# usnistgov/alignn

Hardware: AMD Instinct MI355X
Metric: graphs/sec (train fwd+bwd), batch=64 JARVIS-DFT crystals, 4+4 ALIGNN layers (higher is better)
Workload: dtype f32 (projections: split-product MFMA - 3 fp16-slice or 6 bf16-slice products, fp32 accumulate, fp32-grade error)

## Files before the change

### alignn_amd/_abi.py

```python

from __future__ import annotations

import ctypes as C
import keyword
import os
import re
from functools import lru_cache
from typing import NamedTuple

HEADER = os.path.join(os.path.dirname(os.path.dirname(os.path.abspath(__file__))), "include", "alignn_hip.h")

WORKFLOW_HEADERS = ("alignn_thermo.h", "alignn_neb.h", "alignn_traj.h", "alignn_sym.h", "alignn_order.h", "alignn_phsym.h")
LATER_HEADERS = ("alignn_idpp.h", "alignn_cells.h", "alignn_local.h")
ANALYSIS_HEADERS = ("alignn_vanhove.h",)
STRUCTURE_HEADERS = ("alignn_voronoi.h",)

_BASE = {"void": None, "char": C.c_char, "uint8_t": C.c_uint8, "uint64_t": C.c_uint64, "int": C.c_int, "int32_t": C.c_int32,
         "int64_t": C.c_int64, "size_t": C.c_size_t, "float": C.c_float, "double": C.c_double}

_ITEM = re.compile(r"typedef\s+struct\s+(\w+)\s*\{([^{}]*)\}\s*(\w+)\s*;"
                   r"|typedef\s+([^;{}()]+);"
                   r"|([^;{}()]+?\b\w+)\s*\(([^;{}()]*)\)\s*;")
_GAP = re.compile(r'\s*(extern\s*"C"\s*\{)?\s*\}?\s*')
_DECLARATION = re.compile(r"\s*(?:const\s+)?(\w+)\b(.*)", re.S)
_DECLARATOR = re.compile(r"\s*(\**)\s*(\w+)\s*")
_DIRECTIVE = re.compile(r"^[ \t]*#[ \t]*define\b(.*)$", re.M)
_MACRO = re.compile(r"[ \t]+(\w+)(?![\w(])[ \t]*(.*?)[ \t]*")
_INT = re.compile(r"[+-]?(?:0[xX][0-9a-fA-F]+|[1-9][0-9]*|0)")
_FLOAT = re.compile(r"[+-]?(?:[0-9]+\.[0-9]*|\.[0-9]+|[0-9]+(?=[eE]))(?:[eE][+-]?[0-9]+)?")


def _uncomment(text: str) -> str:
    return re.sub(r"/\*.*?\*/", lambda m: " " + "\n" * m.group().count("\n"), text, flags=re.S)


def parse(text: str):
    text = re.sub(r"^[ \t]*#.*$", "", _uncomment(text), flags=re.M)
    types, structs, sigs = dict(_BASE), {}, {}

    def fail(what, at):
        raise ValueError(f"line {text.count(chr(10), 0, at) + 1}: {what}")

    def gap(a, b):
        if not _GAP.fullmatch(text, a, b):
            junk = text[a:b]
            fail(f"cannot read {junk.strip()!r}", a + len(junk) - len(junk.lstrip()))

    def decl(s, at):
        at += len(s) - len(s.lstrip())
        m = _DECLARATION.fullmatch(s)
        if not m or m.group(1) not in types:
            fail(f"unknown type in {s.strip()!r}", at)
        out = []
        for d in m.group(2).split(","):
            dm = _DECLARATOR.fullmatch(d)
            ctype = (C.c_void_p if dm.group(1) else types[m.group(1)]) if dm else None
            if ctype is None:
                fail(f"cannot read the declarator {d.strip()!r} of {s.strip()!r}", at)
            name = dm.group(2)
            out.append((name + "_" if keyword.iskeyword(name) else name, ctype))
        return out

    pos = 0
    for m in _ITEM.finditer(text):
        gap(pos, m.start())
        pos = m.end()
        tag, body, name, alias, head, params = m.groups()
        if tag is not None:
            if tag != name:
                fail(f"struct {tag} is named {name}", m.start())
            fields = [f for s in body.split(";") if s.strip() for f in decl(s, m.start(2) + body.find(s))]
            types[name] = structs[name] = type(name, (C.Structure,), {"_fields_": fields})
        elif alias is not None:
            (name, ctype), = decl(alias, m.start())
            types[name] = ctype
        else:
            (name, res), = decl(head, m.start(5))
            if re.match(r"\s*const\s+char\s*\*", head):
                res = C.c_char_p
            args = [] if params.strip() == "void" else [decl(p, m.start(6))[0][1] for p in params.split(",")]
            sigs[name] = (res, args)
    gap(pos, len(text))
    return structs, sigs


def defines(text: str) -> dict:
    text, out = _uncomment(text), {}
    for m in _DIRECTIVE.finditer(text):
        macro = _MACRO.fullmatch(m.group(1))
        name, value = macro.groups() if macro else (None, None)
        if value and _INT.fullmatch(value):
            out[name] = int(value, 0)
        elif value and _FLOAT.fullmatch(value):
            out[name] = float(value)
        elif value != "":
            raise ValueError(f"line {text.count(chr(10), 0, m.start()) + 1}: cannot read the macro {m.group().strip()!r}")
    return out


class Header(NamedTuple):
    path: str
    structs: dict
    signatures: dict
    defines: dict


@lru_cache(maxsize=None)
def header(name: str) -> Header:
    path = os.path.join(os.path.dirname(HEADER), name)
    with open(path) as f:
        text = f.read()
    structs, sigs = parse(text)
    for block in structs:
        if sigs.get(block + "_size") != (C.c_size_t, []):
            raise ValueError(f"{name}: the argument block {block} has no size query size_t {block}_size(void)")
    return Header(path, structs, sigs, defines(text))


with open(HEADER) as _f:
    STRUCTS, SIGNATURES = parse(_f.read())
```

### alignn_amd/_lib.py

```python

from __future__ import annotations

import ctypes as C
import os

import torch

from ._abi import SIGNATURES, STRUCTS

HERE = os.path.dirname(os.path.abspath(__file__))
LIB_PATH = os.path.join(HERE, "libalignn_hip.so")
LIB_PATH = os.environ.get("ALIGNN_AMD_LIB_PATH", LIB_PATH)

EgcFwdArgs, EgcBwdArgs, EgcWgradArgs = (STRUCTS[f"alignn_egc_{k}_args"] for k in ("fwd", "bwd", "wgrad"))
FireArgs, MdArgs = STRUCTS["alignn_fire_args"], STRUCTS["alignn_md_args"]


_lib = None
_bound = {}


def _type(lib, signatures):
    for name, (res, args) in signatures.items():
        fn = getattr(lib, name)
        fn.restype = res
        fn.argtypes = args


def _check_size(name, size, block):
    if size != C.sizeof(block):
        raise RuntimeError(f"argument block {name}: library says {size} bytes, the header gives {C.sizeof(block)}")


def load() -> C.CDLL:
    global _lib
    if _lib is None:
        if not os.path.exists(LIB_PATH):
            raise RuntimeError(
                f"{LIB_PATH} not found: build it with `python -m alignn_amd.build` "
                "(hipcc --offload-arch=gfx950); alignn_amd has no CPU/eager fallback."
            )
        lib = C.CDLL(LIB_PATH)
        _type(lib, SIGNATURES)
        sizes = [lib.alignn_egc_args_sizeof(k) for k in range(3)] + [lib.alignn_fire_args_sizeof(), lib.alignn_md_args_sizeof()]
        for size, block in zip(sizes, (EgcFwdArgs, EgcBwdArgs, EgcWgradArgs, FireArgs, MdArgs)):
            _check_size(block.__name__, size, block)
        _lib = lib
    return _lib


def bind(header, lib=None):
    lib = load() if lib is None else lib
    if _bound.get(header.path) is not lib:
        _type(lib, header.signatures)
        for name, block in header.structs.items():
            _check_size(name, getattr(lib, name + "_size")(), block)
        _bound[header.path] = lib
    return lib


def ptr(t):
    return None if t is None else t.data_ptr()


_raw_stream = getattr(torch._C, "_cuda_getCurrentRawStream", None)


def stream():
    if _raw_stream is not None:
        return _raw_stream(torch.cuda.current_device())
    return torch.cuda.current_stream().cuda_stream


class _NoGuard:
    def __enter__(self):
        return None

    def __exit__(self, *exc):
        return False


_NO_GUARD = _NoGuard()


def device_guard(t):
    if t.is_cuda and t.device.index != torch.cuda.current_device():
        return torch.cuda.device(t.device)
    return _NO_GUARD


def check(rc: int, what: str):
    if rc != 0:
        raise RuntimeError(f"libalignn_hip: {what} failed with hipError {rc}")


def require_f32(*tensors):
    for t in tensors:
        if t is None:
            continue
        if t.dtype != torch.float32 or not t.is_cuda:
            raise TypeError(
                f"alignn_amd kernels take float32 CUDA(HIP) tensors, got {t.dtype} on {t.device}; "
                "there is no CPU fallback"
            )
```

### alignn_amd/build.py

```python

from __future__ import annotations

import os
import re
import shutil
import subprocess
import sys
import tempfile
from concurrent.futures import ThreadPoolExecutor

from ._abi import ANALYSIS_HEADERS, LATER_HEADERS, STRUCTURE_HEADERS, WORKFLOW_HEADERS

HERE = os.path.dirname(os.path.abspath(__file__))
CSRC = os.path.join(HERE, "csrc")
OBJ = os.path.join(HERE, "build")
LIB = os.path.join(HERE, "libalignn_hip.so")
SOURCES = ["norm.hip", "conv.hip", "gemm_f32.hip", "gemm_x6.hip", "embed.hip", "dual.hip", "knn.hip", "composite.hip", "model.hip", "stage.hip", "radius.hip", "angle.hip", "ff.hip", "convln.hip", "gemm_dw.hip", "relax.hip", "dynamics.hip", "phonon.hip", "defects.hip", "eos.hip", "elastic.hip", "interface.hip", "thermo.hip", "neb.hip", "trajectory.hip", "symmetry.hip", "order.hip", "phonon_sym.hip", "idpp.hip", "cells.hip", "local_order.hip", "vanhove.hip", "voronoi.hip"]
FLAGS = ["--offload-arch=gfx950", "-O3", "-std=c++17", "-fPIC"]
DEVICE_FLAGS: list = []
_NO_SLP = ["-fno-slp-vectorize"]
EXTRA_FLAGS = {"norm.hip": _NO_SLP, "dual.hip": _NO_SLP, "convln.hip": _NO_SLP, "radius.hip": _NO_SLP, "ff.hip": _NO_SLP}

_OBJDUMP = "/opt/rocm/lib/llvm/bin/llvm-objdump"
_PK = re.compile(r"\b(v_pk_(?:fma|mul|add)_f32)\b(.*)$")
_OPSEL = re.compile(r"op_sel:\[([01]),([01])")
_SYM = re.compile(r"^[0-9a-f]+ <([^>]+)>:$")


def faulting_packed_forms(lib: str = None) -> list:
    lib = lib or LIB
    found = []
    with tempfile.TemporaryDirectory() as tmp:
        copy = os.path.join(tmp, "lib.so")
        shutil.copy(lib, copy)
        subprocess.run([_OBJDUMP, "--offloading", copy], check=True, capture_output=True)
        bundles = sorted(f for f in os.listdir(tmp) if "gfx950" in f)
        if not bundles:
            raise RuntimeError(f"{lib}: no gfx950 code object found")
        for b in bundles:
            dis = subprocess.run([_OBJDUMP, "-d", "--no-show-raw-insn", os.path.join(tmp, b)], check=True, capture_output=True, text=True).stdout
            cur = "?"
            for line in dis.splitlines():
                m = _SYM.match(line)
                if m:
                    cur = m.group(1)
                    continue
                m = _PK.search(line)
                if m:
                    o = _OPSEL.search(m.group(2))
                    if o and o.group(2) == "1":
                        found.append((cur, (m.group(1) + m.group(2)).split("//")[0].strip()))
    return found


def _headers():
    include = os.path.join(os.path.dirname(HERE), "include")
    return [os.path.join(CSRC, f) for f in os.listdir(CSRC) if f.endswith(".h")] + [
        os.path.join(include, f) for f in ("alignn_hip.h",) + WORKFLOW_HEADERS + LATER_HEADERS + ANALYSIS_HEADERS + STRUCTURE_HEADERS]


def _stale(target, deps) -> bool:
    if not os.path.exists(target):
        return True
    t = os.path.getmtime(target)
    return any(os.path.getmtime(d) > t for d in deps)


def build(force: bool = False, verbose: bool = False) -> str:
    hipcc = os.environ.get("HIPCC", "/opt/rocm/bin/hipcc")
    hdrs = _headers()
    srcs = [s for s in SOURCES if os.path.exists(os.path.join(CSRC, s))]
    if not force and not _stale(LIB, [os.path.join(CSRC, s) for s in srcs] + hdrs + [os.path.abspath(__file__)]):
        return LIB
    os.makedirs(OBJ, exist_ok=True)
    objs = [os.path.join(OBJ, s.replace(".hip", ".o")) for s in srcs]

    def compile_one(pair):
        src, obj = pair
        if force or _stale(obj, [os.path.join(CSRC, src), os.path.abspath(__file__)] + hdrs):
            cmd = [hipcc] + FLAGS + DEVICE_FLAGS + EXTRA_FLAGS.get(src, []) + ["-c", os.path.join(CSRC, src), "-o", obj]
            if verbose:
                print(" ".join(cmd), flush=True)
            subprocess.run(cmd, check=True)
            return True
        return False

    with ThreadPoolExecutor(max_workers=min(8, len(srcs))) as pool:
        rebuilt = list(pool.map(compile_one, zip(srcs, objs)))
    if force or any(rebuilt) or _stale(LIB, objs):
        cmd = [hipcc, "--offload-arch=gfx950", "-shared", "-fPIC", "-o", LIB] + objs
        if verbose:
            print(" ".join(cmd), flush=True)
        subprocess.run(cmd, check=True)
        bad = faulting_packed_forms(LIB)
        if bad:
            os.replace(LIB, LIB + ".rejected")
            raise RuntimeError("libalignn_hip.so contains the packed-fp32 form that MI355X gets wrong beside MFMA waves "
                               "(see EXTRA_FLAGS in alignn_amd/build.py): " + "; ".join(f"{k}: {i}" for k, i in bad[:8]))
    return LIB


if __name__ == "__main__":
    print(build(force="--force" in sys.argv, verbose=True))
```

### alignn_amd/csrc/composite.hip

```cpp
#include "common.h"
#include "../../include/alignn_hip.h"

namespace {

inline size_t al(size_t floats) { return (floats + 63) / 64 * 64; }

#define ALIGNN_TRY(call)            \
    do {                            \
        int rc__ = (call);          \
        if (rc__ != 0) return rc__; \
    } while (0)

struct FwdScratch {
    size_t e_part, e_fold, n_part, bd2, total;
    int e_slabs, n_slabs;
};
FwdScratch fwd_scratch(int64_t n, int64_t m, int H, int Kin, int edge_kind) {
    FwdScratch s{};
    s.n_slabs = alignn_egc_slabs(n);
    s.e_slabs = edge_kind >= 1 ? alignn_gemm_nt_x6_row_tiles(m, H, Kin) : s.n_slabs;
    size_t off = 0;
    s.e_part = off, off += al(edge_kind >= 1 ? (size_t)(s.e_slabs + 1) * 2 * H : (size_t)s.e_slabs * (3 * H + 1));
    s.e_fold = off, off += al((size_t)alignn_slab_fold_slabs() * 2 * H);
    s.n_part = off, off += al((size_t)s.n_slabs * (3 * H + 1));
    s.bd2 = off, off += edge_kind == 2 ? al((size_t)n * H) : 0;
    s.total = off;
    return s;
}

struct BwdScratch {
    size_t n_red_part, e_red_part, dx_ws, dy_part, dy_fold, total;
    int n_slabs, e_slabs, dy_tiles;
    size_t dx_bytes;
};
BwdScratch bwd_scratch(int64_t n, int64_t m, int H, int Kin, int dx_kind, int dy_kind) {
    BwdScratch s{};
    s.n_slabs = alignn_col_stats_slabs(n);
    s.e_slabs = alignn_col_stats_slabs(m);
    size_t off = 0;
    s.n_red_part = off, off += al((size_t)s.n_slabs * 2 * H);
    s.e_red_part = off, off += al((size_t)s.e_slabs * 2 * H);
    s.dx_bytes = dx_kind == 2 ? alignn_gemm_nn_split_workspace(n, 4 * H, Kin) : 0;
    s.dx_ws = off, off += al(s.dx_bytes / 4);
    s.dy_tiles = dy_kind == 1 ? alignn_gemm_nt_x6_row_tiles(m, Kin, H) : 0;
    s.dy_part = off, off += al((size_t)(s.dy_tiles + 1) * 2 * Kin);
    s.dy_fold = off, off += al((size_t)alignn_slab_fold_slabs() * 2 * Kin);
    s.total = off;
    return s;
}

int bn_finalize_folded(const float* partial, int slabs, float* fold, int64_t rows, int F, const float* gamma,
                       const float* beta, float eps, float momentum, float* rm, float* rv, float* stat,
                       alignn_stream_t st) {
    if (slabs > kFoldAbove) {
        ALIGNN_TRY(alignn_slab_fold(partial, slabs, 2 * F, fold, st));
        partial = fold;
        slabs = alignn_slab_fold_slabs();
    }
    return alignn_bn_finalize(partial, slabs, rows, F, gamma, beta, eps, momentum, rm, rv, stat, st);
}

hipEvent_t g_fork_ev[kMaxDevices][2];
bool g_fork_ok[kMaxDevices];

inline bool fork_events(hipEvent_t* fork, hipEvent_t* join) {
    int dev = -1;
    if (hipGetDevice(&dev) != hipSuccess || dev < 0 || dev >= kMaxDevices || !g_fork_ok[dev]) return false;
    *fork = g_fork_ev[dev][0];
    *join = g_fork_ev[dev][1];
    return true;
}

}

extern "C" {

int alignn_fork_events_init(void) {
    int dev = -1;
    hipError_t e = hipGetDevice(&dev);
    if (e != hipSuccess) return (int)e;
    if (dev < 0 || dev >= kMaxDevices) return (int)hipErrorInvalidDevice;
    if (g_fork_ok[dev]) return 0;
    for (int i = 0; i < 2; ++i) {
        e = hipEventCreateWithFlags(&g_fork_ev[dev][i], hipEventDisableTiming);
        if (e != hipSuccess) return (int)e;
    }
    g_fork_ok[dev] = true;
    return 0;
}

size_t alignn_egc_args_sizeof(int which) {
    switch (which) {
        case 0: return sizeof(alignn_egc_fwd_args);
        case 1: return sizeof(alignn_egc_bwd_args);
        case 2: return sizeof(alignn_egc_wgrad_args);
        default: return 0;
    }
}

size_t alignn_egc_conv_fwd_scratch(int64_t n, int64_t m, int H, int Kin, int edge_kind) {
    return fwd_scratch(n, m, H, Kin, edge_kind).total * sizeof(float);
}

int alignn_egc_conv_fwd(const alignn_egc_fwd_args* a, alignn_stream_t st) {
    if (a == nullptr || a->scratch == nullptr || a->H <= 0 || (a->H & 3)) return (int)hipErrorInvalidValue;
    const int H = a->H, Kin = a->Kin;
    const int64_t n = a->n, m = a->m;
    const FwdScratch s = fwd_scratch(n, m, H, Kin, a->edge_kind);
    if (a->scratch_bytes < s.total * sizeof(float)) return (int)hipErrorInvalidValue;
    float* e_part = a->scratch + s.e_part;
    float* e_fold = a->scratch + s.e_fold;
    float* n_part = a->scratch + s.n_part;
    if (a->node_kind == 1)
        ALIGNN_TRY(alignn_gemm_nt_f16x3(a->x, Kin, a->x_amax, a->wcat_img, a->wcat_amax, a->bcat, nullptr, 0, a->P, 4 * H, n,
                                        4 * H, Kin, st));
    else
        ALIGNN_TRY(alignn_gemm_nt(a->x, Kin, a->wcat, Kin, a->bcat, nullptr, 0, a->P, 4 * H, n, 4 * H, Kin, st));
    if (a->edge_kind >= 1) {
        if (a->edge_kind == 2) {
            if (a->seg_rank == nullptr || a->seg_node == nullptr) return (int)hipErrorInvalidValue;
            float* bd2 = a->scratch + s.bd2;
            ALIGNN_TRY(alignn_gather_rows_ld(a->P + H, 4 * H, a->seg_node, bd2, H, n, H, st));
            ALIGNN_TRY(alignn_gemm_nt_f16x3_gather2(a->y, Kin, a->y_amax, a->weg_img, a->weg_amax, a->b_eg, a->M, H, m, H, Kin,
                                                    a->P, 4 * H, a->src, bd2, H, a->seg_rank, e_part, st));
        } else
            ALIGNN_TRY(alignn_gemm_nt_f16x3_gather(a->y, Kin, a->y_amax, a->weg_img, a->weg_amax, a->b_eg, a->M, H, m, H, Kin,
                                                   a->P, 4 * H, a->src, a->dst, e_part, st));
        ALIGNN_TRY(bn_finalize_folded(e_part, s.e_slabs, e_fold, m, H, a->e_gamma, a->e_beta, a->eps, a->momentum, a->e_rm,
                                      a->e_rv, a->e_stat, st));
        if (a->y_out != nullptr)
            ALIGNN_TRY(alignn_egc_gate_fwd_pre_norm(a->P, a->M, a->seg_ptr, a->seg_node, a->src, n, m, H, a->xpre, a->s0, a->hh,
                                                    n_part, a->e_stat, a->residual ? a->y : nullptr, a->y_out, a->y_out_amax, st));
        else
            ALIGNN_TRY(alignn_egc_gate_fwd_pre(a->P, a->M, a->seg_ptr, a->seg_node, a->src, n, m, H, a->xpre, a->s0, a->hh,
                                               nullptr, n_part, st));
    } else {
        ALIGNN_TRY(alignn_gemm_nt(a->y, Kin, a->w_eg, Kin, a->b_eg, nullptr, 0, a->M, H, m, H, Kin, st));
        ALIGNN_TRY(alignn_egc_gate_fwd(a->P, a->M, a->seg_ptr, a->seg_node, a->src, n, m, H, a->xpre, a->s0, a->hh, e_part,
                                       n_part, st));
        ALIGNN_TRY(alignn_bn_finalize_welford(e_part, s.e_slabs, m, H, a->e_gamma, a->e_beta, a->eps, a->momentum, a->e_rm,
                                              a->e_rv, a->e_stat, st));
        if (a->y_out != nullptr)
            ALIGNN_TRY(alignn_bn_silu_fwd(a->M, H, a->residual ? a->y : nullptr, a->residual ? Kin : 0, a->e_stat, a->y_out, H,
                                          m, H, a->y_out_amax, st));
    }
    ALIGNN_TRY(alignn_bn_finalize_welford(n_part, s.n_slabs, n, H, a->n_gamma, a->n_beta, a->eps, a->momentum, a->n_rm,
                                          a->n_rv, a->n_stat, st));
    ALIGNN_TRY(alignn_bn_silu_fwd(a->xpre, H, a->residual ? a->x : nullptr, a->residual ? Kin : 0, a->n_stat, a->x_out, H, n, H,
                                  a->x_out_amax, st));
    return 0;
}

size_t alignn_egc_conv_bwd_scratch(int64_t n, int64_t m, int H, int Kin, int dx_kind, int dy_kind) {
    return bwd_scratch(n, m, H, Kin, dx_kind, dy_kind).total * sizeof(float);
}

int alignn_egc_conv_bwd(const alignn_egc_bwd_args* a, alignn_stream_t st) {
    if (a == nullptr || a->scratch == nullptr || a->H <= 0 || (a->H & 3)) return (int)hipErrorInvalidValue;
    const int H = a->H, Kin = a->Kin;
    const int64_t n = a->n, m = a->m;
    const BwdScratch s = bwd_scratch(n, m, H, Kin, a->dx_kind, a->dy_kind);
    if (a->scratch_bytes < s.total * sizeof(float)) return (int)hipErrorInvalidValue;
    float* n_red_part = a->scratch + s.n_red_part;
    float* e_red_part = a->scratch + s.e_red_part;
    float* g_xpre = a->GP + 3 * (size_t)H;
    ALIGNN_TRY(alignn_bn_silu_bwd_reduce(a->gx_out, H, a->xpre, H, a->n_stat, n, H, n_red_part, st));
    ALIGNN_TRY(alignn_bn_bwd_finalize(n_red_part, s.n_slabs, H, a->n_red, st));
    ALIGNN_TRY(alignn_bn_silu_bwd_apply_node(a->gx_out, H, a->xpre, H, a->n_stat, a->n_gamma, a->n_red, 0, g_xpre, 4 * H, n, H,
                                             a->gp_amax, a->s0, a->hh, a->gs1, a->gs0, st));
    const float* e_red = a->e_red_in;
    if (a->gy_out != nullptr && e_red == nullptr) {
        ALIGNN_TRY(alignn_bn_silu_bwd_reduce(a->gy_out, H, a->M, H, a->e_stat, m, H, e_red_part, st));
        ALIGNN_TRY(alignn_bn_bwd_finalize(e_red_part, s.e_slabs, H, a->e_red, st));
        e_red = a->e_red;
    }
    if (a->gate_mode == 2) {
        ALIGNN_TRY(alignn_egc_bwd_lg_dense(a->gy_out, a->M, a->P, a->gs1, a->gs0, a->e_stat, e_red, 0, m, a->grp_seg_ptr,
                                           a->grp_src_ptr, a->n_groups, a->dense_max_src, a->seg_ptr, a->seg_node, H, a->GM,
                                           a->GP, a->gb_part, a->gm_amax, a->gp_amax, st));
    } else if (a->gate_mode == 1) {
        ALIGNN_TRY(alignn_egc_bwd_lg_fused(a->gy_out, a->M, a->P, a->gs1, a->gs0, a->e_stat, e_red, 0, m, a->grp_seg_ptr,
                                           a->grp_src_ptr, a->n_groups, a->seg_ptr, a->seg_node, a->dst, a->out_ptr, a->out_slot,
                                           H, a->GM, a->GP, a->gb_part, a->gm_amax, a->gp_amax, st));
    } else {
        ALIGNN_TRY(alignn_egc_bwd_dst(a->gy_out, a->M, a->P, a->gs1, a->gs0, a->e_stat, a->e_gamma, e_red, 0, m, a->seg_ptr,
                                      a->seg_node, a->src, n, H, a->GM, a->GP, a->gb_part, a->gm_amax, a->gp_amax, st));
        ALIGNN_TRY(alignn_egc_bwd_src(a->GM, a->M, a->gs1, a->out_ptr, a->out_slot, a->dst, n, H, a->GP, a->gp_amax, st));
    }
    hipEvent_t ev_fork, ev_join;
    const bool forked = a->aux_stream != nullptr && fork_events(&ev_fork, &ev_join);
    alignn_stream_t st_main = st;
    if (forked) {
        ALIGNN_TRY((int)hipEventRecord(ev_fork, (hipStream_t)st_main));
        ALIGNN_TRY((int)hipStreamWaitEvent((hipStream_t)a->aux_stream, ev_fork, 0));
        st = a->aux_stream;
    }
    const float* addx = a->residual ? a->gx_out : nullptr;
    switch (a->dx_kind) {
        case 1:
            ALIGNN_TRY(alignn_gemm_nt_f16x3(a->GP, 4 * H, a->gp_amax, a->wcat_t_img, a->wcat_amax, nullptr, addx, addx ? H : 0, a->g_x, Kin, n,
                                            Kin, 4 * H, st));
            break;
        case 2:
            ALIGNN_TRY(alignn_gemm_nn_split(a->GP, 4 * H, a->wcat, Kin, addx, addx ? H : 0, a->g_x, Kin, n, 4 * H, Kin,
                                            a->scratch + s.dx_ws, s.dx_bytes, st));
            break;
        case 4:
            ALIGNN_TRY(alignn_gemm_nt(a->GP, 4 * H, a->wcat_t, 4 * H, nullptr, addx, addx ? H : 0, a->g_x, Kin, n, Kin, 4 * H, st));
            break;
        default:
            ALIGNN_TRY(alignn_gemm_nn(a->GP, 4 * H, a->wcat, Kin, addx, addx ? H : 0, a->g_x, Kin, n, 4 * H, Kin, st));
    }
    if (forked) {
        ALIGNN_TRY((int)hipEventRecord(ev_join, (hipStream_t)a->aux_stream));
        st = st_main;
    }
    const float* addy = (a->residual && a->gy_out != nullptr) ? a->gy_out : nullptr;
    switch (a->dy_kind) {
        case 1: {
            float* part = a->scratch + s.dy_part;
            ALIGNN_TRY(alignn_gemm_nt_f16x3_bnred(a->GM, H, a->gm_amax, a->weg_t_img, a->weg_amax, nullptr, addy, addy ? H : 0,
                                                  a->g_y, Kin, m, Kin, H, a->src_xn, a->src_ldxn, a->src_nstat, part, st));
            int tiles = s.dy_tiles;
            if (tiles > kFoldAbove) {
                ALIGNN_TRY(alignn_slab_fold(part, tiles, 2 * Kin, a->scratch + s.dy_fold, st));
                part = a->scratch + s.dy_fold;
                tiles = alignn_slab_fold_slabs();
            }
            ALIGNN_TRY(alignn_bn_bwd_finalize(part, tiles, Kin, a->src_red, st));
            break;
        }
        case 5:
            ALIGNN_TRY(alignn_gemm_nt_f16x3(a->GM, H, a->gm_amax, a->weg_t_img, a->weg_amax, nullptr, addy, addy ? H : 0, a->g_y,
                                            Kin, m, Kin, H, st));
            break;
        case 2: {
            const size_t bytes = alignn_gemm_nn_split_workspace(m, H, Kin);
            (void)bytes;
            return (int)hipErrorInvalidValue;
        }
        case 4:
            ALIGNN_TRY(alignn_gemm_nt(a->GM, H, a->weg_t, H, nullptr, addy, addy ? H : 0, a->g_y, Kin, m, Kin, H, st));
            break;
        default:
            ALIGNN_TRY(alignn_gemm_nn(a->GM, H, a->w_eg, Kin, addy, addy ? H : 0, a->g_y, Kin, m, H, Kin, st));
    }
    if (forked) ALIGNN_TRY((int)hipStreamWaitEvent((hipStream_t)st_main, ev_join, 0));
    return 0;
}

size_t alignn_egc_conv_wgrad_scratch(int64_t n, int64_t m, int H, int Kin) {
    return (al(alignn_gemm_tn_workspace(m, H, Kin) / 4 + 1) + al(alignn_gemm_tn_workspace(n, 4 * H, Kin) / 4 + 1) +
            al((size_t)alignn_col_stats_slabs(n) * 2 * 4 * H)) * sizeof(float);
}

int alignn_egc_conv_wgrad(const alignn_egc_wgrad_args* a, alignn_stream_t st) {
    if (a == nullptr || a->scratch == nullptr) return (int)hipErrorInvalidValue;
    const int H = a->H, Kin = a->Kin;
    const int64_t n = a->n, m = a->m;
    const size_t b1 = alignn_gemm_tn_workspace(m, H, Kin), b2 = alignn_gemm_tn_workspace(n, 4 * H, Kin);
    float* ws1 = a->scratch;
    float* ws2 = ws1 + al(b1 / 4 + 1);
    float* ws3 = ws2 + al(b2 / 4 + 1);
    if (a->scratch_bytes < alignn_egc_conv_wgrad_scratch(n, m, H, Kin)) return (int)hipErrorInvalidValue;
    ALIGNN_TRY(alignn_slab_sum(a->gb_part, a->gb_slabs, H, a->g_beg, st));
    ALIGNN_TRY(alignn_gemm_tn(a->GM, H, a->gm_amax, a->y, Kin, a->y_amax, a->g_weg, Kin, m, H, Kin, ws1, b1, st));
    ALIGNN_TRY(alignn_gemm_tn(a->GP, 4 * H, a->gp_amax, a->x, Kin, a->x_amax, a->g_wcat, Kin, n, 4 * H, Kin, ws2, b2, st));
    ALIGNN_TRY(alignn_col_sum(a->GP, 4 * H, n, 4 * H, a->g_bcat, ws3, st));
    return 0;
}

}
```

### alignn_amd/csrc/gemm_f32.hip

```cpp
#include "mfma_f16x3.h"
#include "../../include/alignn_hip.h"

namespace {

constexpr int BK = 32;
constexpr int RC_LD = BK + 4;

template <int BMN, bool RC>
struct TileShape {
    static constexpr int kFloats = RC ? BMN * RC_LD : BK * BMN;
};

template <int BMN, bool RC, int NT>
struct Stager {
    static constexpr int NV = (BMN * BK / 4) / NT;
    static_assert((BMN * BK / 4) % NT == 0, "tile must divide over the block");
    float4 v[NV];

    __device__ __forceinline__ void load(const float* __restrict__ S, int64_t ld, int64_t i0, int64_t i_ext,
                                         int64_t r0, int64_t r_ext, int t) {
#pragma unroll
        for (int j = 0; j < NV; ++j) {
            const int id = t + j * NT;
            int64_t gi, gr;
            if (RC) {
                gi = i0 + id / (BK / 4);
                gr = r0 + (id % (BK / 4)) * 4;
            } else {
                gr = r0 + id / (BMN / 4);
                gi = i0 + (id % (BMN / 4)) * 4;
            }
            if (gi < i_ext && gr < r_ext)
                v[j] = RC ? f4_ld(S + gi * ld + gr) : f4_ld(S + gr * ld + gi);
            else
                v[j] = f4_zero();
        }
    }
    __device__ __forceinline__ void store(float* T, int t) const {
#pragma unroll
        for (int j = 0; j < NV; ++j) {
            const int id = t + j * NT;
            if (RC)
                f4_st(T + (id / (BK / 4)) * RC_LD + (id % (BK / 4)) * 4, v[j]);
            else
                f4_st(T + (id / (BMN / 4)) * BMN + (id % (BMN / 4)) * 4, v[j]);
        }
    }
};

template <int BMN, bool RC>
__device__ __forceinline__ void fetch4(const float* T, int irow, int j, int half, float (&out)[4]) {
    if (RC) {
        float4 q = f4_ld(T + irow * RC_LD + 8 * j + 4 * half);
        out[0] = q.x;
        out[1] = q.y;
        out[2] = q.z;
        out[3] = q.w;
    } else {
        const float* p = T + (8 * j + 4 * half) * BMN + irow;
        out[0] = p[0];
        out[1] = p[BMN];
        out[2] = p[2 * BMN];
        out[3] = p[3 * BMN];
    }
}

struct GemmArgs {
    const float* A;
    int64_t lda;
    const float* B;
    int64_t ldb;
    const float* bias;
    const float* addend;
    int64_t ldadd;
    float* C;
    int64_t ldc;
    int64_t Mo;
    int No;
    int64_t R;
    int64_t r_chunk;
    int64_t c_split;
    int xcd_group;
    int tiles_m, tiles_n, splits;
};

template <int BM, int BN, int WM, int WN, bool A_RC, bool B_RC, bool HAS_ADD>
__global__ __launch_bounds__(WM * WN * 64) void gemm_mfma_kernel(GemmArgs g) {
    constexpr int NT = WM * WN * 64;
    constexpr int TM = BM / WM, TN = BN / WN;
    constexpr int RM = TM / 32, RN = TN / 32;
    constexpr int A_FL = TileShape<BM, A_RC>::kFloats, B_FL = TileShape<BN, B_RC>::kFloats;
    extern __shared__ __attribute__((aligned(16))) float smem[];
    constexpr int STAGE = A_FL + B_FL;

    const int t = threadIdx.x;
    const int lane = t & 63, wave = t >> 6;
    const int wm = wave / WN, wn = wave % WN;
    const int il = lane & 31, half = lane >> 5;
    int bx = blockIdx.x, by = blockIdx.y, bz = blockIdx.z;
    if (g.xcd_group) {
        const int tiles = g.tiles_m * g.tiles_n;
        const int L = blockIdx.x;
        const int xcd = L & 7, j = L >> 3;
        bz = xcd + 8 * (j / tiles);
        const int tile = j % tiles;
        bx = tile % g.tiles_m;
        by = tile / g.tiles_m;
        if (bz >= g.splits) return;
    }
    const int64_t m0 = (int64_t)bx * BM;
    const int64_t n0 = (int64_t)by * BN;
    const int64_t rbeg = (int64_t)bz * g.r_chunk;
    int64_t rend = rbeg + g.r_chunk;
    if (rend > g.R) rend = g.R;
    float* C = g.C + (int64_t)bz * g.c_split;

    f32x16 acc[RM][RN];
#pragma unroll
    for (int a = 0; a < RM; ++a)
#pragma unroll
        for (int b = 0; b < RN; ++b)
#pragma unroll
            for (int r = 0; r < 16; ++r) acc[a][b][r] = 0.0f;

    const bool vec = ((g.No & 3) == 0) && ((g.ldc & 3) == 0) && ((reinterpret_cast<uintptr_t>(C) & 15) == 0) &&
                     (g.addend == nullptr || (((g.ldadd & 3) == 0) && ((reinterpret_cast<uintptr_t>(g.addend) & 15) == 0)));
    const int64_t ecol = n0 + wn * TN + (lane & 15) * 4;
    float4 ebias = f4_zero();
    if (vec && g.bias && ecol < g.No) ebias = f4_ld(g.bias + ecol);

    Stager<BM, A_RC, NT> sa;
    Stager<BN, B_RC, NT> sb;
    const int nk = rend > rbeg ? (int)((rend - rbeg + BK - 1) / BK) : 0;
    if (nk > 0) {
        sa.load(g.A, g.lda, m0, g.Mo, rbeg, rend, t);
        sb.load(g.B, g.ldb, n0, g.No, rbeg, rend, t);
        sa.store(smem, t);
        sb.store(smem + A_FL, t);
    }
    __syncthreads();
    for (int kt = 0; kt < nk; ++kt) {
        const int cur = kt & 1;
        if (kt + 1 < nk) {
            sa.load(g.A, g.lda, m0, g.Mo, rbeg + (int64_t)(kt + 1) * BK, rend, t);
            sb.load(g.B, g.ldb, n0, g.No, rbeg + (int64_t)(kt + 1) * BK, rend, t);
        }
        const float* At = smem + cur * STAGE;
        const float* Bt = At + A_FL;
#pragma unroll
        for (int j = 0; j < 4; ++j) {
            float af[RM][4], bf[RN][4];
#pragma unroll
            for (int a = 0; a < RM; ++a) fetch4<BM, A_RC>(At, wm * TM + a * 32 + il, j, half, af[a]);
#pragma unroll
            for (int b = 0; b < RN; ++b) fetch4<BN, B_RC>(Bt, wn * TN + b * 32 + il, j, half, bf[b]);
#pragma unroll
            for (int s = 0; s < 4; ++s)
#pragma unroll
                for (int a = 0; a < RM; ++a)
#pragma unroll
                    for (int b = 0; b < RN; ++b)
                        acc[a][b] = __builtin_amdgcn_mfma_f32_32x32x2f32(af[a][s], bf[b][s], acc[a][b], 0, 0, 0);
        }
        if (kt + 1 < nk) {
            sa.store(smem + (cur ^ 1) * STAGE, t);
            sb.store(smem + (cur ^ 1) * STAGE + A_FL, t);
        }
        __syncthreads();
    }

    if (vec) {
        constexpr int PLD = TN + 4;
        static_assert(WM * WN * 32 * PLD <= 2 * STAGE, "epilogue patch must fit in the staging LDS");
        float* patch = smem + wave * (32 * PLD);
        const int prow = lane >> 4, pc4 = (lane & 15) * 4;
        static_assert(TN == 64, "epilogue assumes 64-column wave tiles");
        const int64_t col = ecol;
        const int64_t colc = col < g.No ? col : 0;
        const float4 bv = ebias;
#pragma unroll
        for (int a = 0; a < RM; ++a) {
            __syncthreads();
#pragma unroll
            for (int b = 0; b < RN; ++b)
#pragma unroll
                for (int r = 0; r < 16; ++r)
                    patch[((r & 3) + 8 * (r >> 2) + 4 * half) * PLD + b * 32 + il] = acc[a][b][r];
            __syncthreads();
            float4 ov[8], av[8];
#pragma unroll
            for (int i = 0; i < 8; ++i) ov[i] = f4_ld(patch + (i * 4 + prow) * PLD + pc4);
            const int64_t row0 = m0 + wm * TM + a * 32 + prow;
            if (HAS_ADD) {
#pragma unroll
                for (int i = 0; i < 8; ++i) {
                    int64_t row = row0 + i * 4;
                    if (row >= g.Mo) row = g.Mo - 1;
                    av[i] = f4_ld(g.addend + row * g.ldadd + colc);
                }
            }
#pragma unroll
            for (int i = 0; i < 8; ++i) {
                const int64_t row = row0 + i * 4;
                float4 v = f4_add(ov[i], bv);
                if (HAS_ADD) v = f4_add(v, av[i]);
                if (row < g.Mo && col < g.No) f4_st(C + row * g.ldc + col, v);
            }
        }
        return;
    }
#pragma unroll
    for (int a = 0; a < RM; ++a) {
#pragma unroll
        for (int b = 0; b < RN; ++b) {
            const int64_t col = n0 + wn * TN + b * 32 + il;
            if (col >= g.No) continue;
            const float bv = g.bias ? g.bias[col] : 0.0f;
#pragma unroll
            for (int r = 0; r < 16; ++r) {
                const int64_t row = m0 + wm * TM + a * 32 + (r & 3) + 8 * (r >> 2) + 4 * half;
                if (row < g.Mo) {
                    float v = acc[a][b][r] + bv;
                    if (HAS_ADD) v += g.addend[row * g.ldadd + col];
                    C[row * g.ldc + col] = v;
                }
            }
        }
    }
}

__global__ void gemm_naive_kernel(const float* __restrict__ A, int64_t sai, int64_t sar, const float* __restrict__ B,
                                  int64_t sbj, int64_t sbr, const float* __restrict__ bias,
                                  const float* __restrict__ addend, int64_t ldadd, float* __restrict__ C, int64_t ldc,
                                  int64_t Mo, int No, int64_t R) {
    int64_t idx = (int64_t)blockIdx.x * blockDim.x + threadIdx.x;
    if (idx >= Mo * No) return;
    int64_t i = idx / No;
    int j = (int)(idx - i * No);
    float acc = 0.0f;
    for (int64_t r = 0; r < R; ++r) acc = fmaf(A[i * sai + r * sar], B[j * sbj + r * sbr], acc);
    if (bias) acc += bias[j];
    if (addend) acc += addend[i * ldadd + j];
    C[i * ldc + j] = acc;
}

__global__ __launch_bounds__(256) void gemm_naive_wave_kernel(const float* __restrict__ A, int64_t sai, const float* __restrict__ B,
                                                              int64_t sbj, const float* __restrict__ bias,
                                                              const float* __restrict__ addend, int64_t ldadd, float* __restrict__ C,
                                                              int64_t ldc, int64_t Mo, int No, int64_t R) {
    const int lane = threadIdx.x & 63;
    const int64_t idx = (int64_t)blockIdx.x * 4 + (threadIdx.x >> 6);
    if (idx >= Mo * No) return;
    const int64_t i = idx / No;
    const int j = (int)(idx - i * No);
    float acc = 0.0f;
    for (int64_t r = lane; r < R; r += 64) acc = fmaf(A[i * sai + r], B[j * sbj + r], acc);
#pragma unroll
    for (int o = 32; o > 0; o >>= 1) acc += __shfl_xor(acc, o, 64);
    if (lane == 0) {
        if (bias) acc += bias[j];
        if (addend) acc += addend[i * ldadd + j];
        C[i * ldc + j] = acc;
    }
}

__global__ __launch_bounds__(1024) void slab_reduce_kernel(const float* __restrict__ ws, int splits, int64_t count,
                                                           int cols, float* __restrict__ out, int64_t ldo) {
    __shared__ double sh[32][32];
    const int64_t idx = (int64_t)blockIdx.x * 32 + threadIdx.x;
    double s = 0.0;
    if (idx < count)
        for (int k = threadIdx.y; k < splits; k += 32) s += (double)ws[(int64_t)k * count + idx];
    sh[threadIdx.y][threadIdx.x] = s;
    __syncthreads();
    if (threadIdx.y == 0 && idx < count) {
        double t = 0.0;
#pragma unroll 8
        for (int k = 0; k < 32; ++k) t += sh[k][threadIdx.x];
        out[(idx / cols) * ldo + (idx % cols)] = (float)t;
    }
}


__global__ __launch_bounds__(1024) void slab_reduce4_kernel(const float* __restrict__ ws, int splits, int64_t count,
                                                            int cols, float* __restrict__ out, int64_t ldo) {
    __shared__ double sh[16][64][4];
    const int64_t idx = ((int64_t)blockIdx.x * 64 + threadIdx.x) * 4;
    double s0 = 0.0, s1 = 0.0, s2 = 0.0, s3 = 0.0;
    if (idx < count) {
        int k = threadIdx.y;
        for (; k + 48 < splits; k += 64) {
            float4 v[4];
#pragma unroll
            for (int u = 0; u < 4; ++u) v[u] = f4_ld(ws + (int64_t)(k + 16 * u) * count + idx);
#pragma unroll
            for (int u = 0; u < 4; ++u) {
                s0 += (double)v[u].x;
                s1 += (double)v[u].y;
                s2 += (double)v[u].z;
                s3 += (double)v[u].w;
            }
        }
        for (; k < splits; k += 16) {
            float4 v = f4_ld(ws + (int64_t)k * count + idx);
            s0 += (double)v.x;
            s1 += (double)v.y;
            s2 += (double)v.z;
            s3 += (double)v.w;
        }
    }
    double* mine = sh[threadIdx.y][threadIdx.x];
    mine[0] = s0, mine[1] = s1, mine[2] = s2, mine[3] = s3;
    __syncthreads();
    if (threadIdx.y == 0 && idx < count) {
        double t0 = 0.0, t1 = 0.0, t2 = 0.0, t3 = 0.0;
#pragma unroll 4
        for (int k = 0; k < 16; ++k) {
            const double* p = sh[k][threadIdx.x];
            t0 += p[0], t1 += p[1], t2 += p[2], t3 += p[3];
        }
        f4_st(out + (idx / cols) * ldo + (idx % cols), make_float4((float)t0, (float)t1, (float)t2, (float)t3));
    }
}

inline void launch_slab_reduce(const float* ws, int splits, int64_t count, int cols, float* out, int64_t ldo,
                               hipStream_t st) {
    if ((count & 3) == 0 && (cols & 3) == 0 && (ldo & 3) == 0 && aligned16(out) && aligned16(ws))
        hipLaunchKernelGGL(slab_reduce4_kernel, dim3(alignn_ceil_div(count, 256)), dim3(64, 16), 0, st, ws, splits, count,
                           cols, out, ldo);
    else
        hipLaunchKernelGGL(slab_reduce_kernel, dim3(alignn_ceil_div(count, 32)), dim3(32, 32), 0, st, ws, splits, count,
                           cols, out, ldo);
}

template <int BM, int BN, int WM, int WN, bool A_RC, bool B_RC, bool HAS_ADD>
int launch_k(const GemmArgs& g, int splits, hipStream_t stream);

template <int BM, int BN, int WM, int WN, bool A_RC, bool B_RC>
int launch(const GemmArgs& g, int splits, hipStream_t stream) {
    return g.addend ? launch_k<BM, BN, WM, WN, A_RC, B_RC, true>(g, splits, stream)
                    : launch_k<BM, BN, WM, WN, A_RC, B_RC, false>(g, splits, stream);
}

template <int BM, int BN, int WM, int WN, bool A_RC, bool B_RC, bool HAS_ADD>
int launch_k(const GemmArgs& g, int splits, hipStream_t stream) {
    constexpr int NT = WM * WN * 64;
    constexpr size_t lds = 2 * (TileShape<BM, A_RC>::kFloats + TileShape<BN, B_RC>::kFloats) * sizeof(float);
    auto kern = gemm_mfma_kernel<BM, BN, WM, WN, A_RC, B_RC, HAS_ADD>;
    static bool attr_set = false;
    if (!attr_set && lds > 64 * 1024) {
        hipError_t e = hipFuncSetAttribute((const void*)kern, hipFuncAttributeMaxDynamicSharedMemorySize, (int)lds);
        if (e != hipSuccess) return (int)e;
        attr_set = true;
    }
    dim3 grid(alignn_ceil_div(g.Mo, BM), alignn_ceil_div(g.No, BN), splits);
    if (g.xcd_group) {
        GemmArgs h = g;
        h.tiles_m = grid.x;
        h.tiles_n = grid.y;
        h.splits = splits;
        const int per_xcd = alignn_ceil_div(splits, 8) * h.tiles_m * h.tiles_n;
        hipLaunchKernelGGL(kern, dim3(per_xcd * 8), dim3(NT), lds, stream, h);
        ALIGNN_CHECK_LAUNCH();
        return 0;
    }
    hipLaunchKernelGGL(kern, grid, dim3(NT), lds, stream, g);
    ALIGNN_CHECK_LAUNCH();
    return 0;
}

int naive(const float* A, int64_t sai, int64_t sar, const float* B, int64_t sbj, int64_t sbr, const float* bias,
          const float* addend, int64_t ldadd, float* C, int64_t ldc, int64_t Mo, int No, int64_t R,
          hipStream_t stream) {
    if (Mo * No == 0) return 0;
    if (sar == 1 && sbr == 1 && R >= 128 && Mo * No <= 4096) {
        hipLaunchKernelGGL(gemm_naive_wave_kernel, dim3(alignn_ceil_div(Mo * No, 4)), dim3(256), 0, stream, A, sai, B, sbj, bias,
                           addend, ldadd, C, ldc, Mo, No, R);
        ALIGNN_CHECK_LAUNCH();
        return 0;
    }
    hipLaunchKernelGGL(gemm_naive_kernel, dim3(alignn_ceil_div(Mo * No, 256)), dim3(256), 0, stream, A, sai, sar, B,
                       sbj, sbr, bias, addend, ldadd, C, ldc, Mo, No, R);
    ALIGNN_CHECK_LAUNCH();
    return 0;
}


inline int64_t tn_chunk(int64_t M, int N, int K) {
    const int bn = K > 64 ? 128 : 64;
    const int bm = (N <= 64 && K <= 64) ? 64 : 128;
    const int64_t tiles = (int64_t)alignn_ceil_div(N, bm) * alignn_ceil_div(K, bn);
    int64_t want = (768 + tiles - 1) / tiles;
    if (want < 1) want = 1;
    int64_t chunk = (M + want - 1) / want;
    chunk = ((chunk + BK - 1) / BK) * BK;
    if (chunk < 4 * BK) chunk = 4 * BK;
    return chunk;
}
inline int tn_splits(int64_t M, int N, int K) {
    const int64_t c = tn_chunk(M, N, K);
    int64_t s = (M + c - 1) / c;
    return (int)(s < 1 ? 1 : s);
}

}

extern "C" {

int alignn_gemm_nt(const float* A, int64_t lda, const float* W, int64_t ldw, const float* bias, const float* addend,
                   int64_t ldadd, float* C, int64_t ldc, int64_t M, int N, int K, alignn_stream_t stream) {
    if (M < 0 || N <= 0 || K <= 0) return (int)hipErrorInvalidValue;
    if (M == 0) return 0;
    hipStream_t st = (hipStream_t)stream;
    const bool vec_ok = (K % 4 == 0) && (lda % 4 == 0) && (ldw % 4 == 0) && aligned16(A) && aligned16(W);
    if (!vec_ok || N < 16 || (bias != nullptr && !aligned16(bias)))
        return naive(A, lda, 1, W, ldw, 1, bias, addend, ldadd, C, ldc, M, N, K, st);
    GemmArgs g{A, lda, W, ldw, bias, addend, ldadd, C, ldc, M, N, K, K, 0, 0, 0, 0, 0};
    const int64_t big_blocks = (int64_t)alignn_ceil_div(M, 128) * alignn_ceil_div(N, 256);
    if (N > 128 && big_blocks >= 1024) return launch<128, 256, 2, 4, true, true>(g, 1, st);
    if (N > 64) return launch<64, 128, 2, 2, true, true>(g, 1, st);
    return launch<128, 64, 4, 1, true, true>(g, 1, st);
}

int alignn_gemm_nn(const float* G, int64_t ldg, const float* W, int64_t ldw, const float* addend, int64_t ldadd,
                   float* C, int64_t ldc, int64_t M, int N, int K, alignn_stream_t stream) {
    if (M < 0 || N <= 0 || K <= 0) return (int)hipErrorInvalidValue;
    if (M == 0) return 0;
    hipStream_t st = (hipStream_t)stream;
    const bool vec_ok = (N % 4 == 0) && (K % 4 == 0) && (ldg % 4 == 0) && (ldw % 4 == 0) && aligned16(G) && aligned16(W);
    if (!vec_ok || K < 16)
        return naive(G, ldg, 1, W, 1, ldw, nullptr, addend, ldadd, C, ldc, M, K, N, st);
    GemmArgs g{G, ldg, W, ldw, nullptr, addend, ldadd, C, ldc, M, K, N, N, 0, 0, 0, 0, 0};
    if (K > 128) return launch<128, 256, 2, 4, true, false>(g, 1, st);
    if (K > 64) return launch<128, 128, 2, 2, true, false>(g, 1, st);
    return launch<128, 64, 4, 1, true, false>(g, 1, st);
}

static int nn_splits(int64_t M, int N, int K) {
    const int64_t tiles = (int64_t)alignn_ceil_div(M, 128) * alignn_ceil_div(K, 256);
    if (K <= 128 || tiles >= 128 || N < 512 || (N % 128) != 0) return 1;
    int s = N / 128;
    while (s > 8) s >>= 1;
    return (N % s == 0 && (N / s) % BK == 0) ? s : 1;
}

namespace {
__global__ __launch_bounds__(256) void splitk_sum_kernel(const float* __restrict__ ws, int splits, int64_t slab, int cols,
                                                         const float* __restrict__ addend, int64_t ldadd,
                                                         float* __restrict__ out, int64_t ldo, int64_t rows) {
    const int Q = cols >> 2;
    const RowQuad rq(Q);
    const int64_t total = rows * Q;
    for (int64_t i = (int64_t)blockIdx.x * 256 + threadIdx.x; i < total; i += (int64_t)gridDim.x * 256) {
        int64_t r;
        int q;
        rq.split(i, total, r, q);
        float4 s = addend ? f4_ld(addend + r * ldadd + q * 4) : f4_zero();
        for (int z = 0; z < splits; ++z) s = f4_add(s, f4_ld(ws + (int64_t)z * slab + r * cols + q * 4));
        f4_st(out + r * ldo + q * 4, s);
    }
}
}

size_t alignn_gemm_nn_split_workspace(int64_t M, int N, int K) {
    const int s = nn_splits(M, N, K);
    return s > 1 ? (size_t)s * (size_t)M * (size_t)K * sizeof(float) : 0;
}

int alignn_gemm_nn_split(const float* G, int64_t ldg, const float* W, int64_t ldw, const float* addend, int64_t ldadd,
                         float* C, int64_t ldc, int64_t M, int N, int K, void* workspace, size_t workspace_bytes,
                         alignn_stream_t stream) {
    const int splits = nn_splits(M, N, K);
    const bool vec_ok = (N % 4 == 0) && (K % 4 == 0) && (ldg % 4 == 0) && (ldw % 4 == 0) && (ldc % 4 == 0) && aligned16(G) &&
                        aligned16(W) && aligned16(C) && (addend == nullptr || ((ldadd % 4 == 0) && aligned16(addend)));
    if (splits <= 1 || !vec_ok || workspace == nullptr || workspace_bytes < alignn_gemm_nn_split_workspace(M, N, K) ||
        !aligned16(workspace))
        return (int)hipErrorInvalidValue;
    hipStream_t st = (hipStream_t)stream;
    GemmArgs g{G, ldg, W, ldw, nullptr, nullptr, 0, (float*)workspace, K, M, K, N, N / splits, M * (int64_t)K, 0, 0, 0, 0};
    int rc = launch<128, 256, 2, 4, true, false>(g, splits, st);
    if (rc) return rc;
    const int64_t quads = M * (int64_t)(K >> 2);
    int grid = (int)((quads + 255) / 256);
    if (grid > 4096) grid = 4096;
    hipLaunchKernelGGL(splitk_sum_kernel, dim3(grid), dim3(256), 0, st, (const float*)workspace, splits, M * (int64_t)K, K,
                       addend, ldadd, C, ldc, M);
    ALIGNN_CHECK_LAUNCH();
    return 0;
}

int alignn_gemm_tn_x6_supported(int64_t M, int N, int K);
size_t alignn_gemm_tn_x6_workspace(int64_t M, int N, int K);
int alignn_gemm_tn_x6_splits(int64_t M, int N, int K);
static bool tn_use_x6(const float* G, int64_t ldg, const float* A, int64_t lda, int64_t M, int N, int K) {
    return alignn_gemm_tn_x6_supported(M, N, K) && (ldg % 4 == 0) && (lda % 4 == 0) && aligned16(G) && aligned16(A);
}

size_t alignn_gemm_tn_workspace(int64_t M, int N, int K) {
    const size_t f32 = (size_t)tn_splits(M, N, K) * (size_t)N * (size_t)K * sizeof(float);
    if (alignn_gemm_tn_x6_supported(M, N, K)) {
        const size_t x6 = alignn_gemm_tn_x6_workspace(M, N, K);
        return x6 > f32 ? x6 : f32;
    }
    return f32;
}

int alignn_gemm_tn(const float* G, int64_t ldg, const float* g_amax, const float* A, int64_t lda, const float* a_amax,
                   float* dW, int64_t lddw, int64_t M, int N, int K, void* workspace, size_t workspace_bytes,
                   alignn_stream_t stream) {
    if (M < 0 || N <= 0 || K <= 0) return (int)hipErrorInvalidValue;
    hipStream_t st = (hipStream_t)stream;
    const bool vec_ok = (N % 4 == 0) && (K % 4 == 0) && (ldg % 4 == 0) && (lda % 4 == 0) && aligned16(G) && aligned16(A);
    if (!vec_ok || M == 0) return naive(G, 1, ldg, A, 1, lda, nullptr, nullptr, 0, dW, lddw, N, K, M, st);
    if (workspace_bytes < alignn_gemm_tn_workspace(M, N, K) || workspace == nullptr) return (int)hipErrorInvalidValue;
    float* ws = (float*)workspace;
    if (tn_use_x6(G, ldg, A, lda, M, N, K)) {
        const bool f16 = g_amax != nullptr && a_amax != nullptr;
        int rc6 = alignn_gemm_tn_x6_partials(G, ldg, f16 ? g_amax : nullptr, A, lda, f16 ? a_amax : nullptr, M, N, K,
                                             workspace, workspace_bytes, stream);
        if (rc6) return rc6;
        const int64_t count6 = (int64_t)N * K;
        launch_slab_reduce(ws, alignn_gemm_tn_x6_splits(M, N, K), count6, K, dW, lddw, st);
        ALIGNN_CHECK_LAUNCH();
        return 0;
    }
    const int splits = tn_splits(M, N, K);
    GemmArgs g{G, ldg, A, lda, nullptr, nullptr, 0, ws, K, N, K, M, tn_chunk(M, N, K), (int64_t)N * K, 1, 0, 0, 0};
    int rc;
    if (K > 64)
        rc = launch<128, 128, 2, 2, false, false>(g, splits, st);
    else if (N > 64)
        rc = launch<128, 64, 4, 1, false, false>(g, splits, st);
    else
        rc = launch<64, 64, 2, 1, false, false>(g, splits, st);
    if (rc) return rc;
    const int64_t count = (int64_t)N * K;
    launch_slab_reduce(ws, splits, count, K, dW, lddw, st);
    ALIGNN_CHECK_LAUNCH();
    return 0;
}

}
```

### alignn_amd/csrc/gemm_x6.hip

```cpp
#include <cstdlib>

#include "mfma_f16x3.h"
#include "../../include/alignn_hip.h"

namespace {

typedef __bf16 bf16x8 __attribute__((ext_vector_type(8)));
typedef _Float16 f16x2 __attribute__((ext_vector_type(2)));

constexpr int WM = 2, WN = 2, NT = WM * WN * 64;
constexpr int BN = 256, BK = 16;
constexpr int TN = BN / WN, RN = TN / 32;
constexpr int B_PLANE = BN * BK * 2;
template <int RM_>
struct Geo {
    static constexpr int RM = RM_, BM = WM * 32 * RM_, TM = BM / WM;
    static constexpr int A_BYTES = BM * BK * 4;
    static constexpr int A_DMA = A_BYTES / 1024 / (NT / 64);
};
constexpr int EPI_BYTES = (NT / 64) * 32 * (64 + 4) * 4;
constexpr int EPI1_LDS = EPI_BYTES + (NT / 64) * 2 * 2 * 256 * 4;
template <bool F16, int RM_ = 2>
struct Sch {
    static constexpr int NPL = F16 ? 2 : 3;
// ... 492 lines not shown
                bh[b] = __builtin_bit_cast(f16x8, *reinterpret_cast<const uint4*>(q));
                bl[b] = __builtin_bit_cast(f16x8, *reinterpret_cast<const uint4*>(q + B_PLANE));
            }
#define X6_PASS(AA, BB)                                                                              \
    _Pragma("unroll") for (int a = 0; a < RM; ++a) _Pragma("unroll") for (int b = 0; b < RN; ++b)    \
        acc[a][b] = __builtin_amdgcn_mfma_f32_32x32x16_f16(AA[a], BB[b], acc[a][b], 0, 0, 0);
            X6_PASS(ah, bh)
#pragma unroll
            for (int a = 0; a < RM; ++a) slice8_f16_lo(xs[a], ah[a], al[a]);
            X6_PASS(ah, bl)
            X6_PASS(al, bh)
#undef X6_PASS
        }
        wait_vmcnt<0>();
        block_barrier();
        float* patch = reinterpret_cast<float*>(smem + (slot == 0 ? NS - 1 : slot - 1) * STAGE_BYTES + wave * PATCH_BYTES);
        const int last_row = (int)(g.M - 1 - m0 < BM - 1 ? g.M - 1 - m0 : BM - 1);
        int prow_e = prow, pc4_e = pc4;
        asm volatile("" : "+v"(prow_e), "+v"(pc4_e));
        float* c_t = g.C + m0 * g.ldc;
        const float* bd_tab = GATHER ? (g.gp2 ? g.gp2 : g.gp + g.N) : nullptr;
        const int64_t bd_ld = GATHER ? (g.gp2 ? g.ldgp2 : g.ldgp) : 0;
        const float* add_t = HAS_ADD ? g.addend + m0 * g.ldadd : nullptr;
        const float* xn_t = BNRED ? g.xn + m0 * g.ldxn : nullptr;
        const int col0 = n0 + wn * TN + pc4_e;
        constexpr int D = (BNRED && HAS_ADD) ? 1 : 2, NH = 2 * RN * RM;
        float4 av[(HAS_ADD || GATHER) ? D : 1][2], xv[BNRED ? D : 1][2], nst[BNRED ? 2 : 1][3], bias_b[2], s0, s1;
        auto row_of = [&](int a, int i) {
            const int rrel = wm * TM + a * 32 + prow_e + i * 8;
            return rrel < last_row ? rrel : last_row;
        };
        auto load_half = [&](int q) {
            const int b = q / (2 * RM), a = (q / 2) % RM, h = q & 1, col = col0 + b * 32, sl = q % D;
            if constexpr (GATHER) {
                int ui[2], vi[2];
#pragma unroll
                for (int i = 0; i < 2; ++i) {
                    const int holder = a * 32 + (2 * h + i) * 8 + prow_e;
                    ui[i] = __shfl(src_l, holder);
                    vi[i] = __shfl(dst_l, holder);
                }
#pragma unroll
                for (int i = 0; i < 2; ++i)
                    av[sl][i] = f4_add(f4_ld(g.gp + (int64_t)ui[i] * g.ldgp + col), f4_ld(bd_tab + (int64_t)vi[i] * bd_ld + col));
            }
            if constexpr (HAS_ADD) {
#pragma unroll
                for (int i = 0; i < 2; ++i) av[sl][i] = f4_ld(add_t + (row_of(a, 2 * h + i) * (int)g.ldadd + col));
            }
            if constexpr (BNRED) {
#pragma unroll
                for (int i = 0; i < 2; ++i) xv[sl][i] = f4_lds<true>(xn_t + (row_of(a, 2 * h + i) * (int)g.ldxn + col));
            }
            if (a == 0 && h == 0) {
                bias_b[b & 1] = g.bias ? f4_ld(g.bias + col) : f4_zero();
                if constexpr (BNRED)
                    nst[b & 1][0] = f4_ld(g.nstat + col), nst[b & 1][1] = f4_ld(g.nstat + 2 * g.N + col),
                              nst[b & 1][2] = f4_ld(g.nstat + 3 * g.N + col);
            }
        };
#pragma unroll
        for (int q = 0; q < D; ++q) load_half(q);
#pragma unroll
        for (int rd = 0; rd < RN * RM; ++rd) {
            const int b = rd / RM, a = rd % RM;
            const int col = col0 + b * 32;
            if (a == 0 && (BNRED || STATS)) s0 = s1 = f4_zero();
#pragma unroll
            for (int r = 0; r < 16; ++r) patch[((r & 3) + 8 * (r >> 2) + 4 * half) * PLD + il] = acc[a][b][r];
#pragma unroll
            for (int h = 0; h < 2; ++h) {
                const int q = 2 * rd + h, sl = q % D;
                float4 v[2];
#pragma unroll
                for (int i = 0; i < 2; ++i) {
                    v[i] = f4_ld(patch + ((2 * h + i) * 8 + prow) * PLD + pc4);
                    v[i] = f4_scale(f4_scale(v[i], inv_sa), inv_sw);
                    v[i] = f4_add(v[i], bias_b[b & 1]);
                    if constexpr (HAS_ADD || GATHER) v[i] = f4_add(v[i], av[sl][i]);
                    const bool valid = wm * TM + a * 32 + prow_e + (2 * h + i) * 8 <= last_row;
                    if constexpr (STATS) {
                        const float4 u = valid ? v[i] : f4_zero();
                        s0 = f4_add(s0, u);
                        s1 = f4_fma(u, u, s1);
                    }
                    if constexpr (BNRED) {
                        const float4 xc = f4_sub(xv[sl][i], nst[b & 1][0]);
                        const float4 z = f4_fma(xc, nst[b & 1][1], nst[b & 1][2]);
                        float4 gz = make_float4(v[i].x * dsilu_f(z.x), v[i].y * dsilu_f(z.y), v[i].z * dsilu_f(z.z), v[i].w * dsilu_f(z.w));
                        gz = valid ? gz : f4_zero();
                        s0 = f4_add(s0, gz);
                        s1 = f4_fma(gz, xc, s1);
                    }
                }
                __builtin_amdgcn_sched_barrier(0);
                if (q + D < NH) load_half(q + D);
                __builtin_amdgcn_sched_barrier(0);
#pragma unroll
                for (int i = 0; i < 2; ++i) f4_sts<true>(c_t + (row_of(a, 2 * h + i) * (int)g.ldc + col), v[i]);
                if (a == RM - 1 && h == 1 && (BNRED || STATS)) {
#pragma unroll
                    for (int d = 8; d < 64; d <<= 1) {
                        s0 = f4_add(s0, make_float4(__shfl_xor(s0.x, d), __shfl_xor(s0.y, d), __shfl_xor(s0.z, d), __shfl_xor(s0.w, d)));
                        s1 = f4_add(s1, make_float4(__shfl_xor(s1.x, d), __shfl_xor(s1.y, d), __shfl_xor(s1.z, d), __shfl_xor(s1.w, d)));
                    }
                    if constexpr (BNRED) s1 = f4_mul(s1, f4_ld(g.nstat + g.N + col));
                    const int64_t n_strips = (g.M + TM - 1) / TM;
                    int64_t strip = m0 / TM + wm;
                    strip = strip < n_strips ? strip : n_strips;
                    f4_st(g.red_partial + (strip * 2 + 0) * g.N + col, s0);
                    f4_st(g.red_partial + (strip * 2 + 1) * g.N + col, s1);
                }
            }
        }
    }
}

template <bool HAS_ADD>
__global__ __launch_bounds__(NT) void gemm_nt_f16p_kernel(X6Args g) {
    gemm_nt_f16p_body<HAS_ADD, 0>(g);
}
template <bool HAS_ADD>
__global__ __launch_bounds__(NT) __attribute__((amdgpu_waves_per_eu(2))) void gemm_nt_f16p_bnred_kernel(X6Args g) {
    gemm_nt_f16p_body<HAS_ADD, 1>(g);
}
template <bool STATS>
__global__ __launch_bounds__(NT) __attribute__((amdgpu_waves_per_eu(2))) void gemm_nt_f16p_gather_kernel(X6Args g) {
    gemm_nt_f16p_body<false, 2 | (STATS ? 4 : 0)>(g);
}
__global__ __launch_bounds__(NT) __attribute__((amdgpu_waves_per_eu(2))) void gemm_nt_f16p_stats_kernel(X6Args g) {
    gemm_nt_f16p_body<false, 4>(g);
}


namespace tn {
constexpr int TBN = 256, TBK = 256, TSTEP = 16;
constexpr int TWM = 4, TWN = 2, TNT = TWM * TWN * 64;
constexpr int TRM = 2, TRN = 4;
constexpr int TPLANE = TBN * TSTEP * 2;
constexpr int TEPI = (TNT / 64) * 32 * (64 + 4) * 4;
template <bool F16>
struct TSch {
    static constexpr int NPL = F16 ? 2 : 3;
    static constexpr int BUF = 2 * NPL * TPLANE;
    static constexpr int LDS = 2 * BUF > TEPI ? 2 * BUF : TEPI;
};

struct TnArgs {
    const float* G;
    int64_t ldg;
    const float* X;
    int64_t ldx;
    float* ws;
    int64_t M;
    int N, K;
    int64_t chunk;
    int tiles_n, tiles_k, splits;
    const float* g_amax;
    const float* x_amax;
};

template <bool F16>
__global__ __launch_bounds__(TNT) void gemm_tn_x6_kernel(TnArgs g) {
    extern __shared__ __attribute__((aligned(16))) unsigned char smem[];
    constexpr int NPL = TSch<F16>::NPL, BUF = TSch<F16>::BUF;
    const int t = threadIdx.x;
    const int lane = t & 63;
    const int wave = __builtin_amdgcn_readfirstlane(t >> 6);
    const int wm = wave / TWN, wn = wave % TWN;
    const int il = lane & 31, half = lane >> 5;
    const int tiles = g.tiles_n * g.tiles_k;
    const int L = blockIdx.x;
    const int z = (L & 7) + 8 * ((L >> 3) / tiles);
    if (z >= g.splits) return;
    const int tile = (L >> 3) % tiles;
    const int n0 = (tile % g.tiles_n) * TBN, k0 = (tile / g.tiles_n) * TBK;
    const int64_t rbeg = (int64_t)z * g.chunk;
    int64_t rend = rbeg + g.chunk;
    if (rend > g.M) rend = g.M;
    const int nst = rend > rbeg ? (int)((rend - rbeg + TSTEP - 1) / TSTEP) : 0;

    f32x16 acc[TRM][TRN];
#pragma unroll
    for (int a = 0; a < TRM; ++a)
#pragma unroll
        for (int b = 0; b < TRN; ++b)
#pragma unroll
            for (int r = 0; r < 16; ++r) acc[a][b][r] = 0.0f;

    const bool is_x = wave >= 4;
    const int col = t & 255;
    const float* src = is_x ? g.X + k0 + col : g.G + n0 + col;
    const int64_t ld = is_x ? g.ldx : g.ldg;
    float scale = 1.0f, inv_s0 = 1.0f, inv_s1 = 1.0f;
    if constexpr (F16) {
        const float sg = f16_scale(*g.g_amax), sx = f16_scale(*g.x_amax);
        scale = is_x ? sx : sg;
        const float inv_sg = 1.0f / sg, inv_sx = 1.0f / sx, inv_gx = inv_sg * inv_sx;
        inv_s0 = inv_gx != 0.0f ? inv_gx : inv_sg;
        inv_s1 = inv_gx != 0.0f ? 1.0f : inv_sx;
    }
    const int w_off = (is_x ? NPL * TPLANE : 0) + col * (TSTEP * 2);
    const int w_swz = (col >> 3) & 1;
    int a_off[TRM], b_off[TRN];
#pragma unroll
    for (int a = 0; a < TRM; ++a) {
        const int n = wm * 64 + a * 32 + il;
        a_off[a] = n * (TSTEP * 2) + ((half ^ ((n >> 3) & 1)) << 4);
    }
#pragma unroll
    for (int b = 0; b < TRN; ++b) {
        const int k = wn * 128 + b * 32 + il;
        b_off[b] = NPL * TPLANE + k * (TSTEP * 2) + ((half ^ ((k >> 3) & 1)) << 4);
    }

    const unsigned col_bytes = (unsigned)col * 4u;
    const char* sbase = reinterpret_cast<const char*>(is_x ? g.X + k0 : g.G + n0);
    const int64_t ld_bytes = ld * 4;
#define TN_LOAD(R, ST)                                                                                 \
    if ((ST) < nst) {                                                                                  \
        const int64_t r0_ = rbeg + (int64_t)(ST) * TSTEP;                                              \
        if (r0_ + TSTEP <= g.M) {                                                                      \
            const char* p_ = sbase + r0_ * ld_bytes;                                                   \
            _Pragma("unroll") for (int m = 0; m < TSTEP; ++m) {                                        \
                R[m] = __builtin_nontemporal_load(reinterpret_cast<const float*>(p_ + col_bytes));     \
                p_ += ld_bytes;                                                                        \
            }                                                                                          \
        } else {                                                                                       \
            _Pragma("unroll") for (int m = 0; m < TSTEP; ++m) {                                        \
                int64_t row = r0_ + m;                                                                 \
                row = row < g.M ? row : g.M - 1;                      \
                R[m] = __builtin_nontemporal_load(src + row * ld);                                     \
            }                                                                                          \
        }                                                                                              \
    }
#define TN_SLICE(R, ST, buf)                                                                                    \
    {                                                                                                           \
        const int valid = (int)((rend - (rbeg + (int64_t)(ST) * TSTEP)) < TSTEP ? (rend - (rbeg + (int64_t)(ST) * TSTEP)) : TSTEP); \
        if (valid < TSTEP) {       \
            _Pragma("unroll") for (int m = 0; m < TSTEP; ++m) R[m] = m < valid ? R[m] : 0.0f;                   \
        }                                                                                                       \
        _Pragma("unroll") for (int c = 0; c < 2; ++c) {                                                         \
            float x[8];                                                                                         \
            _Pragma("unroll") for (int j = 0; j < 8; ++j) x[j] = R[8 * c + j];                                  \
            unsigned char* dst = (buf) + w_off + ((c ^ w_swz) << 4);                                            \
            if constexpr (F16) {                                                                                \
                f16x8 h, l;                                                                                     \
                slice8_f16(make_float4(x[0], x[1], x[2], x[3]), make_float4(x[4], x[5], x[6], x[7]), scale, h, l); \
                *reinterpret_cast<f16x8*>(dst) = h;                                                             \
                *reinterpret_cast<f16x8*>(dst + TPLANE) = l;                                                    \
            } else {                                                                                            \
                bf16x8 h, mm, l;                                                                                \
                slice8(make_float4(x[0], x[1], x[2], x[3]), make_float4(x[4], x[5], x[6], x[7]), h, mm, l);     \
                *reinterpret_cast<bf16x8*>(dst) = h;                                                            \
                *reinterpret_cast<bf16x8*>(dst + TPLANE) = mm;                                                  \
                *reinterpret_cast<bf16x8*>(dst + 2 * TPLANE) = l;                                               \
            }                                                                                                   \
        }                                                                                                       \
    }
#define TN_PASS(TY, AA, BB)                                                                            \
    _Pragma("unroll") for (int a = 0; a < TRM; ++a) _Pragma("unroll") for (int b = 0; b < TRN; ++b)    \
        acc[a][b] = __builtin_amdgcn_mfma_f32_32x32x16_##TY(AA[a], BB[b], acc[a][b], 0, 0, 0);
#define TN_READ_F16(buf)                                                                                        \
    f16x8 ah[TRM], al[TRM], bh[TRN], bl[TRN];                                                                   \
    _Pragma("unroll") for (int a = 0; a < TRM; ++a) {                                                           \
        ah[a] = *reinterpret_cast<const f16x8*>((buf) + a_off[a]);                                              \
        al[a] = *reinterpret_cast<const f16x8*>((buf) + a_off[a] + TPLANE);                                     \
    }                                                                                                           \
    _Pragma("unroll") for (int b = 0; b < TRN; ++b) {                                                           \
        bh[b] = *reinterpret_cast<const f16x8*>((buf) + b_off[b]);                                              \
        bl[b] = *reinterpret_cast<const f16x8*>((buf) + b_off[b] + TPLANE);                                     \
    }
#define TN_MMA_F16 TN_PASS(f16, al, bh) TN_PASS(f16, ah, bl) TN_PASS(f16, ah, bh)
#define TN_MMA_BF16(buf)                                                                                        \
    {                                                                                                           \
        bf16x8 ah[TRM], am[TRM], al[TRM], bh[TRN], bm[TRN], bl[TRN];                                            \
        _Pragma("unroll") for (int a = 0; a < TRM; ++a) {                                                       \
            ah[a] = *reinterpret_cast<const bf16x8*>((buf) + a_off[a]);                                         \
            am[a] = *reinterpret_cast<const bf16x8*>((buf) + a_off[a] + TPLANE);                                \
            al[a] = *reinterpret_cast<const bf16x8*>((buf) + a_off[a] + 2 * TPLANE);                            \
        }                                                                                                       \
        _Pragma("unroll") for (int b = 0; b < TRN; ++b) {                                                       \
            bh[b] = *reinterpret_cast<const bf16x8*>((buf) + b_off[b]);                                         \
            bm[b] = *reinterpret_cast<const bf16x8*>((buf) + b_off[b] + TPLANE);                                \
            bl[b] = *reinterpret_cast<const bf16x8*>((buf) + b_off[b] + 2 * TPLANE);                            \
        }                                                                                                       \
        TN_PASS(bf16, al, bh) TN_PASS(bf16, ah, bl) TN_PASS(bf16, am, bm)                                       \
        TN_PASS(bf16, am, bh) TN_PASS(bf16, ah, bm) TN_PASS(bf16, ah, bh)                                       \
    }

    float ra[TSTEP], rb[TSTEP];
#define TN_STEP(R, ST, BUFI)                                                                                    \
    if ((ST) < nst) {                                                                                           \
        if ((ST) + 1 < nst)                                                                                     \
            wait_vmcnt<TSTEP>();                                                                                \
        else                                                                                                    \
            wait_vmcnt<0>();                                                                                    \
        unsigned char* buf = smem + (BUFI) * BUF;                                                               \
        TN_SLICE(R, ST, buf)                                                                                    \
        TN_LOAD(R, (ST) + 2)                                                                                    \
        block_barrier();     \
        if constexpr (F16) {                                                                                    \
            TN_READ_F16(buf)                                                                                    \
            TN_MMA_F16                                                                                          \
        } else {                                                                                                \
            TN_MMA_BF16(buf)                                                                                    \
        }                                                                                                       \
    }
    TN_LOAD(ra, 0)
    TN_LOAD(rb, 1)
    for (int st = 0; st < nst; st += 2) {
        TN_STEP(ra, st, 0)
        TN_STEP(rb, st + 1, 1)
    }
#undef TN_STEP
#undef TN_MMA_BF16
#undef TN_MMA_F16
#undef TN_READ_F16
#undef TN_PASS
#undef TN_SLICE
#undef TN_LOAD

    constexpr int PLD = 64 + 4;
    float* patch = reinterpret_cast<float*>(smem) + wave * (32 * PLD);
    const int prow = lane >> 4, pc4 = (lane & 15) * 4;
    float* out = g.ws + (int64_t)z * g.N * g.K;
#pragma unroll
    for (int ahb = 0; ahb < TRM * (TRN / 2); ++ahb) {
        const int a = ahb / (TRN / 2), hb = ahb % (TRN / 2);
        __syncthreads();
#pragma unroll
        for (int b = 0; b < 2; ++b)
#pragma unroll
            for (int r = 0; r < 16; ++r)
                patch[((r & 3) + 8 * (r >> 2) + 4 * half) * PLD + b * 32 + il] = acc[a][2 * hb + b][r];
        __syncthreads();
        float4 ov[8];
#pragma unroll
        for (int i = 0; i < 8; ++i) ov[i] = f4_ld(patch + (i * 4 + prow) * PLD + pc4);
        const int ocol = k0 + wn * 128 + hb * 64 + pc4;
        const int row0 = n0 + wm * 64 + a * 32 + prow;
#pragma unroll
        for (int i = 0; i < 8; ++i) {
            float4 v = ov[i];
            if constexpr (F16) v = f4_scale(f4_scale(v, inv_s0), inv_s1);
            f4_st(out + (int64_t)(row0 + i * 4) * g.K + ocol, v);
        }
    }
}

inline int64_t tn_chunk(int64_t M, int N, int K) {
    const int64_t tiles = (int64_t)(N / TBN) * (K / TBK);
    int64_t want = (256 + tiles - 1) / tiles;
    if (want < 1) want = 1;
    int64_t chunk = (M + want - 1) / want;
    chunk = ((chunk + TSTEP - 1) / TSTEP) * TSTEP;
    if (chunk < 8 * TSTEP) chunk = 8 * TSTEP;
    return chunk;
}
inline int tn_splits(int64_t M, int N, int K) {
    const int64_t c = tn_chunk(M, N, K);
    return (int)((M + c - 1) / c);
}
}

__global__ void split_bf16x3_kernel(const float* __restrict__ W, int64_t ldw, int N, int Npad, int K, int transpose,
                                    unsigned short* __restrict__ out) {
    const int64_t total = (int64_t)Npad * K;
    const int ntiles = Npad / BN;
    for (int64_t i = (int64_t)blockIdx.x * blockDim.x + threadIdx.x; i < total; i += (int64_t)gridDim.x * blockDim.x) {
        const int n = (int)(i / K), k = (int)(i % K);
        float x = 0.0f;
        if (n < N) x = transpose ? W[(int64_t)k * ldw + n] : W[(int64_t)n * ldw + k];
        const float r1 = x - trunc16(x);
        const float r2 = r1 - trunc16(r1);
        const int kb = k / BK, c = (k % BK) >> 3, e = k & 7;
        const int nt = n / BN, nin = n % BN;
        constexpr int plane = BN * BK;
        const int64_t o = ((int64_t)kb * ntiles + nt) * (3 * plane) + nin * BK + ((c ^ ((n >> 3) & 1)) << 3) + e;
        out[o] = (unsigned short)(__float_as_uint(x) >> 16);
        out[o + plane] = (unsigned short)(__float_as_uint(r1) >> 16);
        out[o + 2 * plane] = (unsigned short)(__float_as_uint(r2) >> 16);
    }
}

__global__ void split_f16x2_kernel(const float* __restrict__ W, int64_t ldw, int N, int Npad, int K, int transpose,
                                   const float* __restrict__ w_amax, _Float16* __restrict__ out) {
    const int64_t total = (int64_t)Npad * K;
    const int ntiles = Npad / BN;
    const float sw = f16_scale(*w_amax);
    for (int64_t i = (int64_t)blockIdx.x * blockDim.x + threadIdx.x; i < total; i += (int64_t)gridDim.x * blockDim.x) {
        const int n = (int)(i / K), k = (int)(i % K);
        float x = 0.0f;
        if (n < N) x = transpose ? W[(int64_t)k * ldw + n] : W[(int64_t)n * ldw + k];
        x *= sw;
        const _Float16 h = (_Float16)x;
        const _Float16 l = (_Float16)(x - (float)h);
        const int kb = k / BK, c = (k % BK) >> 3, e = k & 7;
        const int nt = n / BN, nin = n % BN;
        constexpr int plane = BN * BK;
        const int64_t o = ((int64_t)kb * ntiles + nt) * (2 * plane) + nin * BK + ((c ^ ((n >> 3) & 1)) << 3) + e;
        out[o] = h;
        out[o + plane] = l;
    }
}

__global__ void split_f16x2_both_kernel(const float* __restrict__ W, int64_t ldw, int N, int K, const float* __restrict__ w_amax,
                                        _Float16* __restrict__ out, _Float16* __restrict__ outT) {
    const float sw = f16_scale(*w_amax);
    constexpr int plane = BN * BK;
#pragma unroll
    for (int tr = 0; tr < 2; ++tr) {
        _Float16* o = tr ? outT : out;
        const int n_ = tr ? K : N, k_ = tr ? N : K, np = ((n_ + BN - 1) / BN) * BN, ntiles = np / BN;
        const int total = np * k_;
        for (int i = blockIdx.x * blockDim.x + threadIdx.x; i < total; i += gridDim.x * blockDim.x) {
            const int n = i / k_, k = i % k_;
            float x = 0.0f;
            if (n < n_) x = tr ? W[(int64_t)k * ldw + n] : W[(int64_t)n * ldw + k];
            x *= sw;
            const _Float16 h = (_Float16)x;
            const _Float16 l = (_Float16)(x - (float)h);
            const int kb = k / BK, c = (k % BK) >> 3, e = k & 7;
            const int nt = n / BN, nin = n % BN;
            const int64_t q = ((int64_t)kb * ntiles + nt) * (2 * plane) + nin * BK + ((c ^ ((n >> 3) & 1)) << 3) + e;
            o[q] = h;
            o[q + plane] = l;
        }
    }
}

__global__ __launch_bounds__(256) void absmax_kernel(const float* __restrict__ X, int64_t ldx, int64_t rows, int F,
                                                      float* __restrict__ amax) {
    const int Q = F >> 2;
    const RowQuad rq(Q);
    const int64_t total = rows * Q;
    float m = 0.0f;
    for (int64_t i = (int64_t)blockIdx.x * 256 + threadIdx.x; i < total; i += (int64_t)gridDim.x * 256) {
        int64_t r;
        int q;
        rq.split(i, total, r, q);
        const float4 v = f4_ld(X + r * ldx + q * 4);
        m = fmaxf(m, fmaxf(fmaxf(fabsf(v.x), fabsf(v.y)), fmaxf(fabsf(v.z), fabsf(v.w))));
    }
    block_amax_commit(m, amax);
}

struct WeightDesc {
    const float* W;
    int64_t ldw;
    int32_t N, K;
    float* amax;
    _Float16* out;
    _Float16* outT;
};
static_assert(sizeof(WeightDesc) == 48, "descriptor layout is part of the C ABI (alignn_prepare_weights)");

__global__ void zero_floats_kernel(float* __restrict__ p, int n) {
    const int i = blockIdx.x * blockDim.x + threadIdx.x;
    if (i < n) p[i] = 0.0f;
}

__global__ __launch_bounds__(256) void absmax_batched_kernel(const WeightDesc* __restrict__ descs) {
    const WeightDesc d = descs[blockIdx.y];
    const int Q = d.K >> 2;
    const int64_t total = (int64_t)d.N * Q;
    float m = 0.0f;
    for (int64_t i = (int64_t)blockIdx.x * 256 + threadIdx.x; i < total; i += (int64_t)gridDim.x * 256) {
        const int64_t r = i / Q;
        const int q = (int)(i - r * Q);
        const float4 v = f4_ld(d.W + r * d.ldw + q * 4);
        m = fmaxf(m, fmaxf(fmaxf(fabsf(v.x), fabsf(v.y)), fmaxf(fabsf(v.z), fabsf(v.w))));
    }
    block_amax_commit(m, d.amax);
}

__global__ __launch_bounds__(256) void split_f16x2_both_batched_kernel(const WeightDesc* __restrict__ descs) {
    const WeightDesc d = descs[blockIdx.y];
    const float sw = f16_scale(*d.amax);
// ... 109 lines not shown
    static bool attr_set = false;
    if (!attr_set) {
        const void* fns[] = {(const void*)gemm_nt_f16p_kernel<false>,        (const void*)gemm_nt_f16p_kernel<true>,
                             (const void*)gemm_nt_f16p_bnred_kernel<false>,  (const void*)gemm_nt_f16p_bnred_kernel<true>,
                             (const void*)gemm_nt_f16p_gather_kernel<false>, (const void*)gemm_nt_f16p_gather_kernel<true>,
                             (const void*)gemm_nt_f16p_stats_kernel};
        for (const void* fn : fns) {
            hipError_t e = hipFuncSetAttribute(fn, hipFuncAttributeMaxDynamicSharedMemorySize, lds);
            if (e != hipSuccess) return (int)e;
        }
        attr_set = true;
    }
    if (g_in.ldc >= (1 << 20) || g_in.ldadd >= (1 << 20) || g_in.ldxn >= (1 << 20)) return (int)hipErrorInvalidValue;
    X6Args g = g_in;
    g.xcd_map = 1;
    const int64_t tiles = alignn_ceil_div(g.M, 128) * (int64_t)(g.Npad / BN);
    constexpr int resident = kResidentP;
    const dim3 grid((unsigned)(tiles < resident ? tiles : resident)), block(NT);
    if (g.gp != nullptr) {
        if (g.red_partial)
            hipLaunchKernelGGL(gemm_nt_f16p_gather_kernel<true>, grid, block, lds, st, g);
        else
            hipLaunchKernelGGL(gemm_nt_f16p_gather_kernel<false>, grid, block, lds, st, g);
    } else if (g.red_partial != nullptr && g.xn == nullptr) {
        if (g.addend) return (int)hipErrorInvalidValue;
        hipLaunchKernelGGL(gemm_nt_f16p_stats_kernel, grid, block, lds, st, g);
    } else if (g.red_partial != nullptr) {
        if (g.addend)
            hipLaunchKernelGGL(gemm_nt_f16p_bnred_kernel<true>, grid, block, lds, st, g);
        else
            hipLaunchKernelGGL(gemm_nt_f16p_bnred_kernel<false>, grid, block, lds, st, g);
    } else if (g.addend) {
        hipLaunchKernelGGL(gemm_nt_f16p_kernel<true>, grid, block, lds, st, g);
    } else {
        hipLaunchKernelGGL(gemm_nt_f16p_kernel<false>, grid, block, lds, st, g);
    }
    ALIGNN_CHECK_LAUNCH();
    return 0;
}
inline int64_t rm1_below() { return 256; }
inline int nt_block_rows(int64_t M, int N, int K) {
    if (nt_persistent(M, N, K)) return 64;
    const int64_t tiles128 = alignn_ceil_div(M, 128) * (int64_t)(npad(N) / BN);
    return (K <= 64 || tiles128 < rm1_below()) ? 64 : 128;
}
template <bool F16>
int launch_nt(const X6Args& g, hipStream_t st) {
    const int64_t tiles128 = alignn_ceil_div(g.M, 128) * (int64_t)(g.Npad / BN);
    if constexpr (F16)
        if (nt_persistent(g.M, g.N, g.K)) {
            if (g.addend == nullptr) return launch_nt_p(g, st);
            X6Args gs = g;
            gs.strip_slabs = 1;
            return launch_nt_rm<F16, 2>(gs, st);
        }
    if (g.K <= 64 || tiles128 < rm1_below()) return launch_nt_rm<F16, 1>(g, st);
    return launch_nt_rm<F16, 2>(g, st);
}
inline bool nt_args_ok(const float* A, int64_t lda, const void* Wsplit, const float* bias, const float* addend,
                       int64_t ldadd, float* C, int64_t ldc) {
    return !((lda & 3) || (ldc & 3) || !aligned16(A) || !aligned16(C) || !aligned16(Wsplit) || (bias && !aligned16(bias)) ||
             (addend && ((ldadd & 3) || !aligned16(addend))));
}
}

extern "C" {

size_t alignn_split_bf16x3_bytes(int N, int K) { return (size_t)3 * npad(N) * (size_t)K * 2; }

int alignn_split_bf16x3(const float* W, int64_t ldw, int N, int K, int transpose, void* out, alignn_stream_t stream) {
    if (N <= 0 || K <= 0 || (K % BK) != 0 || out == nullptr) return (int)hipErrorInvalidValue;
    const int64_t total = (int64_t)npad(N) * K;
    int grid = (int)((total + 255) / 256);
    if (grid > 2048) grid = 2048;
    hipLaunchKernelGGL(split_bf16x3_kernel, dim3(grid), dim3(256), 0, (hipStream_t)stream, W, ldw, N, npad(N), K,
                       transpose, (unsigned short*)out);
    ALIGNN_CHECK_LAUNCH();
    return 0;
}

size_t alignn_split_f16x2_bytes(int N, int K) { return (size_t)2 * npad(N) * (size_t)K * 2; }

int alignn_split_f16x2(const float* W, int64_t ldw, int N, int K, int transpose, const float* w_amax, void* out,
                       alignn_stream_t stream) {
    if (N <= 0 || K <= 0 || (K % BK) != 0 || out == nullptr || w_amax == nullptr) return (int)hipErrorInvalidValue;
    const int64_t total = (int64_t)npad(N) * K;
    int grid = (int)((total + 255) / 256);
    if (grid > 2048) grid = 2048;
    hipLaunchKernelGGL(split_f16x2_kernel, dim3(grid), dim3(256), 0, (hipStream_t)stream, W, ldw, N, npad(N), K,
                       transpose, w_amax, (_Float16*)out);
    ALIGNN_CHECK_LAUNCH();
    return 0;
}

int alignn_split_f16x2_both(const float* W, int64_t ldw, int N, int K, const float* w_amax, void* out, void* out_t,
                            alignn_stream_t stream) {
    if (N <= 0 || K <= 0 || (K % BK) != 0 || (N % BK) != 0 || out == nullptr || out_t == nullptr || w_amax == nullptr ||
        (int64_t)npad(N) * K > ((int64_t)1 << 28) || (int64_t)npad(K) * N > ((int64_t)1 << 28))
        return (int)hipErrorInvalidValue;
    const int64_t total = (int64_t)npad(N) * K > (int64_t)npad(K) * N ? (int64_t)npad(N) * K : (int64_t)npad(K) * N;
    int grid = (int)((total + 255) / 256);
    if (grid > 2048) grid = 2048;
    hipLaunchKernelGGL(split_f16x2_both_kernel, dim3(grid), dim3(256), 0, (hipStream_t)stream, W, ldw, N, K, w_amax,
                       (_Float16*)out, (_Float16*)out_t);
    ALIGNN_CHECK_LAUNCH();
    return 0;
}

int alignn_prepare_weights(const void* descs, int n_weights, float* amax_slots, alignn_stream_t stream) {
    if (n_weights == 0) return 0;
    if (descs == nullptr || n_weights < 0 || amax_slots == nullptr) return (int)hipErrorInvalidValue;
    hipLaunchKernelGGL(zero_floats_kernel, dim3(alignn_ceil_div(n_weights, 256)), dim3(256), 0, (hipStream_t)stream, amax_slots,
                       n_weights);
    hipLaunchKernelGGL(absmax_batched_kernel, dim3(32, n_weights), dim3(256), 0, (hipStream_t)stream, (const WeightDesc*)descs);
    hipLaunchKernelGGL(split_f16x2_both_batched_kernel, dim3(256, n_weights), dim3(256), 0, (hipStream_t)stream,
                       (const WeightDesc*)descs);
    ALIGNN_CHECK_LAUNCH();
    return 0;
}

int alignn_absmax_raise(const float* X, int64_t ldx, int64_t rows, int F, float* amax, alignn_stream_t stream) {
    if (F <= 0 || (F & 3) || (ldx & 3) || rows < 0 || amax == nullptr || !aligned16(X)) return (int)hipErrorInvalidValue;
    if (rows == 0) return 0;
    int64_t blocks = (rows * (F >> 2) + 256 * 8 - 1) / (256 * 8);
    if (blocks > 4096) blocks = 4096;
    if (blocks < 1) blocks = 1;
    hipLaunchKernelGGL(absmax_kernel, dim3((int)blocks), dim3(256), 0, (hipStream_t)stream, X, ldx, rows, F, amax);
    ALIGNN_CHECK_LAUNCH();
    return 0;
}

int alignn_absmax(const float* X, int64_t ldx, int64_t rows, int F, float* amax, alignn_stream_t stream) {
    if (F <= 0 || (F & 3) || (ldx & 3) || rows < 0 || amax == nullptr || !aligned16(X)) return (int)hipErrorInvalidValue;
    hipLaunchKernelGGL(zero_floats_kernel, dim3(1), dim3(64), 0, (hipStream_t)stream, amax, 1);
    if (rows == 0) return 0;
    int64_t blocks = (rows * (F >> 2) + 256 * 8 - 1) / (256 * 8);
    if (blocks > 4096) blocks = 4096;
    if (blocks < 1) blocks = 1;
    hipLaunchKernelGGL(absmax_kernel, dim3((int)blocks), dim3(256), 0, (hipStream_t)stream, X, ldx, rows, F, amax);
    ALIGNN_CHECK_LAUNCH();
    return 0;
}

int alignn_gemm_tn_x6_supported(int64_t M, int N, int K) {
    return (M >= 4096 && N % tn::TBN == 0 && K % tn::TBK == 0) ? 1 : 0;
}

size_t alignn_gemm_tn_x6_workspace(int64_t M, int N, int K) {
    return (size_t)tn::tn_splits(M, N, K) * (size_t)N * (size_t)K * sizeof(float);
}

int alignn_gemm_tn_x6_splits(int64_t M, int N, int K) { return tn::tn_splits(M, N, K); }

int alignn_gemm_tn_x6_partials(const float* G, int64_t ldg, const float* g_amax, const float* X, int64_t ldx,
                               const float* x_amax, int64_t M, int N, int K, void* workspace, size_t workspace_bytes,
                               alignn_stream_t stream) {
    if (!alignn_gemm_tn_x6_supported(M, N, K)) return (int)hipErrorInvalidValue;
    if ((ldg & 3) || (ldx & 3) || !aligned16(G) || !aligned16(X) || !aligned16(workspace) ||
        workspace_bytes < alignn_gemm_tn_x6_workspace(M, N, K))
        return (int)hipErrorInvalidValue;
    if ((g_amax == nullptr) != (x_amax == nullptr)) return (int)hipErrorInvalidValue;
    tn::TnArgs g{G, ldg, X, ldx, (float*)workspace, M, N, K, tn::tn_chunk(M, N, K), N / tn::TBN, K / tn::TBK,
                 tn::tn_splits(M, N, K), g_amax, x_amax};
    static bool tn_attr = false;
    if (!tn_attr) {
        hipError_t e = hipFuncSetAttribute((const void*)tn::gemm_tn_x6_kernel<false>,
                                           hipFuncAttributeMaxDynamicSharedMemorySize, tn::TSch<false>::LDS);
        if (e == hipSuccess)
            e = hipFuncSetAttribute((const void*)tn::gemm_tn_x6_kernel<true>, hipFuncAttributeMaxDynamicSharedMemorySize,
                                    tn::TSch<true>::LDS);
        if (e != hipSuccess) return (int)e;
        tn_attr = true;
    }
    const int tiles = g.tiles_n * g.tiles_k;
    const int per_xcd = alignn_ceil_div(g.splits, 8) * tiles;
    if (g_amax)
        hipLaunchKernelGGL(tn::gemm_tn_x6_kernel<true>, dim3(per_xcd * 8), dim3(tn::TNT), tn::TSch<true>::LDS, (hipStream_t)stream, g);
    else
        hipLaunchKernelGGL(tn::gemm_tn_x6_kernel<false>, dim3(per_xcd * 8), dim3(tn::TNT), tn::TSch<false>::LDS, (hipStream_t)stream, g);
    ALIGNN_CHECK_LAUNCH();
    return 0;
}

int alignn_gemm_nt_x6_supported(int64_t M, int N, int K) { return (M > 0 && N >= 128 && N % 4 == 0 && K > 0 && K % BK == 0) ? 1 : 0; }

int alignn_gemm_nt_x6(const float* A, int64_t lda, const void* Wsplit, const float* bias, const float* addend,
                      int64_t ldadd, float* C, int64_t ldc, int64_t M, int N, int K, alignn_stream_t stream) {
    if (!alignn_gemm_nt_x6_supported(M, N, K)) return (int)hipErrorInvalidValue;
    if (!nt_args_ok(A, lda, Wsplit, bias, addend, ldadd, C, ldc)) return (int)hipErrorInvalidValue;
    X6Args g{A, lda, (const unsigned char*)Wsplit, nullptr, nullptr, bias, addend, ldadd, C, ldc, M, N, npad(N), K,
             exceeds_llc(M, N), nullptr, 0, nullptr, nullptr, nullptr, 0, nullptr, nullptr};
    return launch_nt<false>(g, (hipStream_t)stream);
}

int alignn_gemm_nt_f16x3(const float* A, int64_t lda, const float* a_amax, const void* Wsplit, const float* w_amax,
                         const float* bias, const float* addend, int64_t ldadd, float* C, int64_t ldc, int64_t M, int N,
                         int K, alignn_stream_t stream) {
    if (!alignn_gemm_nt_x6_supported(M, N, K) || a_amax == nullptr || w_amax == nullptr) return (int)hipErrorInvalidValue;
    if (!nt_args_ok(A, lda, Wsplit, bias, addend, ldadd, C, ldc)) return (int)hipErrorInvalidValue;
    X6Args g{A, lda, (const unsigned char*)Wsplit, a_amax, w_amax, bias, addend, ldadd, C, ldc, M, N, npad(N), K,
             exceeds_llc(M, N), nullptr, 0, nullptr, nullptr, nullptr, 0, nullptr, nullptr};
    return launch_nt<true>(g, (hipStream_t)stream);
}

int alignn_gemm_nt_f16x3_gather(const float* A, int64_t lda, const float* a_amax, const void* Wsplit, const float* w_amax,
                                const float* bias, float* C, int64_t ldc, int64_t M, int N, int K, const float* P, int64_t ldp,
                                const int32_t* src, const int32_t* dst, float* stats_partial, alignn_stream_t stream) {
    if (!alignn_gemm_nt_x6_supported(M, N, K) || a_amax == nullptr || w_amax == nullptr) return (int)hipErrorInvalidValue;
    if (!nt_args_ok(A, lda, Wsplit, bias, nullptr, 0, C, ldc)) return (int)hipErrorInvalidValue;
    if (P == nullptr || src == nullptr || dst == nullptr || (ldp & 3) || !aligned16(P) || (N & 3) || ldp < 2 * (int64_t)N ||
        (stats_partial && !aligned16(stats_partial)))
        return (int)hipErrorInvalidValue;
    X6Args g{A, lda, (const unsigned char*)Wsplit, a_amax, w_amax, bias, nullptr, 0, C, ldc, M, N, npad(N), K,
             exceeds_llc(M, N), nullptr, 0, nullptr, stats_partial, P, ldp, src, dst};
    return launch_nt<true>(g, (hipStream_t)stream);
}

int alignn_gemm_nt_f16x3_gather2(const float* A, int64_t lda, const float* a_amax, const void* Wsplit, const float* w_amax,
                                 const float* bias, float* C, int64_t ldc, int64_t M, int N, int K, const float* P, int64_t ldp,
                                 const int32_t* src, const float* Bd2, int64_t ldbd2, const int32_t* rank,
                                 float* stats_partial, alignn_stream_t stream) {
    if (!alignn_gemm_nt_x6_supported(M, N, K) || a_amax == nullptr || w_amax == nullptr) return (int)hipErrorInvalidValue;
    if (!nt_args_ok(A, lda, Wsplit, bias, nullptr, 0, C, ldc)) return (int)hipErrorInvalidValue;
    if (P == nullptr || src == nullptr || Bd2 == nullptr || rank == nullptr || (ldp & 3) || (ldbd2 & 3) || !aligned16(P) || !aligned16(Bd2) ||
        (N & 3) || ldp < (int64_t)N || ldbd2 < (int64_t)N || (stats_partial && !aligned16(stats_partial)))
        return (int)hipErrorInvalidValue;
    X6Args g{A, lda, (const unsigned char*)Wsplit, a_amax, w_amax, bias, nullptr, 0, C, ldc, M, N, npad(N), K,
             exceeds_llc(M, N), nullptr, 0, nullptr, stats_partial, P, ldp, src, rank};
    g.gp2 = Bd2;
    g.ldgp2 = ldbd2;
    return launch_nt<true>(g, (hipStream_t)stream);
}

int alignn_gemm_nt_f16x3_stats(const float* A, int64_t lda, const float* a_amax, const void* Wsplit, const float* w_amax,
                               const float* bias, float* C, int64_t ldc, int64_t M, int N, int K, float* stats_partial,
                               alignn_stream_t stream) {
    if (!alignn_gemm_nt_x6_supported(M, N, K) || a_amax == nullptr || w_amax == nullptr) return (int)hipErrorInvalidValue;
    if (!nt_args_ok(A, lda, Wsplit, bias, nullptr, 0, C, ldc)) return (int)hipErrorInvalidValue;
    if (stats_partial == nullptr || !aligned16(stats_partial) || (N & 3)) return (int)hipErrorInvalidValue;
    X6Args g{A, lda, (const unsigned char*)Wsplit, a_amax, w_amax, bias, nullptr, 0, C, ldc, M, N, npad(N), K,
             exceeds_llc(M, N), nullptr, 0, nullptr, stats_partial, nullptr, 0, nullptr, nullptr};
    return launch_nt<true>(g, (hipStream_t)stream);
}

int alignn_gemm_nt_x6_row_tiles(int64_t M, int N, int K) { return alignn_ceil_div(M, nt_block_rows(M, N, K)); }

int alignn_gemm_nt_f16x3_bnred(const float* A, int64_t lda, const float* a_amax, const void* Wsplit, const float* w_amax,
                               const float* bias, const float* addend, int64_t ldadd, float* C, int64_t ldc, int64_t M,
                               int N, int K, const float* Xn, int64_t ldxn, const float* nstat, float* red_partial,
                               alignn_stream_t stream) {
    if (!alignn_gemm_nt_x6_supported(M, N, K) || a_amax == nullptr || w_amax == nullptr) return (int)hipErrorInvalidValue;
    if (!nt_args_ok(A, lda, Wsplit, bias, addend, ldadd, C, ldc)) return (int)hipErrorInvalidValue;
    if (Xn == nullptr || nstat == nullptr || red_partial == nullptr || (ldxn & 3) || !aligned16(Xn) || !aligned16(nstat) ||
        !aligned16(red_partial))
        return (int)hipErrorInvalidValue;
    X6Args g{A, lda, (const unsigned char*)Wsplit, a_amax, w_amax, bias, addend, ldadd, C, ldc, M, N, npad(N), K,
             exceeds_llc(M, N), Xn, ldxn, nstat, red_partial, nullptr, 0, nullptr, nullptr};
    return launch_nt<true>(g, (hipStream_t)stream);
}

}
```

### alignn_amd/csrc/model.hip

```cpp
#include <atomic>
#include <chrono>
#include <cstdio>
#include <cstdlib>
#include <vector>

#include "../../include/alignn_hip.h"
#include "common.h"

namespace {

constexpr int kEvents = 512;
constexpr int kAmaxSlots = 1024;

struct EventPool {
    hipEvent_t ev[kEvents];
    int next = 0;
    bool ok = false;
};
EventPool g_pool[kMaxDevices];

__global__ void fill_kernel(float* __restrict__ p, int64_t n, float v) {
    const int64_t i = (int64_t)blockIdx.x * blockDim.x + threadIdx.x;
    if (i < n) p[i] = v;
}
__global__ void bump_kernel(int64_t* const* __restrict__ ptrs, int n) {
    const int i = blockIdx.x * blockDim.x + threadIdx.x;
    if (i < n) ptrs[i][0] += 1;
}
__global__ __launch_bounds__(256) void transpose_kernel(const float* __restrict__ in, int64_t ld, int rows, int cols,
                                                        float* __restrict__ out) {
    __shared__ float tile[32][33];
    const int tx = threadIdx.x & 31, ty = threadIdx.x >> 5;
    const int r0 = blockIdx.y * 32, c0 = blockIdx.x * 32;
    for (int j = ty; j < 32; j += 8)
        if (r0 + j < rows && c0 + tx < cols) tile[j][tx] = in[(int64_t)(r0 + j) * ld + c0 + tx];
    __syncthreads();
    for (int j = ty; j < 32; j += 8)
        if (c0 + j < cols && r0 + tx < rows) out[(int64_t)(c0 + j) * rows + r0 + tx] = tile[tx][j];
}

struct Ready {
    hipStream_t st = nullptr;
    hipEvent_t ev = nullptr;
    int at = 0;
};
struct Act {
    float* p = nullptr;
    float* amax = nullptr;
    float* xn = nullptr;
    float* stat = nullptr;
    float* red = nullptr;
    Ready rdy;
};
struct Grad {
    float* p = nullptr;
    Ready rdy;
    bool pre_red = false;
};

struct MlpTape {
    const alignn_mlp_params* p = nullptr;
    Act x, y;
    float *pre = nullptr, *stat = nullptr;
    int64_t rows = 0;
    bool lane = false;
};
struct ConvTape {
    const alignn_conv_params* p = nullptr;
    const alignn_graph_csr* g = nullptr;
    Act x, y, x_out, y_out;
    float *P = nullptr, *M = nullptr, *xpre = nullptr, *s0 = nullptr, *hh = nullptr, *n_stat = nullptr, *e_stat = nullptr;
    bool lane = false, need_y = true;
};
struct Tape {
    float *bl = nullptr, *rbf_e = nullptr, *rbf_a = nullptr, *pool = nullptr;
    float *hcos_buf = nullptr, *pred = nullptr, *seed = nullptr, *g_r = nullptr;
    const float* hcos = nullptr;
    bool angle_fused = false, angle_lane = false;
    float *a_stat1 = nullptr, *a_stat2 = nullptr, *a_scal = nullptr;
    MlpTape atom, e1, e2, a1, a2;
    std::vector<ConvTape> convs;
};

std::atomic<int64_t> g_dbg_aux_marks{0}, g_dbg_late_waits{0}, g_dbg_max_dist{0};
std::vector<std::pair<size_t, size_t>> g_dbg_allocs;
bool dbg_allocs_on() {
    static int on = -1;
    if (on < 0) on = getenv("ALIGNN_AMD_DEBUG_ALLOCS") ? 1 : 0;
    return on == 1;
}

struct Ctx {
    const alignn_model_desc* d;
    const alignn_model_batch* b;
    char* base;
    size_t off = 0, cap = 0;
    bool launch = false;
    bool unsupported = false;
    int unsupported_line = 0;
    int rc = 0;
    hipStream_t main = nullptr, T = nullptr, side = nullptr, aux = nullptr;
    float* amax_arena = nullptr;
    int amax_next = 0;
    EventPool* pool = nullptr;

    float* alloc(size_t floats) {
        const size_t bytes = al256(floats * sizeof(float));
        float* p = reinterpret_cast<float*>(base + off);
        if (launch && dbg_allocs_on()) g_dbg_allocs.emplace_back(off, bytes);
        off += bytes;
        if (launch && off > cap && rc == 0) rc = (int)hipErrorInvalidValue;
        return p;
    }
    size_t sbase[4] = {0, 0, 0, 0}, scur[4] = {0, 0, 0, 0}, speak[4] = {0, 0, 0, 0};
    int which(hipStream_t st) const { return st == main ? 0 : st == T ? 1 : st == side ? 2 : 3; }
    void tmp_reset(hipStream_t st) { scur[which(st)] = 0; }
    float* tmp(hipStream_t st, size_t floats) {
        const int i = which(st);
        const size_t bytes = al256(floats * sizeof(float));
        float* p = reinterpret_cast<float*>(base + sbase[i] + scur[i]);
        scur[i] += bytes;
        if (scur[i] > speak[i]) speak[i] = scur[i];
        if (launch && sbase[i] + scur[i] > cap && rc == 0) rc = (int)hipErrorInvalidValue;
        return p;
    }
    float* new_amax() {
        if (amax_next >= kAmaxSlots) {
            if (rc == 0) rc = (int)hipErrorInvalidValue;
            return amax_arena;
        }
        return amax_arena + amax_next++;
    }
    float* new_amax2() {
        if (amax_next + 2 > kAmaxSlots) {
            if (rc == 0) rc = (int)hipErrorInvalidValue;
            return amax_arena;
        }
        amax_next += 2;
        return amax_arena + amax_next - 2;
    }
    bool track(int64_t rows) const { return rows >= d->amax_min_rows; }
    const alignn_ff_desc* ff = nullptr;
    bool param_grads = true;
    bool geom = false;
    float *g_rbf_e = nullptr, *g_rbf_a = nullptr;
    bool g_rbf_a_on_T = false;
    ptrdiff_t toff = 0;
    float* sink = nullptr;
    int64_t sink_floats = 0;
    ptrdiff_t sink_toff = 0;
    float* twin(float* dW) const { return dW + ((sink != nullptr && dW >= sink && dW < sink + sink_floats) ? sink_toff : toff); }
    int n_sync = 0, n_launch = 0;
    double t_sync = 0.0;
    bool timing = false;
    void sync(hipStream_t waiter, hipStream_t src) {
        if (!launch || rc != 0 || waiter == src) return;
        const auto t0 = timing ? std::chrono::steady_clock::now() : std::chrono::steady_clock::time_point();
        wait(waiter, mark(src));
        ++n_sync;
// ... 285 lines not shown

void run_forward(Ctx& c, Tape& tp, float* out) {
    const alignn_model_desc& d = *c.d;
    const alignn_model_batch& b = *c.b;
    const int64_t N = b.g.n, E = b.g.m, Tn = b.lg.m;
    const int H = d.H;
    c.amax_arena = c.alloc(kAmaxSlots);
    c.amax_next = 0;
    fill(c, c.amax_arena, kAmaxSlots, 0.0f, c.main);
    const bool angle_first = c.ff == nullptr && d.norm == 0 && d.angle_fused != 0 && Tn > 0 && c.T != c.main && Tn >= d.lane_min_rows &&
                             alignn_angle_embed_supported(d.angle_bins, d.angle1.out, d.angle2.out) != 0;
    if (angle_first) c.sync(c.T, c.main);
    const bool prep_aside = angle_first && c.aux != c.main && d.n_weights > 0 && c.ff == nullptr &&
                            !x6_shape_ok(c, N, d.atom.in, d.atom.out, d.atom.in) &&
                            !x6_shape_ok(c, E, d.edge1.in, d.edge1.out, d.edge1.in);
    hipStream_t prep_st = prep_aside ? c.aux : c.main;
    if (prep_aside) c.sync(c.aux, c.main);
    if (d.n_weights > 0) L(alignn_prepare_weights(d.weight_descs, d.n_weights, d.weight_amax, prep_st));
    if (d.n_bump > 0 && c.launch && c.rc == 0) {
        hipLaunchKernelGGL(bump_kernel, dim3((d.n_bump + 63) / 64), dim3(64), 0, c.main, (int64_t* const*)d.bump_ptrs, d.n_bump);
        c.rc = (int)hipGetLastError();
    }
    tp.hcos = b.h;
    if (c.ff != nullptr && c.ff->lg_on_fly) {
        tp.hcos_buf = c.alloc((size_t)Tn);
        L(alignn_bond_cosine_fwd(b.r, b.lg.src, b.lg.dst, tp.hcos_buf, Tn, c.main));
        tp.hcos = tp.hcos_buf;
    }
    if (!angle_first) c.sync(c.T, c.main);
    Act z;
    tp.angle_fused = d.norm == 0 && d.angle_fused != 0 && Tn > 0 &&
                     alignn_angle_embed_supported(d.angle_bins, d.angle1.out, d.angle2.out) != 0;
    if (tp.angle_fused) {
        tp.angle_lane = c.T != c.main && Tn >= d.lane_min_rows;
        hipStream_t st = tp.angle_lane ? c.T : c.main;
        tp.a_stat1 = c.alloc((size_t)4 * d.angle1.out);
        tp.a_stat2 = c.alloc((size_t)4 * d.angle2.out);
        tp.a_scal = c.alloc((size_t)alignn_angle_embed_scal_floats());
        alignn_angle_args a = angle_args(c, tp);
        z.p = c.alloc((size_t)Tn * H);
        z.amax = c.track(Tn) ? c.new_amax() : nullptr;
        z.rdy = c.by(st);
        a.z = z.p;
        a.z_amax = z.amax;
        a.workspace_bytes = alignn_angle_embed_workspace(Tn, d.angle_bins, 0);
        a.workspace = c.alloc(a.workspace_bytes / sizeof(float));
        L(alignn_angle_embed_fwd(&a, st));
    } else {
        tp.rbf_a = c.alloc((size_t)Tn * d.angle_bins);
        L(alignn_rbf_fwd(tp.hcos, d.angle_centers, d.angle_gamma, tp.rbf_a, Tn, d.angle_bins, c.main));
        Act za;
        za.p = tp.rbf_a;
        z = mlp_fwd(c, tp.a2, d.angle2, mlp_fwd(c, tp.a1, d.angle1, za, Tn), Tn);
    }
    Act xa;
    xa.p = const_cast<float*>(b.atom_features);
    Act x = mlp_fwd(c, tp.atom, d.atom, xa, N);
    tp.bl = c.alloc((size_t)E);
    L(alignn_norm3_fwd(b.r, tp.bl, E, c.main));
    tp.rbf_e = c.alloc((size_t)E * d.edge_bins);
    L(alignn_rbf_fwd(tp.bl, d.edge_centers, d.edge_gamma, tp.rbf_e, E, d.edge_bins, c.main));
    Act ye;
    ye.p = tp.rbf_e;
    Act y1 = mlp_fwd(c, tp.e1, d.edge1, ye, E);
    if (prep_aside) c.sync(c.main, c.aux);
    Act y = mlp_fwd(c, tp.e2, d.edge2, y1, E);
    if (c.unsupported) return;
    tp.convs.assign(conv_count(d), ConvTape{});
    int k = 0;
    for (int i = 0; i < d.alignn_layers; ++i) {
        ConvTape& tg = tp.convs[k];
        conv_fwd(c, tg, d.convs[k], b.g, x, y, true);
        ++k;
        ConvTape& tl = tp.convs[k];
        conv_fwd(c, tl, d.convs[k], b.lg, tg.y_out, z, i + 1 < d.alignn_layers);
        ++k;
        x = tg.x_out;
        y = tl.x_out;
        z = tl.y_out;
        if (c.unsupported) return;
    }
    for (int i = 0; i < d.gcn_layers; ++i) {
        ConvTape& tg = tp.convs[k];
        conv_fwd(c, tg, d.convs[k], b.g, x, y, i + 1 < d.gcn_layers);
        ++k;
        x = tg.x_out;
        y = tg.y_out;
        if (c.unsupported) return;
    }
    c.need(c.main, x.rdy);
    tp.pool = c.alloc((size_t)b.B * H);
    L(alignn_segment_mean_fwd(x.p, b.graph_ptr, tp.pool, b.B, H, c.main));
    L(alignn_gemm_nt(tp.pool, H, d.fc_W, H, d.fc_b, nullptr, 0, out, d.out_features, b.B, d.out_features, H, c.main));
    c.sync(c.main, c.T);
}


void transpose(Ctx& c, const float* w, int64_t ld, int rows, int cols, float* out, hipStream_t st) {
    if (!c.launch || c.rc != 0) return;
    hipLaunchKernelGGL(transpose_kernel, dim3((cols + 31) / 32, (rows + 31) / 32), dim3(256), 0, st, w, ld, rows, cols, out);
    c.rc = (int)hipGetLastError();
}

void dgrad(Ctx& c, const float* g, int64_t ldg, const float* g_amax, const float* w, int Nred, int Kout, const void* img_t,
           const float* w_amax, const float* addend, int64_t ldadd, float* out, int64_t M, hipStream_t st, const Act* src,
           bool* pre_red) {
    if (pre_red) *pre_red = false;
    const bool x6 = x6_shape_ok(c, M, ldg, Kout, Nred);
    if (x6) {
        if (g_amax == nullptr || img_t == nullptr) {
            UNSUP();
            return;
        }
        if (src != nullptr && src->xn != nullptr) {
            const int tiles = alignn_gemm_nt_x6_row_tiles(M, Kout, Nred);
            float* part = c.alloc((size_t)(tiles + 1) * 2 * Kout);
            L(alignn_gemm_nt_f16x3_bnred(g, ldg, g_amax, img_t, w_amax, nullptr, addend, ldadd, out, Kout, M, Kout, Nred, src->xn,
                                         Kout, src->stat, part, st));
            bn_bwd_finalize_folded(c, part, tiles, Kout, src->red, st);
            if (pre_red) *pre_red = true;
            return;
        }
        L(alignn_gemm_nt_f16x3(g, ldg, g_amax, img_t, w_amax, nullptr, addend, ldadd, out, Kout, M, Kout, Nred, st));
        return;
    }
    const size_t sb = alignn_gemm_nn_split_workspace(M, Nred, Kout);
    if (sb) {
        if ((ldg % 4) == 0 && (Kout % 4) == 0 && (addend == nullptr || (ldadd % 4) == 0)) {
            c.tmp_reset(st);
            float* ws = c.tmp(st, sb / 4);
            L(alignn_gemm_nn_split(g, ldg, w, Kout, addend, ldadd, out, Kout, M, Nred, Kout, ws, sb, st));
        } else
            L(alignn_gemm_nn(g, ldg, w, Kout, addend, ldadd, out, Kout, M, Nred, Kout, st));
        return;
    }
    if ((Nred % 4) == 0 && Kout >= 16) {
        c.tmp_reset(st);
        float* wt = c.tmp(st, (size_t)Kout * Nred);
        transpose(c, w, Kout, Nred, Kout, wt, st);
        L(alignn_gemm_nt(g, ldg, wt, Nred, nullptr, addend, ldadd, out, Kout, M, Kout, Nred, st));
        return;
    }
    L(alignn_gemm_nn(g, ldg, w, Kout, addend, ldadd, out, Kout, M, Nred, Kout, st));
}

void gemm_tn(Ctx& c, const float* g, int64_t ldg, const float* g_amax, const float* a, int64_t lda, const float* a_amax,
             float* dW, int64_t M, int N, int K, hipStream_t st) {
    if (g_amax == nullptr || a_amax == nullptr) g_amax = a_amax = nullptr;
    const size_t nb = alignn_gemm_tn_workspace(M, N, K);
    float* ws = c.tmp(st, nb / 4 + 1);
    L(alignn_gemm_tn(g, ldg, g_amax, a, lda, a_amax, dW, K, M, N, K, ws, nb, st));
}

void col_sum(Ctx& c, const float* x, int64_t ldx, int64_t rows, int F, float* out, hipStream_t st) {
    float* ws = c.tmp(st, (size_t)alignn_col_stats_slabs(rows) * 2 * F);
    L(alignn_col_sum(x, ldx, rows, F, out, ws, st));
}

hipStream_t side_for(Ctx& c, int64_t rows) { return (c.side != c.main && rows >= c.d->side_min_rows) ? c.side : c.main; }

float* edge_grad_buffer(Ctx& c, const ConvTape& t, int64_t m, int Kin) {
    if (c.d->reuse_tape && c.ff == nullptr && t.M != nullptr && Kin == c.d->H) return t.M;
    return c.alloc((size_t)m * Kin);
}

bool dgrad_wgrad(Ctx& c, const ConvTape& t, const float* GM, const float* gm_amax, const float* gy, float* g_y, int64_t m, int H,
                 int Kin, hipStream_t st, const Act* src, bool* pre_red) {
    const alignn_conv_params& p = *t.p;
    if (c.d->dw_fused <= 0 || m < c.d->dw_fused || !c.param_grads || gm_amax == nullptr || t.y.amax == nullptr || p.weg_img_t == nullptr || Kin != H ||
        !alignn_gemm_dgrad_wgrad_supported(m, H, Kin) || !x6_shape_ok(c, m, H, Kin, H))
        return false;
    const size_t nb = alignn_gemm_dgrad_wgrad_workspace(m);
    c.tmp_reset(st);
    float* ws = c.tmp(st, nb / 4);
    const int slabs = 2 * alignn_gemm_dgrad_wgrad_slabs(m);
    float* part = src != nullptr ? c.alloc((size_t)slabs * 2 * Kin) : nullptr;
    L(alignn_gemm_dgrad_wgrad_f16x3(GM, H, gm_amax, t.y.p, Kin, t.y.amax, p.weg_img_t, p.weg_amax, gy, H, g_y, Kin,
                                    src != nullptr ? src->xn : nullptr, Kin, src != nullptr ? src->stat : nullptr, part, p.g_weg, Kin, m,
                                    ws, nb, st));
    if (src != nullptr) bn_bwd_finalize_folded(c, part, slabs, Kin, src->red, st);
    if (pre_red) *pre_red = src != nullptr;
    return true;
}

Grad mlp_bwd(Ctx& c, const MlpTape& t, const Grad& gy, bool need_gx) {
    const bool ln = c.d->norm == 1;
    const alignn_mlp_params& p = *t.p;
    const int F = p.out, K = p.in;
    const int64_t rows = t.rows;
    hipStream_t st = t.lane ? c.T : c.main;
    c.need(st, gy.rdy);
    float* gpre = c.alloc((size_t)rows * F);
    float* g_amax = c.track(rows) ? c.new_amax() : nullptr;
    const int slabs = ln ? alignn_ln_slabs(rows) : alignn_col_stats_slabs(rows);
    float* gb_part = nullptr;
    if (ln) {
        float* part = c.alloc((size_t)slabs * 2 * F);
        L(alignn_ln_silu_bwd(gy.p, F, t.pre, F, p.gamma, p.beta, t.stat, gpre, F, part, rows, F, g_amax, st));
        if (c.param_grads) L(alignn_bn_bwd_finalize(part, slabs, F, p.red, st));
    } else {
        if (!gy.pre_red) {
            float* part = c.alloc((size_t)slabs * 2 * F);
            L(alignn_bn_silu_bwd_reduce(gy.p, F, t.pre, F, t.stat, rows, F, part, st));
            L(alignn_bn_bwd_finalize(part, slabs, F, p.red, st));
        }
        if (F <= 1024) {
            gb_part = c.alloc((size_t)slabs * F);
            L(alignn_bn_silu_bwd_apply_sum(gy.p, F, t.pre, F, t.stat, p.red, 0, gpre, F, rows, F, g_amax, gb_part, st));
        } else
            L(alignn_bn_silu_bwd_apply(gy.p, F, t.pre, F, t.stat, p.gamma, p.red, 0, gpre, F, rows, F, g_amax, st));
    }
    Grad gx;
    if (need_gx) {
        gx.p = c.alloc((size_t)rows * K);
        gx.rdy = c.by(st);
        const Act* src = (t.x.xn != nullptr && g_amax != nullptr) ? &t.x : nullptr;
        dgrad(c, gpre, F, g_amax, p.W, F, K, p.img_t, p.w_amax, nullptr, 0, gx.p, rows, st, src, &gx.pre_red);
    }
    if (!c.param_grads) return gx;
    hipStream_t sd = side_for(c, rows);
    if (sd != st) {
        c.sync(sd, c.main);
        if (t.lane) c.sync(sd, c.T);
    }
    c.tmp_reset(sd);
    gemm_tn(c, gpre, F, g_amax, t.x.p, K, t.x.amax, p.gW, rows, F, K, sd);
    if (gb_part != nullptr)
        L(alignn_slab_sum(gb_part, slabs, F, p.gb, sd));
    else
        col_sum(c, gpre, F, rows, F, p.gb, sd);
    return gx;
}

struct NodeBranch {
    float *GP = nullptr, *gp_amax = nullptr, *gm_amax = nullptr, *gs1 = nullptr, *gs0 = nullptr;
    Ready rdy;
};
NodeBranch conv_bwd_node(Ctx& c, const ConvTape& t, const Grad& gx_out) {
    const bool ln = c.d->norm == 1;
    const alignn_conv_params& p = *t.p;
    const int H = c.d->H;
    const int64_t n = t.g->n, m = t.g->m;
    hipStream_t st = (!t.lane && c.aux != c.main && c.where(gx_out.rdy) == c.aux) ? c.aux : c.main;
    c.need(st, gx_out.rdy);
    NodeBranch nb;
    nb.GP = c.alloc((size_t)n * 4 * H);
    nb.gp_amax = c.track(n) ? c.new_amax() : nullptr;
    nb.gm_amax = c.track(m) ? c.new_amax() : nullptr;
    float* g_xpre = nb.GP + 3 * (size_t)H;
    const int n_slabs = ln ? alignn_ln_slabs(n) : alignn_col_stats_slabs(n);
    float* n_part = c.alloc((size_t)n_slabs * 2 * H);
    nb.gs1 = c.alloc((size_t)n * H);
    nb.gs0 = c.alloc((size_t)n * H);
    if (ln) {
        L(alignn_ln_silu_bwd_node(gx_out.p, H, t.xpre, H, p.n_gamma, p.n_beta, t.n_stat, g_xpre, 4 * H, n_part, n, H, nb.gp_amax, t.s0,
                                  t.hh, nb.gs1, nb.gs0, st));
        if (c.param_grads) L(alignn_bn_bwd_finalize(n_part, n_slabs, H, p.n_red, st));
    } else {
        L(alignn_bn_silu_bwd_reduce(gx_out.p, H, t.xpre, H, t.n_stat, n, H, n_part, st));
        L(alignn_bn_bwd_finalize(n_part, n_slabs, H, p.n_red, st));
        L(alignn_bn_silu_bwd_apply_node(gx_out.p, H, t.xpre, H, t.n_stat, p.n_gamma, p.n_red, 0, g_xpre, 4 * H, n, H, nb.gp_amax, t.s0,
                                        t.hh, nb.gs1, nb.gs0, st));
    }
    nb.rdy = c.marked(st);
    return nb;
}

void conv_bwd(Ctx& c, const ConvTape& t, const NodeBranch& nb, const Grad& gx_out, const Grad* gy_out, Grad& g_x, Grad& g_y,
              bool need_gx = true) {
    const bool ln = c.d->norm == 1;
    const alignn_conv_params& p = *t.p;
    const alignn_graph_csr& g = *t.g;
    const int H = c.d->H, Kin = H;
    const int64_t n = g.n, m = g.m;
    hipStream_t main = c.main, T = t.lane ? c.T : c.main;
    float *GP = nb.GP, *gp_amax = nb.gp_amax, *gm_amax = nb.gm_amax, *gs1 = nb.gs1, *gs0 = nb.gs0;
    if (!t.lane && gy_out != nullptr) c.need(main, gy_out->rdy);
    const float* gy = gy_out != nullptr ? gy_out->p : nullptr;
    if (t.lane && gy_out != nullptr) c.need(T, gy_out->rdy);
    const bool lg_blocks = g.grp_seg_ptr != nullptr;
    const bool dense = lg_blocks && g.dense_max_src > 0 && alignn_egc_bwd_lg_dense_supported(g.dense_max_src);
    const bool ln_inside = ln && gy != nullptr && dense && alignn_egc_ln_fused_supported(H, m);
    const bool ln_dst = ln && gy != nullptr && !lg_blocks && alignn_egc_ln_dst_supported(H);
    const float *ge = gy, *e_stat = t.e_stat, *e_red = nullptr;
    if (ln) {
        ge = e_stat = nullptr;
        if (gy != nullptr && !ln_inside && !ln_dst) {
            float* g_branch = c.alloc((size_t)m * H);
            const int e_slabs = alignn_ln_slabs(m);
            float* e_part = c.alloc((size_t)e_slabs * 2 * H);
            L(alignn_ln_silu_bwd(gy, H, t.M, H, p.e_gamma, p.e_beta, t.e_stat, g_branch, H, e_part, m, H, nullptr, T));
            if (c.param_grads) L(alignn_bn_bwd_finalize(e_part, e_slabs, H, p.e_red, T));
            ge = g_branch;
        }
    } else if (gy != nullptr) {
        if (!gy_out->pre_red) {
            const int e_slabs = alignn_col_stats_slabs(m);
            float* e_part = c.alloc((size_t)e_slabs * 2 * H);
            L(alignn_bn_silu_bwd_reduce(gy, H, t.M, H, t.e_stat, m, H, e_part, T));
            L(alignn_bn_bwd_finalize(e_part, e_slabs, H, p.e_red, T));
        }
        e_red = p.e_red;
    }
    c.need(main, nb.rdy);
    if (t.lane) c.sync(T, main);
    float* GM = c.alloc((size_t)m * H);
    const int gslabs = lg_blocks ? (int)g.n_groups : (ln_dst ? alignn_egc_ln_dst_slabs(n) : alignn_egc_slabs(n));
    float* gb_part = c.alloc((size_t)gslabs * H);
    float* e_part = (ln_inside || ln_dst) ? c.alloc((size_t)gslabs * 2 * H) : nullptr;
    if (ln_inside)
        L(alignn_egc_bwd_lg_dense_ln(gy, t.M, t.P, gs1, gs0, p.e_gamma, p.e_beta, t.e_stat, m, g.grp_seg_ptr, g.grp_src_ptr, g.n_groups,
                                     g.dense_max_src, g.seg_ptr, g.seg_node, H, GM, GP, gb_part, e_part, gm_amax, gp_amax, T));
    else if (dense)
        L(alignn_egc_bwd_lg_dense(ge, t.M, t.P, gs1, gs0, e_stat, e_red, 0, m, g.grp_seg_ptr, g.grp_src_ptr, g.n_groups,
                                  g.dense_max_src, g.seg_ptr, g.seg_node, H, GM, GP, gb_part, gm_amax, gp_amax, T));
    else if (lg_blocks)
        L(alignn_egc_bwd_lg_fused(ge, t.M, t.P, gs1, gs0, e_stat, e_red, 0, m, g.grp_seg_ptr, g.grp_src_ptr, g.n_groups,
                                  g.seg_ptr, g.seg_node, g.dst, g.out_ptr, g.out_slot, H, GM, GP, gb_part, gm_amax, gp_amax, T));
    else if (ln_dst)
        L(alignn_egc_bwd_dst_ln(gy, t.M, t.P, gs1, gs0, p.e_gamma, p.e_beta, t.e_stat, g.seg_ptr, g.seg_node, g.src, n, H, GM, GP, gb_part,
                                e_part, gm_amax, gp_amax, T));
    else
        L(alignn_egc_bwd_dst(ge, t.M, t.P, gs1, gs0, e_stat, p.e_gamma, e_red, 0, m, g.seg_ptr, g.seg_node, g.src, n, H, GM, GP,
                             gb_part, gm_amax, gp_amax, T));
    if (e_part != nullptr && c.param_grads) L(alignn_bn_bwd_finalize(e_part, gslabs, H, p.e_red, T));
    if (!lg_blocks) L(alignn_egc_bwd_src(GM, t.M, gs1, g.out_ptr, g.out_slot, g.dst, n, H, GP, gp_amax, T));
    if (t.lane) c.sync(main, T);
    g_y.p = edge_grad_buffer(c, t, m, Kin);
    hipStream_t sx = main;
    if (need_gx) {
        g_x.p = c.alloc((size_t)n * Kin);
        if (!t.lane && c.aux != main) {
            c.sync(c.aux, main);
            sx = c.aux;
        }
        c.need(sx, gx_out.rdy);
        dgrad(c, GP, 4 * H, gp_amax, p.wcat, 4 * H, Kin, p.wcat_img_t, p.wcat_amax, gx_out.p, H, g_x.p, n, sx, nullptr, nullptr);
    }
    const Act* src = (t.y.xn != nullptr && gm_amax != nullptr) ? &t.y : nullptr;
    const bool dw = dgrad_wgrad(c, t, GM, gm_amax, gy, g_y.p, m, H, Kin, T, src, &g_y.pre_red);
    if (!dw) dgrad(c, GM, H, gm_amax, p.w_eg, H, Kin, p.weg_img_t, p.weg_amax, gy, H, g_y.p, m, T, src, &g_y.pre_red);
    g_y.rdy = c.by(T);
    if (need_gx) g_x.rdy = c.marked(sx);
    if (!c.param_grads) return;
    hipStream_t sd = side_for(c, m);
    if (sd != main) {
        c.sync(sd, main);
        if (t.lane) c.sync(sd, c.T);
    } else if (t.lane)
        c.sync(main, c.T);
    c.tmp_reset(sd);
    L(alignn_slab_sum(gb_part, gslabs, H, p.g_beg, sd));
    if (!dw) gemm_tn(c, GM, H, gm_amax, t.y.p, Kin, t.y.amax, p.g_weg, m, H, Kin, sd);
    gemm_tn(c, GP, 4 * H, gp_amax, t.x.p, Kin, t.x.amax, p.g_wcat, n, 4 * H, Kin, sd);
    col_sum(c, GP, 4 * H, n, 4 * H, p.g_bcat, sd);
}

void run_backward(Ctx& c, const Tape& tp, const float* g_out) {
    const alignn_model_desc& d = *c.d;
    const alignn_model_batch& b = *c.b;
    const int64_t N = b.g.n;
    const int H = d.H, OF = d.out_features, B = b.B;
    c.amax_arena = c.alloc(kAmaxSlots);
    c.amax_next = 0;
    fill(c, c.amax_arena, kAmaxSlots, 0.0f, c.main);
    c.sync(c.T, c.main);
    c.sync(c.side, c.main);
    float* g_pool = c.alloc((size_t)B * H);
    dgrad(c, g_out, OF, nullptr, d.fc_W, OF, H, nullptr, nullptr, nullptr, 0, g_pool, B, c.main, nullptr, nullptr);
    if (c.param_grads) {
        c.tmp_reset(c.main);
        gemm_tn(c, g_out, OF, nullptr, tp.pool, H, nullptr, d.g_fc_W, B, OF, H, c.main);
        if ((OF % 4) == 0)
            col_sum(c, g_out, OF, B, OF, d.g_fc_b, c.main);
        else {
            float* ones = c.alloc((size_t)B);
            fill(c, ones, B, 1.0f, c.main);
            gemm_tn(c, g_out, OF, nullptr, ones, 1, nullptr, d.g_fc_b, B, OF, 1, c.main);
        }
    }
    Grad gx;
    gx.p = c.alloc((size_t)N * H);
    L(alignn_segment_mean_bwd(g_pool, b.graph_ptr, gx.p, B, H, c.main));
    int k = conv_count(d) - 1;
    Grad gy, gz;
    bool have_gy = false, have_gz = false;
    for (int i = d.gcn_layers - 1; i >= 0; --i, --k) {
        Grad nx, ny;
        const NodeBranch nb = conv_bwd_node(c, tp.convs[k], gx);
        conv_bwd(c, tp.convs[k], nb, gx, have_gy ? &gy : nullptr, nx, ny);
        gx = nx;
        gy = ny;
        have_gy = true;
        if (c.unsupported) return;
    }
    const bool angle_geom = c.geom && c.ff != nullptr && c.ff->lg_on_fly;
    for (int i = d.alignn_layers - 1; i >= 0; --i) {
        const NodeBranch nb_g = conv_bwd_node(c, tp.convs[k - 1], gx);
        Grad gm, nz;
        const NodeBranch nb_lg = conv_bwd_node(c, tp.convs[k], gy);
        conv_bwd(c, tp.convs[k], nb_lg, gy, have_gz ? &gz : nullptr, gm, nz);
        --k;
        gz = nz;
        have_gz = true;
        if (i == 0) {
            if (tp.angle_fused) {
                hipStream_t st = tp.angle_lane ? c.T : c.main;
                c.need(st, gz.rdy);
                alignn_angle_args a = angle_args(c, tp);
                a.gz = gz.p;
                a.workspace_bytes = alignn_angle_embed_workspace(a.rows, d.angle_bins, 1);
                a.workspace = c.alloc(a.workspace_bytes / sizeof(float));
                L(alignn_angle_embed_bwd(&a, st));
            } else if (c.param_grads || angle_geom) {
                Grad ga = mlp_bwd(c, tp.a2, gz, true);
                Grad gr = mlp_bwd(c, tp.a1, ga, angle_geom);
                c.g_rbf_a = gr.p;
                c.g_rbf_a_on_T = c.where(gr.rdy) != c.main;
            }
        }
        Grad nx, ny;
        conv_bwd(c, tp.convs[k], nb_g, gx, &gm, nx, ny, i > 0 || c.param_grads);
        --k;
        gx = nx;
        gy = ny;
        if (c.unsupported) return;
    }
    if (c.param_grads) mlp_bwd(c, tp.atom, gx, false);
    Grad ge = mlp_bwd(c, tp.e2, gy, true);
    Grad gre = mlp_bwd(c, tp.e1, ge, c.geom);
    c.g_rbf_e = gre.p;
    c.join_aux();
    c.sync(c.main, c.T);
    c.sync(c.main, c.side);
}

Act mlp_infer(Ctx& c, const alignn_mlp_params& p, const Act& x, int64_t rows) {
    const int F = p.out, K = p.in;
    const bool lane = c.T != c.main && rows >= c.d->lane_min_rows;
    hipStream_t st = lane ? c.T : c.main;
    c.need(st, x.rdy);
    float* pre = c.alloc((size_t)rows * F);
    float* stat = c.alloc((size_t)4 * F);
    project(c, x.p, K, x.amax, p.W, K, p.img, p.w_amax, p.b, pre, F, rows, F, K, st);
    L(alignn_bn_finalize(nullptr, 0, rows, F, p.gamma, p.beta, c.d->eps, c.d->momentum, p.rm, p.rv, stat, st));
    Act y;
    y.p = c.alloc((size_t)rows * F);
    y.amax = c.track(rows) ? c.new_amax() : nullptr;
    L(alignn_bn_silu_fwd(pre, F, nullptr, 0, stat, y.p, F, rows, F, y.amax, st));
    y.rdy = c.by(st);
    return y;
}

void conv_infer(Ctx& c, const alignn_conv_params& p, const alignn_graph_csr& g, const Act& x, const Act& y, bool need_y,
                Act& x_out, Act& y_out) {
    const int H = c.d->H, Kin = H;
    const int64_t n = g.n, m = g.m;
    const bool lane = c.T != c.main && m >= c.d->lane_min_rows;
    hipStream_t main = c.main, T = lane ? c.T : c.main;
    c.need(main, x.rdy);
    if (!lane) c.need(main, y.rdy);
    float* P = c.alloc((size_t)n * 4 * H);
    project(c, x.p, Kin, x.amax, p.wcat, Kin, p.wcat_img, p.wcat_amax, p.bcat, P, 4 * H, n, 4 * H, Kin, main);
    float* stats = c.alloc((size_t)8 * H);
    L(alignn_bn_finalize(nullptr, 0, n, H, p.n_gamma, p.n_beta, c.d->eps, c.d->momentum, p.n_rm, p.n_rv, stats, main));
    L(alignn_bn_finalize(nullptr, 0, m, H, p.e_gamma, p.e_beta, c.d->eps, c.d->momentum, p.e_rm, p.e_rv, stats + 4 * H, main));
    if (lane) c.sync(T, main);
    float* Cm = c.alloc((size_t)m * H);
    project(c, y.p, Kin, y.amax, p.w_eg, Kin, p.weg_img, p.weg_amax, p.b_eg, Cm, H, m, H, Kin, T);
    float* xpre = c.alloc((size_t)n * H);
    Act yo;
    if (need_y) {
        yo.p = c.alloc((size_t)m * H);
        yo.amax = c.track(m) ? c.new_amax() : nullptr;
        yo.rdy = c.by(T);
    }
    L(alignn_egc_gate_infer(P, Cm, g.seg_ptr, g.seg_node, g.src, n, m, H, xpre, stats + 4 * H, y.p, yo.p, yo.amax, T));
    if (lane) c.sync(main, T);
    x_out = Act{};
    x_out.p = c.alloc((size_t)n * H);
    x_out.amax = c.track(n) ? c.new_amax() : nullptr;
    L(alignn_bn_silu_fwd(xpre, H, x.p, Kin, stats, x_out.p, H, n, H, x_out.amax, main));
    y_out = yo;
}

void run_infer(Ctx& c, float* out) {
    const alignn_model_desc& d = *c.d;
    const alignn_model_batch& b = *c.b;
    const int64_t N = b.g.n, E = b.g.m, Tn = b.lg.m;
    c.amax_arena = c.alloc(kAmaxSlots);
    c.amax_next = 0;
    fill(c, c.amax_arena, kAmaxSlots, 0.0f, c.main);
    if (d.n_weights > 0) L(alignn_prepare_weights(d.weight_descs, d.n_weights, d.weight_amax, c.main));
    c.sync(c.T, c.main);
    Act z;
    if (d.angle_fused != 0 && Tn > 0 && alignn_angle_embed_supported(d.angle_bins, d.angle1.out, d.angle2.out) != 0) {
        const bool lane = c.T != c.main && Tn >= d.lane_min_rows;
        Tape tp;
        tp.hcos = b.h;
        tp.a_stat1 = c.alloc((size_t)4 * d.angle1.out);
        tp.a_stat2 = c.alloc((size_t)4 * d.angle2.out);
        tp.a_scal = c.alloc((size_t)alignn_angle_embed_scal_floats());
        alignn_angle_args a = angle_args(c, tp);
        z.p = c.alloc((size_t)Tn * d.H);
        z.amax = c.track(Tn) ? c.new_amax() : nullptr;
        z.rdy = c.by(lane ? c.T : c.main);
        a.z = z.p;
        a.z_amax = z.amax;
// ... 711 lines not shown
```

### alignn_amd/ops.py

```python

from __future__ import annotations

import ctypes
import weakref

import torch

from . import _lib
from ._lib import check, ptr, require_f32, stream
from .graph import CSRGraph

BN_EPS = 1e-5
BN_MOMENTUM = 0.1
FUSED_LG_BACKWARD = True
INFER_FUSED = True
DENSE_LG_BACKWARD = True


_PARAM_GRADS = {"on": True}


class no_param_grad:
    def __enter__(self):
        self.prev = _PARAM_GRADS["on"]
# ... 634 lines not shown
    N = ws.n
    if K != ws.k:
        raise ValueError(f"reduction length mismatch: {K} vs {ws.k}")
    if out is None:
        out = _empty(M, N, like=a)
    check(
        lib.alignn_gemm_nt_x6(ptr(a), a.stride(0), ptr(ws.buf), ptr(bias), ptr(addend),
                              addend.stride(0) if addend is not None else 0, ptr(out), out.stride(0), M, N, K, stream()),
        "gemm_nt_x6",
    )
    return out


NN_SPLIT = True


def project(a, w, bias=None, addend=None, transpose_w=False, a_amax=None):
    lib = _lib.load()
    M = a.shape[0]
    N, K = (w.shape[1], w.shape[0]) if transpose_w else (w.shape[0], w.shape[1])
    x6_tiles = ((M + 63) // 64) * ((N + 255) // 256)
    if x6_tiles >= X6_MIN_TILES and a.stride(0) % 4 == 0 and lib.alignn_gemm_nt_x6_supported(M, N, K):
        if a_amax is None:
            a_amax = get_amax(a)
        if F16X3 and a_amax is not None:
            return gemm_nt_f16x3(a, a_amax, split_f16x2(w, transpose_w), bias, addend)
        if F16X3:
            REGISTRY_STATS["bf16x6_fallback"] += 1
            _warn_once("bf16x6", f"alignn_amd: a [{M},{K}] x [{K},{N}] projection runs the six-product bf16 scheme because max|a| "
                                 "of its input is unknown (the tensor did not come from a kernel that tracks it, or was cloned / "
                                 "edited in between): correct, but ~1.6x slower than the three-product fp16 scheme")
        return gemm_nt_x6(a, split_bf16x3(w, transpose_w), bias, addend)
    if transpose_w:
        if NN_SPLIT and bias is None and lib.alignn_gemm_nn_split_workspace(M, w.shape[0], w.shape[1]):
            return gemm_nn(a, w, addend)
        if w.shape[0] % 4 == 0 and w.shape[1] >= 16:
            return gemm_nt(a, w.t().contiguous(), bias, addend)
        return gemm_nn(a, w, addend)
    return gemm_nt(a, w, bias, addend)


def gemm_nn(g, w, addend=None, out=None):
    lib = _lib.load()
    require_f32(g, w, addend)
    M, N = g.shape
    K = w.shape[1]
    if out is None:
        out = _empty(M, K, like=g)
    nbytes = lib.alignn_gemm_nn_split_workspace(M, N, K) if NN_SPLIT else 0
    if nbytes and g.stride(0) % 4 == 0 and w.stride(0) % 4 == 0 and (addend is None or addend.stride(0) % 4 == 0):
        ws = torch.empty(nbytes // 4, dtype=torch.float32, device=g.device)
        check(lib.alignn_gemm_nn_split(ptr(g), g.stride(0), ptr(w), w.stride(0), ptr(addend),
                                       addend.stride(0) if addend is not None else 0, ptr(out), out.stride(0), M, N, K,
                                       ptr(ws), nbytes, stream()), "gemm_nn_split")
        return out
    check(
        lib.alignn_gemm_nn(ptr(g), g.stride(0), ptr(w), w.stride(0), ptr(addend),
                           addend.stride(0) if addend is not None else 0, ptr(out), out.stride(0), M, N, K, stream()),
        "gemm_nn",
    )
    return out


def _dgrad(g, w, addend=None, g_amax=None):
    return project(g, w, None, addend, transpose_w=True, a_amax=g_amax)


BNRED_FUSED = True
BNRED_STATS = {"fused": 0, "used": 0}
_NORM_SRC = {}
_PRE_RED = {}


def _register_norm_src(y, xn, stat):
    if y is not None and BNRED_FUSED:
        k = id(y)
        _NORM_SRC[k] = (weakref.ref(y, lambda _r, k=k: _NORM_SRC.pop(k, None)), xn, stat)


def _norm_src_of(y):
    e = _NORM_SRC.get(id(y))
    hit = e is not None and e[0]() is y
    if BNRED_FUSED:
        REGISTRY_STATS["norm_src_hit" if hit else "norm_src_miss"] += 1
    return (e[1], e[2]) if hit else None


def _take_pre_red(gy, xn):
    if gy is None:
        return None
    e = _PRE_RED.pop(id(gy), None)
    if e is not None and e[0]() is gy and e[1] is xn:
        BNRED_STATS["used"] += 1
        REGISTRY_STATS["pre_red_hit"] += 1
        return e[2]
    REGISTRY_STATS["pre_red_miss"] += 1
    lost = _PRE_RED_ORPHANS.pop(id(xn), None) is not None
    for k, rec in list(_PRE_RED.items()):
        if rec[1] is xn:
            _PRE_RED.pop(k, None)
            lost = True
    if lost:
        REGISTRY_STATS["separate_bn_reduce"] += 1
        _warn_once("pre_red", "alignn_amd: BatchNorm-backward sums taken in a projection's epilogue were not picked up by the "
                              "layer they belong to (its incoming gradient is a different tensor object than the one the "
                              "projection wrote: hook / clone / checkpoint in between?) - reducing again in a separate pass")
    return None


_PRE_RED_ORPHANS = {}


def _orphan_pre_red(k):
    rec = _PRE_RED.pop(k, None)
    if rec is not None:
        xn = rec[1]
        kx = id(xn)
        _PRE_RED_ORPHANS[kx] = weakref.ref(xn, lambda _r, kx=kx: _PRE_RED_ORPHANS.pop(kx, None))


def _dgrad_bnred(g, w, addend, g_amax, src):
    lib = _lib.load()
    M, N, K = g.shape[0], w.shape[1], w.shape[0]
    ok = (src is not None and BNRED_FUSED and F16X3 and g_amax is not None and g.stride(0) % 4 == 0
          and ((M + 63) // 64) * ((N + 255) // 256) >= X6_MIN_TILES and lib.alignn_gemm_nt_x6_supported(M, N, K)
          and tuple(src[0].shape) == (M, N) and src[0].stride(0) % 4 == 0)
    if not ok:
        return _dgrad(g, w, addend, g_amax)
    out, red = gemm_nt_f16x3_bnred(g, g_amax, split_f16x2(w, True), src[0], src[1], None, addend)
    BNRED_STATS["fused"] += 1
    k = id(out)
    _PRE_RED[k] = (weakref.ref(out, lambda _r, k=k: _orphan_pre_red(k)), src[0], red)
    return out


def gemm_tn(g, a, g_amax=None, a_amax=None):
    if not F16X3 or g_amax is None or a_amax is None:
        g_amax = a_amax = None
    lib = _lib.load()
    require_f32(g, a)
    M, N = g.shape
    K = a.shape[1]
    out = _empty(N, K, like=g)
    nbytes = lib.alignn_gemm_tn_workspace(M, N, K)
    ws = torch.empty(max(nbytes // 4, 1), dtype=torch.float32, device=g.device)
    check(
        lib.alignn_gemm_tn(ptr(g), g.stride(0), ptr(g_amax), ptr(a), a.stride(0), ptr(a_amax), ptr(out), out.stride(0),
                           M, N, K, ptr(ws), nbytes, stream()),
        "gemm_tn",
    )
    return out


def col_sum(x):
    lib = _lib.load()
    rows, F = x.shape
    out = _empty(F, like=x)
    ws = _empty(lib.alignn_col_stats_slabs(rows) * 2 * F, like=x)
    check(lib.alignn_col_sum(ptr(x), x.stride(0), rows, F, ptr(out), ptr(ws), stream()), "col_sum")
    return out


FOLD_ABOVE = 1024


def _fold(partial, slabs, width):
    if slabs <= FOLD_ABOVE:
        return partial, slabs
    lib = _lib.load()
    g = lib.alignn_slab_fold_slabs()
    out = _empty(g, width, like=partial)
    check(lib.alignn_slab_fold(ptr(partial), slabs, width, ptr(out), stream()), "slab_fold")
    return out, g


def _welford_slabs(slabs, F, like):
    return _empty(slabs * (3 * F + 1), like=like)


def _bn_finalize(partial, slabs, rows, gamma, beta, running_mean, running_var, update_running, welford=False):
    lib = _lib.load()
    F = gamma.numel()
    stat = _empty(4, F, like=gamma)
    rm = running_mean if (update_running or slabs == 0) else None
    rv = running_var if (update_running or slabs == 0) else None
    if welford and slabs:
        check(lib.alignn_bn_finalize_welford(ptr(partial), slabs, rows, F, ptr(gamma), ptr(beta), BN_EPS, BN_MOMENTUM, ptr(rm),
                                             ptr(rv), ptr(stat), stream()), "bn_finalize_welford")
        return stat
    if slabs:
        partial, slabs = _fold(partial, slabs, 2 * F)
    check(
        lib.alignn_bn_finalize(ptr(partial), slabs, rows, F, ptr(gamma), ptr(beta), BN_EPS, BN_MOMENTUM, ptr(rm),
                               ptr(rv), ptr(stat), stream()),
        "bn_finalize",
    )
    return stat


def _bn_silu_fwd(x, res, stat):
    lib = _lib.load()
    rows, F = x.shape
    y = _empty(rows, F, like=x)
    amax = new_amax(x) if _track(rows) else None
    check(
        lib.alignn_bn_silu_fwd(ptr(x), x.stride(0), ptr(res), res.stride(0) if res is not None else 0, ptr(stat),
                               ptr(y), y.stride(0), rows, F, ptr(amax), stream()),
        "bn_silu_fwd",
    )
    return set_amax(y, amax) if amax is not None else y


def _bn_silu_bwd_reduce(gy, x, stat):
    lib = _lib.load()
    rows, F = x.shape
    slabs = lib.alignn_col_stats_slabs(rows)
    partial = _empty(slabs, 2, F, like=x)
    check(
        lib.alignn_bn_silu_bwd_reduce(ptr(gy), gy.stride(0), ptr(x), x.stride(0), ptr(stat), rows, F, ptr(partial),
                                      stream()),
        "bn_silu_bwd_reduce",
    )
    red = _empty(2, F, like=x)
    check(lib.alignn_bn_bwd_finalize(ptr(partial), slabs, F, ptr(red), stream()), "bn_bwd_finalize")
    return red


def _bn_silu_bwd_apply(gy, x, stat, gamma, red, eval_mode, out, amax=None):
    lib = _lib.load()
    rows, F = x.shape
    check(
        lib.alignn_bn_silu_bwd_apply(ptr(gy), gy.stride(0), ptr(x), x.stride(0), ptr(stat), ptr(gamma), ptr(red),
                                     int(eval_mode), ptr(out), out.stride(0), rows, F, ptr(amax), stream()),
        "bn_silu_bwd_apply",
    )
    return out


LN_EPS = 1e-5


def _ln_silu_fwd(x, res, gamma, beta, want_stats=True):
    lib = _lib.load()
    rows, F = x.shape
    y = _empty(rows, F, like=x)
    stats = _empty(rows, 2, like=x) if want_stats else None
    amax = new_amax(x) if _track(rows) else None
    check(
        lib.alignn_ln_silu_fwd(ptr(x), x.stride(0), ptr(res), res.stride(0) if res is not None else 0, ptr(gamma),
                               ptr(beta), LN_EPS, ptr(y), y.stride(0), ptr(stats), rows, F, ptr(amax), stream()),
        "ln_silu_fwd",
    )
    if amax is not None:
        set_amax(y, amax)
    return y, stats


def _ln_silu_bwd(gy, x, gamma, beta, stats, out, amax=None, node=None):
    lib = _lib.load()
    rows, F = x.shape
    slabs = lib.alignn_ln_slabs(rows)
    partial = _empty(slabs, 2, F, like=x)
    if node is not None:
        s0, hh, gs1, gs0 = node
        check(
            lib.alignn_ln_silu_bwd_node(ptr(gy), gy.stride(0), ptr(x), x.stride(0), ptr(gamma), ptr(beta), ptr(stats), ptr(out),
                                        out.stride(0), ptr(partial), rows, F, ptr(amax), ptr(s0), ptr(hh), ptr(gs1), ptr(gs0),
                                        stream()),
            "ln_silu_bwd_node",
        )
    else:
        check(
            lib.alignn_ln_silu_bwd(ptr(gy), gy.stride(0), ptr(x), x.stride(0), ptr(gamma), ptr(beta), ptr(stats), ptr(out),
                                   out.stride(0), ptr(partial), rows, F, ptr(amax), stream()),
            "ln_silu_bwd",
        )
    red = _empty(2, F, like=x)
    check(lib.alignn_bn_bwd_finalize(ptr(partial), slabs, F, ptr(red), stream()), "ln_bwd_finalize")
    return red


def _bond_cosines_raw(r, e1, e2):
    lib = _lib.load()
    require_f32(r)
    h = _empty(e1.numel(), like=r)
    check(lib.alignn_bond_cosine_fwd(ptr(r), ptr(e1), ptr(e2), ptr(h), e1.numel(), stream()), "bond_cosine_fwd")
    return h


def _segment_sum_raw(vals, seg_ptr, slot, node, n_out):
    lib = _lib.load()
    vals = vals.contiguous()
    out = _empty(n_out, vals.shape[1], like=vals)
    check(lib.alignn_segment_sum(ptr(vals), vals.stride(0), ptr(seg_ptr), ptr(slot), ptr(node), ptr(out), out.stride(0),
                                 seg_ptr.numel() - 1, vals.shape[1], stream()), "segment_sum")
    return out


class BondCosFn(torch.autograd.Function):

    @staticmethod
    def forward(ctx, r, lg):
        r = r.contiguous()
        ctx.save_for_backward(r)
        ctx.lg = lg
        return _bond_cosines_raw(r, lg.src, lg.dst)
# ... 16 lines not shown
    if isinstance(e1, CSRGraph):
        if r.requires_grad:
            return BondCosFn.apply(r, e1)
        return _bond_cosines_raw(r.contiguous(), e1.src, e1.dst)
    if r.requires_grad:
        raise NotImplementedError("pass the line graph itself (bond_cosines(r, lg)) to differentiate w.r.t. r")
    return _bond_cosines_raw(r.contiguous(), e1, e2)


class LinearFn(torch.autograd.Function):

    @staticmethod
    def forward(ctx, x, w, b):
        x = x.contiguous()
        w = w.contiguous()
        ctx.save_for_backward(x, w)
        ctx.has_bias = b is not None
        ctx.param_grads = _PARAM_GRADS["on"]
        return project(x, w, b)

    @staticmethod
    def backward(ctx, gy):
        x, w = ctx.saved_tensors
        gy = gy.contiguous()
        gx = _dgrad(gy, w) if ctx.needs_input_grad[0] else None
        gw = gemm_tn(gy, x) if (ctx.needs_input_grad[1] and ctx.param_grads) else None
        gb = None
        if ctx.has_bias and ctx.needs_input_grad[2] and ctx.param_grads:
            if gy.shape[1] % 4 == 0:
                gb = col_sum(gy)
            else:
                ones = torch.ones(gy.shape[0], 1, dtype=torch.float32, device=gy.device)
                gb = gemm_tn(gy, ones).reshape(-1)
        return gx, gw, gb


def linear(x, w, b=None):
    return LinearFn.apply(x, w, b)


APPLY_SUM = True


class MLPLayerFn(torch.autograd.Function):

    @staticmethod
    def _fwd(ctx, x, w, b, gamma, beta, running_mean, running_var, training, norm):
        lib = _lib.load()
        ctx.x_amax = get_amax(x)
        fused_stats = (norm == "batch" and training and STATS_FUSED
                       and _f16x3_applies(x, ctx.x_amax, w.shape[0], w.shape[1]))
        if fused_stats:
            pre, partial, slabs = gemm_nt_f16x3_stats(x, ctx.x_amax, split_f16x2(w), b)
        else:
            pre = project(x, w, b, a_amax=ctx.x_amax)
        rows, F = pre.shape
        if norm == "layer":
            y, stat = _ln_silu_fwd(pre, None, gamma, beta)
        else:
            if training:
                if not fused_stats:
                    slabs = lib.alignn_col_stats_slabs(rows)
                    partial = _welford_slabs(slabs, F, pre)
                    check(lib.alignn_col_stats_welford(ptr(pre), pre.stride(0), rows, F, ptr(partial), stream()), "col_stats")
                stat = _bn_finalize(partial, slabs, rows, gamma, beta, running_mean, running_var, True, welford=not fused_stats)
            else:
                stat = _bn_finalize(None, 0, rows, gamma, beta, running_mean, running_var, False)
            y = _bn_silu_fwd(pre, None, stat)
            _register_norm_src(y, pre, stat)
        return y, pre, stat

    @staticmethod
    def forward(ctx, x, w, b, gamma, beta, running_mean, running_var, training, norm="batch"):
        x = x.contiguous()
        w = w.contiguous()
        lane = _lane_for(x.shape[0])
        ctx.lane = lane is not None
        ctx.x_on_T = _is_on_T(x)
        ctx.x_src = _norm_src_of(x)
        if lane is not None:
            with _on_T(*lane, reads=(x,)):
                y, pre, stat = MLPLayerFn._fwd(ctx, x, w, b, gamma, beta, running_mean, running_var, training, norm)
            _mark_on_T(y)
        else:
            _main_reads(x)
            y, pre, stat = MLPLayerFn._fwd(ctx, x, w, b, gamma, beta, running_mean, running_var, training, norm)
        ctx.save_for_backward(x, w, pre, stat, gamma, beta)
        ctx.training = training
        ctx.norm = norm
        ctx.param_grads = _PARAM_GRADS["on"]
        ctx.wb = (w, b)
        _note_forward(ctx.wb)
        if FORWARD_TAPE is not None and norm == "layer":
            FORWARD_TAPE[w.data_ptr()] = ("mlp", x, pre, y)
        return y

    @staticmethod
    def _bwd(ctx, gy, x, w, pre, stat, gamma, beta):
        gpre = torch.empty_like(pre)
        gb_part = None
        g_amax = new_amax(pre) if _track(pre.shape[0]) else None
        if ctx.norm == "layer":
            red = _ln_silu_bwd(gy, pre, gamma, beta, stat, gpre, g_amax)
        else:
            red = _take_pre_red(gy, pre)
            if red is None:
                red = _bn_silu_bwd_reduce(gy, pre, stat)
            if APPLY_SUM and getattr(ctx, "param_grads", False) and pre.shape[1] <= 1024:
                lib = _lib.load()
                rows, F = pre.shape
                slabs = lib.alignn_col_stats_slabs(rows)
                gb_part = _empty(slabs, F, like=pre)
                check(lib.alignn_bn_silu_bwd_apply_sum(ptr(gy), gy.stride(0), ptr(pre), pre.stride(0), ptr(stat), ptr(red),
                                                       int(not ctx.training), ptr(gpre), gpre.stride(0), rows, F, ptr(g_amax),
                                                       ptr(gb_part), stream()), "bn_silu_bwd_apply_sum")
                gb_part = (gb_part, slabs)
            else:
                _bn_silu_bwd_apply(gy, pre, stat, gamma, red, not ctx.training, gpre, g_amax)
        gx = _dgrad_bnred(gpre, w, None, g_amax, ctx.x_src) if ctx.needs_input_grad[0] else None
        return gpre, g_amax, red, gx, gb_part

    @staticmethod
    def backward(ctx, gy):
        x, w, pre, stat, gamma, beta = ctx.saved_tensors
        gy = gy.contiguous()
        ev = None
        if ctx.lane:
            main, T = _lane_streams(gy.device)
            with _on_T(main, T, reads=(gy,)):
                gpre, g_amax, red, gx, gb_part = MLPLayerFn._bwd(ctx, gy, x, w, pre, stat, gamma, beta)
            ev = _event_after(T)
            if (gx is None or ctx.x_on_T) and (not ctx.param_grads or _deferred_join_is_safe((gamma, beta))):
                _arm_backward_join()
                _mark_on_T(gx)
            else:
                main.wait_event(ev)
                for t in (gx, red):
                    if t is not None:
                        t.record_stream(main)
        else:
            _main_reads(gy)
            gpre, g_amax, red, gx, gb_part = MLPLayerFn._bwd(ctx, gy, x, w, pre, stat, gamma, beta)
        dbeta, dgamma = red[0], red[1]
        if not ctx.param_grads:
            return gx, None, None, None, None, None, None, None, None
        x_amax = ctx.x_amax
        def bias_grad():
            if gb_part is None:
                return col_sum(gpre)
            out = _empty(gpre.shape[1], like=gpre)
            check(_lib.load().alignn_slab_sum(ptr(gb_part[0]), gb_part[1], gpre.shape[1], ptr(out), stream()), "slab_sum")
            return out

        gw, gb = on_side_stream(lambda: (gemm_tn(gpre, x, g_amax, x_amax), bias_grad()),
                                [gpre, x, g_amax, x_amax, gb_part[0] if gb_part is not None else None], ctx.wb, wait=(ev,))
        return gx, gw, gb, dgamma, dbeta, None, None, None, None


ANGLE_FUSED = True


def angle_fused_applies(h, rbf, l1, l2, training) -> bool:
    if not training and (torch.is_grad_enabled() or not INFER_FUSED):
        return False
    if not (ANGLE_FUSED and h.is_cuda and h.dtype == torch.float32 and not h.requires_grad and h.dim() == 1
            and h.numel() > 0):
        return False
    lin1, bn1, lin2, bn2 = l1.layer[0], l1.layer[1], l2.layer[0], l2.layer[1]
    if not (isinstance(bn1, torch.nn.BatchNorm1d) and isinstance(bn2, torch.nn.BatchNorm1d)):
        return False
    for bn in (bn1, bn2):
        if bn.running_mean is None or bn.momentum is None or bn.weight is None or abs(bn.momentum - BN_MOMENTUM) > 0 or bn.eps != BN_EPS:
            return False
    for m in (rbf, l1, l2, lin1, bn1, lin2, bn2, l1.layer, l2.layer):
        if m._forward_hooks or m._forward_pre_hooks or m._backward_hooks:
            return False
    if lin1.weight.dtype != torch.float32 or lin1.bias is None or lin2.bias is None:
        return False
    return bool(_lib.load().alignn_angle_embed_supported(lin1.weight.shape[1], lin1.weight.shape[0], lin2.weight.shape[0])) and (
        lin1.weight.shape[1] == rbf.centers.numel() and lin2.weight.shape[1] == lin1.weight.shape[0])


def _angle_args(h, centers, gamma, p1, p2, bufs, stat1, stat2, scal):
    from .angle import AngleArgs
    from .cmodel import MlpParams

    a = AngleArgs()
    a.h, a.rows = ptr(h), h.numel()
    a.centers, a.gamma, a.bins = ptr(centers), float(gamma), centers.numel()
    for dst, (w, b, g, be), (rm, rv) in ((a.l1, p1, bufs[0]), (a.l2, p2, bufs[1])):
        dst.W, dst.b, dst.gamma, dst.beta, dst.rm, dst.rv = ptr(w), ptr(b), ptr(g), ptr(be), ptr(rm), ptr(rv)
        dst.in_, dst.out = w.shape[1], w.shape[0]
    a.eps, a.momentum = BN_EPS, BN_MOMENTUM
    a.stat1, a.stat2, a.scal = ptr(stat1), ptr(stat2), ptr(scal)
    return a


class AngleEmbedFn(torch.autograd.Function):

    @staticmethod
    def forward(ctx, h, centers, gamma, w1, b1, g1, be1, w2, b2, g2, be2, rm1, rv1, rm2, rv2):
        import ctypes as C

        lib = _lib.load()
        h = h.contiguous()
        T = h.numel()
        lane = _lane_for(T)
        ctx.lane = lane is not None

        def run():
            z = _empty(T, w2.shape[0], like=h)
            amax = new_amax(z) if _track(T) else None
            stat1, stat2, scal = _empty(4 * w1.shape[0], like=h), _empty(4 * w2.shape[0], like=h), _empty(lib.alignn_angle_embed_scal_floats(), like=h)
            a = _angle_args(h, centers, gamma, (w1, b1, g1, be1), (w2, b2, g2, be2), ((rm1, rv1), (rm2, rv2)), stat1, stat2, scal)
            nbytes = lib.alignn_angle_embed_workspace(T, centers.numel(), 0)
            ws = torch.empty(nbytes, dtype=torch.uint8, device=h.device)
            a.z, a.z_amax, a.workspace, a.workspace_bytes = ptr(z), ptr(amax), ptr(ws), nbytes
            check(lib.alignn_angle_embed_fwd(C.byref(a), stream()), "angle_embed_fwd")
            return z, amax, stat1, stat2, scal

        if lane is not None:
            with _on_T(*lane, reads=(h,)):
                z, amax, stat1, stat2, scal = run()
            _mark_on_T(z)
        else:
            z, amax, stat1, stat2, scal = run()
        if amax is not None:
            set_amax(z, amax)
        ctx.save_for_backward(h, centers, w1, b1, g1, be1, w2, b2, g2, be2, rm1, rv1, rm2, rv2, stat1, stat2, scal)
        ctx.gamma = gamma
        ctx.param_grads = _PARAM_GRADS["on"]
        return z

    @staticmethod
    def backward(ctx, gz):
        import ctypes as C

        lib = _lib.load()
        h, centers, w1, b1, g1, be1, w2, b2, g2, be2, rm1, rv1, rm2, rv2, stat1, stat2, scal = ctx.saved_tensors
        none = (None,) * 15
        if not ctx.param_grads:
            return none
        gz = gz.contiguous()
        T = h.numel()

        def run():
            out = [(_empty(*w.shape, like=w), _empty(w.shape[0], like=w), _empty(2, w.shape[0], like=w)) for w in (w1, w2)]
            a = _angle_args(h, centers, ctx.gamma, (w1, b1, g1, be1), (w2, b2, g2, be2), ((rm1, rv1), (rm2, rv2)), stat1, stat2, scal)
            for dst, (gw, gb, red) in ((a.l1, out[0]), (a.l2, out[1])):
                dst.gW, dst.gb, dst.red = ptr(gw), ptr(gb), ptr(red)
            nbytes = lib.alignn_angle_embed_workspace(T, centers.numel(), 1)
            ws = torch.empty(nbytes, dtype=torch.uint8, device=h.device)
            a.gz, a.workspace, a.workspace_bytes = ptr(gz), ptr(ws), nbytes
            check(lib.alignn_angle_embed_bwd(C.byref(a), stream()), "angle_embed_bwd")
            return out

        params = (w1, b1, g1, be1, w2, b2, g2, be2)
        if ctx.lane:
            main, T_ = _lane_streams(gz.device)
            with _on_T(main, T_, reads=(gz,)):
                out = run()
            ev = _event_after(T_)
            if _deferred_join_is_safe(params):
                _arm_backward_join()
            else:
                main.wait_event(ev)
                for grp in out:
                    for t in grp:
                        t.record_stream(main)
        else:
            _main_reads(gz)
            out = run()
        (gw1, gb1, red1), (gw2, gb2, red2) = out
        return (None, None, None, gw1, gb1, red1[1], red1[0], gw2, gb2, red2[1], red2[0], None, None, None, None)


def angle_embed_infer(h, rbf, l1, l2):
    import ctypes as C

    lib = _lib.load()
    lin1, bn1, lin2, bn2 = l1.layer[0], l1.layer[1], l2.layer[0], l2.layer[1]
    h = h.contiguous()
    T = h.numel()
    lane = _lane_for(T)

    def run():
        z = _empty(T, lin2.weight.shape[0], like=h)
        amax = new_amax(z) if _track(T) else None
        stat1, stat2, scal = _empty(4 * lin1.weight.shape[0], like=h), _empty(4 * lin2.weight.shape[0], like=h), _empty(lib.alignn_angle_embed_scal_floats(), like=h)
        a = _angle_args(h, rbf.centers, rbf.gamma, (lin1.weight, lin1.bias, bn1.weight, bn1.bias),
                        (lin2.weight, lin2.bias, bn2.weight, bn2.bias),
                        ((bn1.running_mean, bn1.running_var), (bn2.running_mean, bn2.running_var)), stat1, stat2, scal)
        a.z, a.z_amax = ptr(z), ptr(amax)
        check(lib.alignn_angle_embed_infer(C.byref(a), stream()), "angle_embed_infer")
        return z, amax

    if lane is not None:
        with _on_T(*lane, reads=(h,)):
            z, amax = run()
        _mark_on_T(z)
    else:
        z, amax = run()
    if amax is not None:
        set_amax(z, amax)
    return z


# ... 413 lines not shown
            n_red = _bn_silu_bwd_reduce(gx_out, xpre, n_stat)
        if not layer:
            check(lib.alignn_bn_silu_bwd_apply_node(ptr(gx_out), gx_out.stride(0), ptr(xpre), xpre.stride(0), ptr(n_stat),
                                                    ptr(n_gamma), ptr(n_red), int(ev), ptr(g_xpre), g_xpre.stride(0), n, H,
                                                    ptr(gp_amax), ptr(s0), ptr(hh), ptr(gs1), ptr(gs0), stream()),
                  "bn_silu_bwd_apply_node")
        if gy_out is not None:
            gy_out = gy_out.contiguous()
        lg_blocks = graph.grp_seg_ptr is not None and FUSED_LG_BACKWARD
        dense = lg_blocks and DENSE_LG_BACKWARD and lib.alignn_egc_bwd_lg_dense_supported(graph.dense_max_src)
        ln_inside = bool(layer and dense and gy_out is not None and lib.alignn_egc_ln_fused_supported(H, m))
        ln_dst = bool(layer and not lg_blocks and gy_out is not None and lib.alignn_egc_ln_dst_supported(H))
        fused_red = {}

        def edge_branch():
            e_red = None
            g_branch, e_stat_arg = gy_out, e_stat
            if gy_out is not None:
                if ln_inside or ln_dst:
                    pass
                elif layer:
                    g_branch = _empty(m, H, like=x)
                    e_red = _ln_silu_bwd(gy_out, M, e_gamma, e_beta, e_stat, g_branch)
                    e_stat_arg = None
                else:
                    e_red = _take_pre_red(gy_out, M)
                    if e_red is None:
                        e_red = _bn_silu_bwd_reduce(gy_out, M, e_stat)
            return e_red, g_branch, e_stat_arg

        def gate_backward(e_red, g_branch, e_stat_arg):
            GM = _empty(m, H, like=x)
            if ln_inside:
                gslabs = graph.grp_seg_ptr.numel() - 1
                gb_part = _empty(gslabs, H, like=x)
                ln_part = _empty(gslabs, 2, H, like=x)
                check(
                    lib.alignn_egc_bwd_lg_dense_ln(ptr(gy_out), ptr(M), ptr(P), ptr(gs1), ptr(gs0), ptr(e_gamma), ptr(e_beta),
                                                   ptr(e_stat), m, ptr(graph.grp_seg_ptr), ptr(graph.grp_src_ptr), gslabs,
                                                   graph.dense_max_src, ptr(graph.seg_ptr), ptr(graph.seg_node), H, ptr(GM),
                                                   ptr(GP), ptr(gb_part), ptr(ln_part), ptr(gm_amax), ptr(gp_amax), stream()),
                    "egc_bwd_lg_dense_ln",
                )
                red = _empty(2, H, like=x)
                check(lib.alignn_bn_bwd_finalize(ptr(ln_part), gslabs, H, ptr(red), stream()), "ln_finalize")
                fused_red["e"] = red
            elif dense:
                gslabs = graph.grp_seg_ptr.numel() - 1
                gb_part = _empty(gslabs, H, like=x)
                check(
                    lib.alignn_egc_bwd_lg_dense(ptr(g_branch), ptr(M), ptr(P), ptr(gs1), ptr(gs0), ptr(e_stat_arg),
                                                ptr(e_red), int(ev), m, ptr(graph.grp_seg_ptr), ptr(graph.grp_src_ptr),
                                                gslabs, graph.dense_max_src, ptr(graph.seg_ptr), ptr(graph.seg_node), H,
                                                ptr(GM), ptr(GP), ptr(gb_part), ptr(gm_amax), ptr(gp_amax), stream()),
                    "egc_bwd_lg_dense",
                )
            elif lg_blocks:
                gslabs = graph.grp_seg_ptr.numel() - 1
                gb_part = _empty(gslabs, H, like=x)
                check(
                    lib.alignn_egc_bwd_lg_fused(ptr(g_branch), ptr(M), ptr(P), ptr(gs1), ptr(gs0), ptr(e_stat_arg),
                                                ptr(e_red), int(ev), m, ptr(graph.grp_seg_ptr), ptr(graph.grp_src_ptr),
                                                gslabs, ptr(graph.seg_ptr), ptr(graph.seg_node), ptr(graph.dst),
                                                ptr(graph.out_ptr), ptr(graph.out_slot), H, ptr(GM), ptr(GP), ptr(gb_part),
                                                ptr(gm_amax), ptr(gp_amax), stream()),
                    "egc_bwd_lg_fused",
                )
            elif ln_dst:
                gslabs = lib.alignn_egc_ln_dst_slabs(n)
                gb_part = _empty(gslabs, H, like=x)
                ln_part = _empty(gslabs, 2, H, like=x)
                check(
                    lib.alignn_egc_bwd_dst_ln(ptr(gy_out), ptr(M), ptr(P), ptr(gs1), ptr(gs0), ptr(e_gamma), ptr(e_beta), ptr(e_stat),
                                              ptr(graph.seg_ptr), ptr(graph.seg_node), ptr(graph.src), n, H, ptr(GM), ptr(GP),
                                              ptr(gb_part), ptr(ln_part), ptr(gm_amax), ptr(gp_amax), stream()),
                    "egc_bwd_dst_ln",
                )
                red = _empty(2, H, like=x)
                check(lib.alignn_bn_bwd_finalize(ptr(ln_part), gslabs, H, ptr(red), stream()), "ln_finalize")
                fused_red["e"] = red
                check(
                    lib.alignn_egc_bwd_src(ptr(GM), ptr(M), ptr(gs1), ptr(graph.out_ptr), ptr(graph.out_slot),
                                           ptr(graph.dst), n, H, ptr(GP), ptr(gp_amax), stream()),
                    "egc_bwd_src",
                )
            else:
                gslabs = lib.alignn_egc_slabs(n)
                gb_part = _empty(gslabs, H, like=x)
                check(
                    lib.alignn_egc_bwd_dst(ptr(g_branch), ptr(M), ptr(P), ptr(gs1), ptr(gs0), ptr(e_stat_arg), ptr(e_gamma),
                                           ptr(e_red), int(ev), m, ptr(graph.seg_ptr), ptr(graph.seg_node), ptr(graph.src),
                                           n, H, ptr(GM), ptr(GP), ptr(gb_part), ptr(gm_amax), ptr(gp_amax), stream()),
                    "egc_bwd_dst",
                )
                check(
                    lib.alignn_egc_bwd_src(ptr(GM), ptr(M), ptr(gs1), ptr(graph.out_ptr), ptr(graph.out_slot),
                                           ptr(graph.dst), n, H, ptr(GP), ptr(gp_amax), stream()),
                    "egc_bwd_src",
                )
            return GM, gb_part, gslabs

        fused_dw = {}

        def edge_dgrad(GM):
            addend = gy_out if (ctx.residual and gy_out is not None) else None
            Kin_ = y.shape[1]
            if (ctx.param_grads and Kin_ == H and w_eg.shape == (H, Kin_) and GM.stride(0) % 4 == 0 and y.stride(0) % 4 == 0
                    and dgrad_wgrad_applies(m, H, Kin_, gm_amax, ctx.y_amax) and _x6_shape_ok(_Shape(m, H), Kin_, H)):
                src = ctx.y_src if (ctx.y_src is not None and BNRED_FUSED and not layer and tuple(ctx.y_src[0].shape) == (m, Kin_)
                                    and ctx.y_src[0].stride(0) % 4 == 0) else None
                out, dW, red = gemm_dgrad_wgrad(GM, gm_amax, y, ctx.y_amax, split_f16x2(w_eg, True), addend,
                                                src[0] if src is not None else None, src[1] if src is not None else None)
                fused_dw["g_weg"] = dW
                if src is not None:
                    BNRED_STATS["fused"] += 1
                    k = id(out)
                    _PRE_RED[k] = (weakref.ref(out, lambda _r, k=k: _orphan_pre_red(k)), src[0], red)
                return out
            return _dgrad_bnred(GM, w_eg, addend, gm_amax, ctx.y_src)

        ev_d = ev_w = None
        if ctx.lane:
            main, T = _lane_streams(x.device)
            ev_n = _event_after(main)
            for t in (GP, gs1, gs0, gp_amax, gm_amax, P):
                if t is not None:
                    t.record_stream(T)
            with _on_T(main, T, reads=(gy_out,)):
                e_red, g_branch, e_stat_arg = edge_branch()
                T.wait_event(ev_n)
                GM, gb_part, gslabs = gate_backward(e_red, g_branch, e_stat_arg)
                e_red = fused_red.get("e", e_red)
                ev_d = _event_after(T)
                g_y = edge_dgrad(GM)
                if "g_weg" in fused_dw:
                    ev_w = _event_after(T)
            main.wait_event(ev_d)
            if ctx.y_on_T and (not ctx.param_grads or _deferred_join_is_safe((e_gamma, e_beta))):
                _arm_backward_join()
                _mark_on_T(g_y)
            else:
                main.wait_stream(T)
                for t in (g_y, e_red):
                    if t is not None:
                        t.record_stream(main)
        else:
            e_red, g_branch, e_stat_arg = edge_branch()
            GM, gb_part, gslabs = gate_backward(e_red, g_branch, e_stat_arg)
            e_red = fused_red.get("e", e_red)
        def _wgrads():
            g_beg_ = _empty(H, like=x)
            check(lib.alignn_slab_sum(ptr(gb_part), gslabs, H, ptr(g_beg_), stream()), "slab_sum")
            g_weg_ = fused_dw["g_weg"] if "g_weg" in fused_dw else gemm_tn(GM, y, gm_amax, y_amax)
            return g_weg_, g_beg_, gemm_tn(GP, x, gp_amax, x_amax), col_sum(GP)

        x_amax, y_amax = ctx.x_amax, ctx.y_amax

        g_x = _dgrad(GP, wcat, addend=gx_out if ctx.residual else None, g_amax=gp_amax)
        if not ctx.lane:
            g_y = edge_dgrad(GM)
        if not ctx.param_grads:
            return (None, g_x, g_y) + (None,) * 24
        g_weg, g_beg, g_wcat, g_bcat = on_side_stream(_wgrads, [GM, y, GP, x, gb_part, gm_amax, gp_amax, x_amax, y_amax],
                                                      ctx.leaves, wait=(ev_d, ev_w))
        dn_gamma, dn_beta = n_red[1], n_red[0]
        de_gamma = e_red[1] if e_red is not None else None
        de_beta = e_red[0] if e_red is not None else None
        gw4 = tuple(g_wcat[i * H:(i + 1) * H] for i in range(4))
        gb4 = tuple(g_bcat[i * H:(i + 1) * H] for i in range(4))
        return (None, g_x, g_y, None, None) + gw4 + gb4 + (g_weg, g_beg, dn_gamma, dn_beta, None, None, de_gamma,
                                                            de_beta, None, None, None, None, None, None)


def edge_gated_conv_cat(graph: CSRGraph, x, y, wcat, bcat, w_eg, b_eg, n_gamma, n_beta, n_rm, n_rv, e_gamma, e_beta, e_rm,
                        e_rv, training: bool, residual: bool, need_y: bool = True, norm: str = "batch"):
    H = wcat.shape[0] // 4
    w4 = tuple(wcat[i * H:(i + 1) * H] for i in range(4))
    b4 = tuple(bcat[i * H:(i + 1) * H] for i in range(4))
    return EdgeGatedConvFn.apply(graph, x, y, wcat.detach(), bcat.detach(), *w4, *b4, w_eg, b_eg, n_gamma, n_beta, n_rm,
                                 n_rv, e_gamma, e_beta, e_rm, e_rv, training, residual, need_y, norm)


def edge_gated_conv_infer(graph: CSRGraph, x, y, wcat, bcat, w_eg, b_eg, n_gamma, n_beta, n_rm, n_rv, e_gamma, e_beta,
                          e_rm, e_rv, residual: bool, need_y: bool = True):
    lib = _lib.load()
    x, y = x.contiguous(), y.contiguous()
    n, H = x.shape
    m = y.shape[0]
    if n != graph.n_nodes or m != graph.n_edges:
        raise ValueError(f"feature rows ({n},{m}) do not match graph ({graph.n_nodes},{graph.n_edges})")
    P = project(x, wcat, bcat)
    C = project(y, w_eg, b_eg)
    n_stat = _bn_finalize(None, 0, n, n_gamma, n_beta, n_rm, n_rv, False)
    e_stat = _bn_finalize(None, 0, m, e_gamma, e_beta, e_rm, e_rv, False)
    xpre = _empty(n, H, like=x)
    y_out = _empty(m, H, like=x) if need_y else None
    y_amax = new_amax(x) if (need_y and _track(m)) else None
    check(
        lib.alignn_egc_gate_infer(ptr(P), ptr(C), ptr(graph.seg_ptr), ptr(graph.seg_node), ptr(graph.src), n, m, H,
                                  ptr(xpre), ptr(e_stat), ptr(y) if residual else None, ptr(y_out), ptr(y_amax), stream()),
        "egc_gate_infer",
    )
    if y_amax is not None:
        set_amax(y_out, y_amax)
    x_out = _bn_silu_fwd(xpre, x if residual else None, n_stat)
    return x_out, y_out


def _rbf_raw(d, centers, gamma):
    lib = _lib.load()
    require_f32(d, centers)
    rows, bins = d.numel(), centers.numel()
    out = _empty(rows, bins, like=d)
    check(lib.alignn_rbf_fwd(ptr(d), ptr(centers), float(gamma), ptr(out), rows, bins, stream()), "rbf_fwd")
    return out


class RbfFn(torch.autograd.Function):

    @staticmethod
    def forward(ctx, d, centers, gamma):
        d = d.contiguous()
        ctx.save_for_backward(d, centers)
        ctx.gamma = float(gamma)
        return _rbf_raw(d, centers, gamma)

    @staticmethod
    def backward(ctx, g):
        lib = _lib.load()
        d, centers = ctx.saved_tensors
        g = g.contiguous()
        gd = _empty(d.numel(), like=d)
        check(lib.alignn_rbf_bwd(ptr(d), ptr(centers), ctx.gamma, ptr(g), ptr(gd), d.numel(), centers.numel(), stream()),
              "rbf_bwd")
        return gd.reshape(d.shape), None, None


def rbf_expand(d, centers, gamma):
    if d.requires_grad:
        return RbfFn.apply(d, centers, gamma)
    return _rbf_raw(d.contiguous(), centers, gamma)


def _bond_length_raw(r):
    lib = _lib.load()
    require_f32(r)
    out = _empty(r.shape[0], like=r)
    check(lib.alignn_norm3_fwd(ptr(r), ptr(out), r.shape[0], stream()), "norm3_fwd")
    return out


class BondLengthFn(torch.autograd.Function):
    @staticmethod
    def forward(ctx, r):
        r = r.contiguous()
        ctx.save_for_backward(r)
        return _bond_length_raw(r)

    @staticmethod
    def backward(ctx, g):
        lib = _lib.load()
        (r,) = ctx.saved_tensors
        gr = torch.empty_like(r)
        check(lib.alignn_norm3_bwd(ptr(r), ptr(g.contiguous()), ptr(gr), r.shape[0], stream()), "norm3_bwd")
        return gr


def bond_length(r):
    if r.requires_grad:
        return BondLengthFn.apply(r)
    return _bond_length_raw(r.contiguous())


class AvgPoolFn(torch.autograd.Function):

    @staticmethod
    def forward(ctx, x, graph_ptr):
        lib = _lib.load()
        x = x.contiguous()
        B = graph_ptr.numel() - 1
        H = x.shape[1]
        out = _empty(B, H, like=x)
        check(lib.alignn_segment_mean_fwd(ptr(x), ptr(graph_ptr), ptr(out), B, H, stream()), "segment_mean_fwd")
        ctx.save_for_backward(graph_ptr)
        ctx.n = x.shape[0]
        return out

    @staticmethod
    def backward(ctx, g):
        lib = _lib.load()
        (graph_ptr,) = ctx.saved_tensors
        g = g.contiguous()
        B, H = g.shape
        gx = _empty(ctx.n, H, like=g)
        check(lib.alignn_segment_mean_bwd(ptr(g), ptr(graph_ptr), ptr(gx), B, H, stream()), "segment_mean_bwd")
        return gx, None
```

Before: 4499.

## Fuse bias-gradient column sums into the split-product TN weight-gradient GEMM

Adds alignn_gemm_tn_bias, which computes the bias gradient (column sums of the output gradient) inside the x6 TN GEMM kernel. Only the first k-tile blocks accumulate the sums, and they are reduced together with the dW partials in one combined slab-reduce launch. The edge-gated conv wgrad and large MLP backward now call it instead of a separate col_sum pass, which avoids re-reading GP and saves kernel launches. The cost is extra template variants, a larger workspace, and a fallback path when the fused conditions fail.

```diff
diff --git a/alignn_amd/_abi.py b/alignn_amd/_abi.py
--- a/alignn_amd/_abi.py
+++ b/alignn_amd/_abi.py
@@ -14,6 +14,7 @@
 LATER_HEADERS = ("alignn_idpp.h", "alignn_cells.h", "alignn_local.h")
 ANALYSIS_HEADERS = ("alignn_vanhove.h",)
 STRUCTURE_HEADERS = ("alignn_voronoi.h",)
+KERNEL_HEADERS = ("alignn_gemm_bias.h",)
 
 _BASE = {"void": None, "char": C.c_char, "uint8_t": C.c_uint8, "uint64_t": C.c_uint64, "int": C.c_int, "int32_t": C.c_int32,
          "int64_t": C.c_int64, "size_t": C.c_size_t, "float": C.c_float, "double": C.c_double}
diff --git a/alignn_amd/_lib.py b/alignn_amd/_lib.py
--- a/alignn_amd/_lib.py
+++ b/alignn_amd/_lib.py
@@ -6,6 +6,7 @@
 
 import torch
 
+from ._abi import KERNEL_HEADERS, header
 from ._abi import SIGNATURES, STRUCTS
 
 HERE = os.path.dirname(os.path.abspath(__file__))
@@ -42,6 +43,8 @@
             )
         lib = C.CDLL(LIB_PATH)
         _type(lib, SIGNATURES)
+        for name in KERNEL_HEADERS:
+            _type(lib, header(name).signatures)
         sizes = [lib.alignn_egc_args_sizeof(k) for k in range(3)] + [lib.alignn_fire_args_sizeof(), lib.alignn_md_args_sizeof()]
         for size, block in zip(sizes, (EgcFwdArgs, EgcBwdArgs, EgcWgradArgs, FireArgs, MdArgs)):
             _check_size(block.__name__, size, block)
diff --git a/alignn_amd/build.py b/alignn_amd/build.py
--- a/alignn_amd/build.py
+++ b/alignn_amd/build.py
@@ -9,7 +9,7 @@
 import tempfile
 from concurrent.futures import ThreadPoolExecutor
 
-from ._abi import ANALYSIS_HEADERS, LATER_HEADERS, STRUCTURE_HEADERS, WORKFLOW_HEADERS
+from ._abi import ANALYSIS_HEADERS, KERNEL_HEADERS, LATER_HEADERS, STRUCTURE_HEADERS, WORKFLOW_HEADERS
 
 HERE = os.path.dirname(os.path.abspath(__file__))
 CSRC = os.path.join(HERE, "csrc")
@@ -56,7 +56,8 @@
 def _headers():
     include = os.path.join(os.path.dirname(HERE), "include")
     return [os.path.join(CSRC, f) for f in os.listdir(CSRC) if f.endswith(".h")] + [
-        os.path.join(include, f) for f in ("alignn_hip.h",) + WORKFLOW_HEADERS + LATER_HEADERS + ANALYSIS_HEADERS + STRUCTURE_HEADERS]
+        os.path.join(include, f)
+        for f in ("alignn_hip.h",) + KERNEL_HEADERS + WORKFLOW_HEADERS + LATER_HEADERS + ANALYSIS_HEADERS + STRUCTURE_HEADERS]
 
 
 def _stale(target, deps) -> bool:
diff --git a/alignn_amd/csrc/composite.hip b/alignn_amd/csrc/composite.hip
--- a/alignn_amd/csrc/composite.hip
+++ b/alignn_amd/csrc/composite.hip
@@ -1,5 +1,6 @@
 #include "common.h"
 #include "../../include/alignn_hip.h"
+#include "../../include/alignn_gemm_bias.h"
 
 namespace {
 
@@ -250,8 +251,7 @@
 }
 
 size_t alignn_egc_conv_wgrad_scratch(int64_t n, int64_t m, int H, int Kin) {
-    return (al(alignn_gemm_tn_workspace(m, H, Kin) / 4 + 1) + al(alignn_gemm_tn_workspace(n, 4 * H, Kin) / 4 + 1) +
-            al((size_t)alignn_col_stats_slabs(n) * 2 * 4 * H)) * sizeof(float);
+    return (al(alignn_gemm_tn_workspace(m, H, Kin) / 4 + 1) + al(alignn_gemm_tn_workspace(n, 4 * H, Kin) / 4 + 1)) * sizeof(float);
 }
 
 int alignn_egc_conv_wgrad(const alignn_egc_wgrad_args* a, alignn_stream_t st) {
@@ -261,13 +261,12 @@
     const size_t b1 = alignn_gemm_tn_workspace(m, H, Kin), b2 = alignn_gemm_tn_workspace(n, 4 * H, Kin);
     float* ws1 = a->scratch;
     float* ws2 = ws1 + al(b1 / 4 + 1);
-    float* ws3 = ws2 + al(b2 / 4 + 1);
     if (a->scratch_bytes < alignn_egc_conv_wgrad_scratch(n, m, H, Kin)) return (int)hipErrorInvalidValue;
     ALIGNN_TRY(alignn_slab_sum(a->gb_part, a->gb_slabs, H, a->g_beg, st));
     ALIGNN_TRY(alignn_gemm_tn(a->GM, H, a->gm_amax, a->y, Kin, a->y_amax, a->g_weg, Kin, m, H, Kin, ws1, b1, st));
-    ALIGNN_TRY(alignn_gemm_tn(a->GP, 4 * H, a->gp_amax, a->x, Kin, a->x_amax, a->g_wcat, Kin, n, 4 * H, Kin, ws2, b2, st));
-    ALIGNN_TRY(alignn_col_sum(a->GP, 4 * H, n, 4 * H, a->g_bcat, ws3, st));
-    return 0;
-}
-
-}
+    ALIGNN_TRY(alignn_gemm_tn_bias(a->GP, 4 * H, a->gp_amax, a->x, Kin, a->x_amax, a->g_wcat, Kin, a->g_bcat, n, 4 * H, Kin, ws2, b2,
+                                   st));
+    return 0;
+}
+
+}
diff --git a/alignn_amd/csrc/gemm_f32.hip b/alignn_amd/csrc/gemm_f32.hip
--- a/alignn_amd/csrc/gemm_f32.hip
+++ b/alignn_amd/csrc/gemm_f32.hip
@@ -1,5 +1,6 @@
 #include "mfma_f16x3.h"
 #include "../../include/alignn_hip.h"
+#include "../../include/alignn_gemm_bias.h"
 
 namespace {
 
@@ -282,10 +283,10 @@
 }
 
 
-__global__ __launch_bounds__(1024) void slab_reduce4_kernel(const float* __restrict__ ws, int splits, int64_t count,
-                                                            int cols, float* __restrict__ out, int64_t ldo) {
-    __shared__ double sh[16][64][4];
-    const int64_t idx = ((int64_t)blockIdx.x * 64 + threadIdx.x) * 4;
+template <bool VEC>
+__device__ __forceinline__ void slab_reduce4_block(const float* __restrict__ ws, int splits, int64_t count, int cols,
+                                                   float* __restrict__ out, int64_t ldo, int64_t block, double (*sh)[64][4]) {
+    const int64_t idx = (block * 64 + threadIdx.x) * 4;
     double s0 = 0.0, s1 = 0.0, s2 = 0.0, s3 = 0.0;
     if (idx < count) {
         int k = threadIdx.y;
@@ -319,8 +320,30 @@
             const double* p = sh[k][threadIdx.x];
             t0 += p[0], t1 += p[1], t2 += p[2], t3 += p[3];
         }
-        f4_st(out + (idx / cols) * ldo + (idx % cols), make_float4((float)t0, (float)t1, (float)t2, (float)t3));
-    }
+        float* o = out + (idx / cols) * ldo + (idx % cols);
+        if (VEC)
+            f4_st(o, make_float4((float)t0, (float)t1, (float)t2, (float)t3));
+        else
+            o[0] = (float)t0, o[1] = (float)t1, o[2] = (float)t2, o[3] = (float)t3;
+    }
+}
+
+__global__ __launch_bounds__(1024) void slab_reduce4_kernel(const float* __restrict__ ws, int splits, int64_t count,
+                                                            int cols, float* __restrict__ out, int64_t ldo) {
+    __shared__ double sh[16][64][4];
+    slab_reduce4_block<true>(ws, splits, count, cols, out, ldo, blockIdx.x, sh);
+}
+
+__global__ __launch_bounds__(1024) void slab_reduce4_sums_kernel(const float* __restrict__ ws, int splits, int64_t count,
+                                                                 int cols, float* __restrict__ out, int64_t ldo,
+                                                                 const float* __restrict__ sums_ws, int n_sums,
+                                                                 float* __restrict__ sums) {
+    __shared__ double sh[16][64][4];
+    const int64_t dw_blocks = (count + 255) / 256;
+    if ((int64_t)blockIdx.x < dw_blocks)
+        slab_reduce4_block<true>(ws, splits, count, cols, out, ldo, blockIdx.x, sh);
+    else
+        slab_reduce4_block<false>(sums_ws, splits, n_sums, n_sums, sums, n_sums, (int64_t)blockIdx.x - dw_blocks, sh);
 }
 
 inline void launch_slab_reduce(const float* ws, int splits, int64_t count, int cols, float* out, int64_t ldo,
@@ -492,52 +515,105 @@
 int alignn_gemm_tn_x6_supported(int64_t M, int N, int K);
 size_t alignn_gemm_tn_x6_workspace(int64_t M, int N, int K);
 int alignn_gemm_tn_x6_splits(int64_t M, int N, int K);
+int alignn_gemm_tn_x6_sums_fused(int64_t M, int N, int K);
+int alignn_gemm_tn_x6_partials_sums(const float* G, int64_t ldg, const float* g_amax, const float* X, int64_t ldx,
+                                    const float* x_amax, int64_t M, int N, int K, void* workspace, size_t workspace_bytes,
+                                    float* bias_ws, alignn_stream_t stream);
 static bool tn_use_x6(const float* G, int64_t ldg, const float* A, int64_t lda, int64_t M, int N, int K) {
     return alignn_gemm_tn_x6_supported(M, N, K) && (ldg % 4 == 0) && (lda % 4 == 0) && aligned16(G) && aligned16(A);
 }
 
 size_t alignn_gemm_tn_workspace(int64_t M, int N, int K) {
-    const size_t f32 = (size_t)tn_splits(M, N, K) * (size_t)N * (size_t)K * sizeof(float);
+    size_t nb = (size_t)tn_splits(M, N, K) * (size_t)N * (size_t)K * sizeof(float);
     if (alignn_gemm_tn_x6_supported(M, N, K)) {
-        const size_t x6 = alignn_gemm_tn_x6_workspace(M, N, K);
-        return x6 > f32 ? x6 : f32;
-    }
-    return f32;
+        size_t x6 = alignn_gemm_tn_x6_workspace(M, N, K);
+        if (alignn_gemm_tn_x6_sums_fused(M, N, K)) x6 += (size_t)alignn_gemm_tn_x6_splits(M, N, K) * (size_t)N * sizeof(float);
+        if (x6 > nb) nb = x6;
+    }
+    if (N % 4 == 0) {
+        const size_t cs = (size_t)alignn_col_stats_slabs(M) * 2 * (size_t)N * sizeof(float);
+        if (cs > nb) nb = cs;
+    }
+    return nb;
+}
+
+namespace {
+__global__ __launch_bounds__(256) void col_walk_kernel(const float* __restrict__ G, int64_t ldg, int64_t M, int N,
+                                                       float* __restrict__ sums) {
+    const int n = blockIdx.x * 256 + threadIdx.x;
+    if (n >= N) return;
+    float s = 0.0f;
+    for (int64_t m = 0; m < M; ++m) s += G[m * ldg + n];
+    sums[n] = s;
+}
+
+int gemm_tn(const float* G, int64_t ldg, const float* g_amax, const float* A, int64_t lda, const float* a_amax, float* dW,
+            int64_t lddw, float* col_sums, int64_t M, int N, int K, void* workspace, size_t workspace_bytes, hipStream_t st) {
+    if (M < 0 || N <= 0 || K <= 0) return (int)hipErrorInvalidValue;
+    const bool vec_ok = (N % 4 == 0) && (K % 4 == 0) && (ldg % 4 == 0) && (lda % 4 == 0) && aligned16(G) && aligned16(A);
+    if (!vec_ok || M == 0) {
+        const int rc = naive(G, 1, ldg, A, 1, lda, nullptr, nullptr, 0, dW, lddw, N, K, M, st);
+        if (rc || col_sums == nullptr) return rc;
+        hipLaunchKernelGGL(col_walk_kernel, dim3(alignn_ceil_div(N, 256)), dim3(256), 0, st, G, ldg, M, N, col_sums);
+        ALIGNN_CHECK_LAUNCH();
+        return 0;
+    }
+    if (workspace_bytes < alignn_gemm_tn_workspace(M, N, K) || workspace == nullptr) return (int)hipErrorInvalidValue;
+    float* ws = (float*)workspace;
+    const int64_t count = (int64_t)N * K;
+    if (tn_use_x6(G, ldg, A, lda, M, N, K)) {
+        const bool f16 = g_amax != nullptr && a_amax != nullptr;
+        const int splits6 = alignn_gemm_tn_x6_splits(M, N, K);
+        if (col_sums != nullptr && alignn_gemm_tn_x6_sums_fused(M, N, K)) {
+            float* sums_ws = ws + (size_t)splits6 * count;
+            int rc6 = alignn_gemm_tn_x6_partials_sums(G, ldg, f16 ? g_amax : nullptr, A, lda, f16 ? a_amax : nullptr, M, N, K,
+                                                      workspace, workspace_bytes, sums_ws, (alignn_stream_t)st);
+            if (rc6) return rc6;
+            if ((lddw & 3) == 0 && aligned16(dW)) {
+                hipLaunchKernelGGL(slab_reduce4_sums_kernel, dim3(alignn_ceil_div(count, 256) + N / 256), dim3(64, 16), 0, st, ws,
+                                   splits6, count, K, dW, lddw, sums_ws, N, col_sums);
+            } else {
+                launch_slab_reduce(ws, splits6, count, K, dW, lddw, st);
+                hipLaunchKernelGGL(slab_reduce_kernel, dim3(alignn_ceil_div(N, 32)), dim3(32, 32), 0, st, sums_ws, splits6,
+                                   (int64_t)N, N, col_sums, (int64_t)N);
+            }
+            ALIGNN_CHECK_LAUNCH();
+            return 0;
+        }
+        int rc6 = alignn_gemm_tn_x6_partials(G, ldg, f16 ? g_amax : nullptr, A, lda, f16 ? a_amax : nullptr, M, N, K,
+                                             workspace, workspace_bytes, (alignn_stream_t)st);
+        if (rc6) return rc6;
+        launch_slab_reduce(ws, splits6, count, K, dW, lddw, st);
+        ALIGNN_CHECK_LAUNCH();
+    } else {
+        const int splits = tn_splits(M, N, K);
+        GemmArgs g{G, ldg, A, lda, nullptr, nullptr, 0, ws, K, N, K, M, tn_chunk(M, N, K), (int64_t)N * K, 1, 0, 0, 0};
+        int rc;
+        if (K > 64)
+            rc = launch<128, 128, 2, 2, false, false>(g, splits, st);
+        else if (N > 64)
+            rc = launch<128, 64, 4, 1, false, false>(g, splits, st);
+        else
+            rc = launch<64, 64, 2, 1, false, false>(g, splits, st);
+        if (rc) return rc;
+        launch_slab_reduce(ws, splits, count, K, dW, lddw, st);
+        ALIGNN_CHECK_LAUNCH();
+    }
+    return col_sums != nullptr ? alignn_col_sum(G, ldg, M, N, col_sums, ws, (alignn_stream_t)st) : 0;
+}
 }
 
 int alignn_gemm_tn(const float* G, int64_t ldg, const float* g_amax, const float* A, int64_t lda, const float* a_amax,
                    float* dW, int64_t lddw, int64_t M, int N, int K, void* workspace, size_t workspace_bytes,
                    alignn_stream_t stream) {
-    if (M < 0 || N <= 0 || K <= 0) return (int)hipErrorInvalidValue;
-    hipStream_t st = (hipStream_t)stream;
-    const bool vec_ok = (N % 4 == 0) && (K % 4 == 0) && (ldg % 4 == 0) && (lda % 4 == 0) && aligned16(G) && aligned16(A);
-    if (!vec_ok || M == 0) return naive(G, 1, ldg, A, 1, lda, nullptr, nullptr, 0, dW, lddw, N, K, M, st);
-    if (workspace_bytes < alignn_gemm_tn_workspace(M, N, K) || workspace == nullptr) return (int)hipErrorInvalidValue;
-    float* ws = (float*)workspace;
-    if (tn_use_x6(G, ldg, A, lda, M, N, K)) {
-        const bool f16 = g_amax != nullptr && a_amax != nullptr;
-        int rc6 = alignn_gemm_tn_x6_partials(G, ldg, f16 ? g_amax : nullptr, A, lda, f16 ? a_amax : nullptr, M, N, K,
-                                             workspace, workspace_bytes, stream);
-        if (rc6) return rc6;
-        const int64_t count6 = (int64_t)N * K;
-        launch_slab_reduce(ws, alignn_gemm_tn_x6_splits(M, N, K), count6, K, dW, lddw, st);
-        ALIGNN_CHECK_LAUNCH();
-        return 0;
-    }
-    const int splits = tn_splits(M, N, K);
-    GemmArgs g{G, ldg, A, lda, nullptr, nullptr, 0, ws, K, N, K, M, tn_chunk(M, N, K), (int64_t)N * K, 1, 0, 0, 0};
-    int rc;
-    if (K > 64)
-        rc = launch<128, 128, 2, 2, false, false>(g, splits, st);
-    else if (N > 64)
-        rc = launch<128, 64, 4, 1, false, false>(g, splits, st);
-    else
-        rc = launch<64, 64, 2, 1, false, false>(g, splits, st);
-    if (rc) return rc;
-    const int64_t count = (int64_t)N * K;
-    launch_slab_reduce(ws, splits, count, K, dW, lddw, st);
-    ALIGNN_CHECK_LAUNCH();
-    return 0;
-}
-
-}
+    return gemm_tn(G, ldg, g_amax, A, lda, a_amax, dW, lddw, nullptr, M, N, K, workspace, workspace_bytes, (hipStream_t)stream);
+}
+
+int alignn_gemm_tn_bias(const float* G, int64_t ldg, const float* g_amax, const float* A, int64_t lda, const float* a_amax,
+                        float* dW, int64_t lddw, float* col_sums, int64_t M, int N, int K, void* workspace,
+                        size_t workspace_bytes, alignn_stream_t stream) {
+    if (col_sums == nullptr) return (int)hipErrorInvalidValue;
+    return gemm_tn(G, ldg, g_amax, A, lda, a_amax, dW, lddw, col_sums, M, N, K, workspace, workspace_bytes, (hipStream_t)stream);
+}
+
+}
diff --git a/alignn_amd/csrc/gemm_x6.hip b/alignn_amd/csrc/gemm_x6.hip
--- a/alignn_amd/csrc/gemm_x6.hip
+++ b/alignn_amd/csrc/gemm_x6.hip
@@ -668,6 +668,7 @@
     const float* X;
     int64_t ldx;
     float* ws;
+    float* bias_ws;
     int64_t M;
     int N, K;
     int64_t chunk;
@@ -676,7 +677,7 @@
     const float* x_amax;
 };
 
-template <bool F16>
+template <bool F16, bool BIAS = false>
 __global__ __launch_bounds__(TNT) void gemm_tn_x6_kernel(TnArgs g) {
     extern __shared__ __attribute__((aligned(16))) unsigned char smem[];
     constexpr int NPL = TSch<F16>::NPL, BUF = TSch<F16>::BUF;
@@ -708,6 +709,8 @@
     const int col = t & 255;
     const float* src = is_x ? g.X + k0 + col : g.G + n0 + col;
     const int64_t ld = is_x ? g.ldx : g.ldg;
+    const bool sums = BIAS && !is_x && k0 == 0;
+    float csum = 0.0f;
     float scale = 1.0f, inv_s0 = 1.0f, inv_s1 = 1.0f;
     if constexpr (F16) {
         const float sg = f16_scale(*g.g_amax), sx = f16_scale(*g.x_amax);
@@ -756,6 +759,11 @@
         if (valid < TSTEP) {       \
             _Pragma("unroll") for (int m = 0; m < TSTEP; ++m) R[m] = m < valid ? R[m] : 0.0f;                   \
         }                                                                                                       \
+        if constexpr (BIAS) {                                                                                   \
+            if (sums) {                                                                                         \
+                _Pragma("unroll") for (int m = 0; m < TSTEP; ++m) csum += R[m];                                 \
+            }                                                                                                   \
+        }                                                                                                       \
         _Pragma("unroll") for (int c = 0; c < 2; ++c) {                                                         \
             float x[8];                                                                                         \
             _Pragma("unroll") for (int j = 0; j < 8; ++j) x[j] = R[8 * c + j];                                  \
@@ -841,6 +849,9 @@
     float* patch = reinterpret_cast<float*>(smem) + wave * (32 * PLD);
     const int prow = lane >> 4, pc4 = (lane & 15) * 4;
     float* out = g.ws + (int64_t)z * g.N * g.K;
+    if constexpr (BIAS) {
+        if (sums) g.bias_ws[(int64_t)z * g.N + n0 + col] = csum;
+    }
 #pragma unroll
     for (int ahb = 0; ahb < TRM * (TRN / 2); ++ahb) {
         const int a = ahb / (TRN / 2), hb = ahb % (TRN / 2);
@@ -1256,34 +1267,59 @@
 
 int alignn_gemm_tn_x6_splits(int64_t M, int N, int K) { return tn::tn_splits(M, N, K); }
 
-int alignn_gemm_tn_x6_partials(const float* G, int64_t ldg, const float* g_amax, const float* X, int64_t ldx,
-                               const float* x_amax, int64_t M, int N, int K, void* workspace, size_t workspace_bytes,
-                               alignn_stream_t stream) {
+static int tn_partials(const float* G, int64_t ldg, const float* g_amax, const float* X, int64_t ldx, const float* x_amax, int64_t M,
+                int N, int K, void* workspace, size_t workspace_bytes, float* bias_ws, alignn_stream_t stream) {
     if (!alignn_gemm_tn_x6_supported(M, N, K)) return (int)hipErrorInvalidValue;
     if ((ldg & 3) || (ldx & 3) || !aligned16(G) || !aligned16(X) || !aligned16(workspace) ||
         workspace_bytes < alignn_gemm_tn_x6_workspace(M, N, K))
         return (int)hipErrorInvalidValue;
     if ((g_amax == nullptr) != (x_amax == nullptr)) return (int)hipErrorInvalidValue;
-    tn::TnArgs g{G, ldg, X, ldx, (float*)workspace, M, N, K, tn::tn_chunk(M, N, K), N / tn::TBN, K / tn::TBK,
+    tn::TnArgs g{G, ldg, X, ldx, (float*)workspace, bias_ws, M, N, K, tn::tn_chunk(M, N, K), N / tn::TBN, K / tn::TBK,
                  tn::tn_splits(M, N, K), g_amax, x_amax};
     static bool tn_attr = false;
     if (!tn_attr) {
-        hipError_t e = hipFuncSetAttribute((const void*)tn::gemm_tn_x6_kernel<false>,
-                                           hipFuncAttributeMaxDynamicSharedMemorySize, tn::TSch<false>::LDS);
-        if (e == hipSuccess)
-            e = hipFuncSetAttribute((const void*)tn::gemm_tn_x6_kernel<true>, hipFuncAttributeMaxDynamicSharedMemorySize,
-                                    tn::TSch<true>::LDS);
-        if (e != hipSuccess) return (int)e;
+        const void* kernels[4] = {(const void*)tn::gemm_tn_x6_kernel<false, false>, (const void*)tn::gemm_tn_x6_kernel<false, true>,
+                                  (const void*)tn::gemm_tn_x6_kernel<true, false>, (const void*)tn::gemm_tn_x6_kernel<true, true>};
+        for (int i = 0; i < 4; ++i) {
+            hipError_t e = hipFuncSetAttribute(kernels[i], hipFuncAttributeMaxDynamicSharedMemorySize,
+                                               i < 2 ? tn::TSch<false>::LDS : tn::TSch<true>::LDS);
+            if (e != hipSuccess) return (int)e;
+        }
         tn_attr = true;
     }
     const int tiles = g.tiles_n * g.tiles_k;
-    const int per_xcd = alignn_ceil_div(g.splits, 8) * tiles;
-    if (g_amax)
-        hipLaunchKernelGGL(tn::gemm_tn_x6_kernel<true>, dim3(per_xcd * 8), dim3(tn::TNT), tn::TSch<true>::LDS, (hipStream_t)stream, g);
-    else
-        hipLaunchKernelGGL(tn::gemm_tn_x6_kernel<false>, dim3(per_xcd * 8), dim3(tn::TNT), tn::TSch<false>::LDS, (hipStream_t)stream, g);
+    const dim3 grid(alignn_ceil_div(g.splits, 8) * tiles * 8), block(tn::TNT);
+    hipStream_t st = (hipStream_t)stream;
+    if (g_amax) {
+        if (bias_ws)
+            hipLaunchKernelGGL((tn::gemm_tn_x6_kernel<true, true>), grid, block, tn::TSch<true>::LDS, st, g);
+        else
+            hipLaunchKernelGGL((tn::gemm_tn_x6_kernel<true, false>), grid, block, tn::TSch<true>::LDS, st, g);
+    } else {
+        if (bias_ws)
+            hipLaunchKernelGGL((tn::gemm_tn_x6_kernel<false, true>), grid, block, tn::TSch<false>::LDS, st, g);
+        else
+            hipLaunchKernelGGL((tn::gemm_tn_x6_kernel<false, false>), grid, block, tn::TSch<false>::LDS, st, g);
+    }
     ALIGNN_CHECK_LAUNCH();
     return 0;
+}
+
+int alignn_gemm_tn_x6_partials(const float* G, int64_t ldg, const float* g_amax, const float* X, int64_t ldx,
+                               const float* x_amax, int64_t M, int N, int K, void* workspace, size_t workspace_bytes,
+                               alignn_stream_t stream) {
+    return tn_partials(G, ldg, g_amax, X, ldx, x_amax, M, N, K, workspace, workspace_bytes, nullptr, stream);
+}
+
+int alignn_gemm_tn_x6_sums_fused(int64_t M, int N, int K) {
+    return (alignn_gemm_tn_x6_supported(M, N, K) && tn::tn_chunk(M, N, K) > 8 * tn::TSTEP) ? 1 : 0;
+}
+
+int alignn_gemm_tn_x6_partials_sums(const float* G, int64_t ldg, const float* g_amax, const float* X, int64_t ldx,
+                                    const float* x_amax, int64_t M, int N, int K, void* workspace, size_t workspace_bytes,
+                                    float* bias_ws, alignn_stream_t stream) {
+    if (bias_ws == nullptr || !aligned16(bias_ws) || !alignn_gemm_tn_x6_sums_fused(M, N, K)) return (int)hipErrorInvalidValue;
+    return tn_partials(G, ldg, g_amax, X, ldx, x_amax, M, N, K, workspace, workspace_bytes, bias_ws, stream);
 }
 
 int alignn_gemm_nt_x6_supported(int64_t M, int N, int K) { return (M > 0 && N >= 128 && N % 4 == 0 && K > 0 && K % BK == 0) ? 1 : 0; }
diff --git a/alignn_amd/csrc/model.hip b/alignn_amd/csrc/model.hip
--- a/alignn_amd/csrc/model.hip
+++ b/alignn_amd/csrc/model.hip
@@ -5,6 +5,7 @@
 #include <vector>
 
 #include "../../include/alignn_hip.h"
+#include "../../include/alignn_gemm_bias.h"
 #include "common.h"
 
 namespace {
@@ -596,6 +597,14 @@
     L(alignn_gemm_tn(g, ldg, g_amax, a, lda, a_amax, dW, K, M, N, K, ws, nb, st));
 }
 
+void gemm_tn_bias(Ctx& c, const float* g, int64_t ldg, const float* g_amax, const float* a, int64_t lda, const float* a_amax,
+                  float* dW, float* gb, int64_t M, int N, int K, hipStream_t st) {
+    if (g_amax == nullptr || a_amax == nullptr) g_amax = a_amax = nullptr;
+    const size_t nb = alignn_gemm_tn_workspace(M, N, K);
+    float* ws = c.tmp(st, nb / 4 + 1);
+    L(alignn_gemm_tn_bias(g, ldg, g_amax, a, lda, a_amax, dW, K, gb, M, N, K, ws, nb, st));
+}
+
 void col_sum(Ctx& c, const float* x, int64_t ldx, int64_t rows, int F, float* out, hipStream_t st) {
     float* ws = c.tmp(st, (size_t)alignn_col_stats_slabs(rows) * 2 * F);
     L(alignn_col_sum(x, ldx, rows, F, out, ws, st));
@@ -668,6 +677,10 @@
         if (t.lane) c.sync(sd, c.T);
     }
     c.tmp_reset(sd);
+    if (!ln && gb_part == nullptr) {
+        gemm_tn_bias(c, gpre, F, g_amax, t.x.p, K, t.x.amax, p.gW, p.gb, rows, F, K, sd);
+        return gx;
+    }
     gemm_tn(c, gpre, F, g_amax, t.x.p, K, t.x.amax, p.gW, rows, F, K, sd);
     if (gb_part != nullptr)
         L(alignn_slab_sum(gb_part, slabs, F, p.gb, sd));
@@ -796,8 +809,7 @@
     c.tmp_reset(sd);
     L(alignn_slab_sum(gb_part, gslabs, H, p.g_beg, sd));
     if (!dw) gemm_tn(c, GM, H, gm_amax, t.y.p, Kin, t.y.amax, p.g_weg, m, H, Kin, sd);
-    gemm_tn(c, GP, 4 * H, gp_amax, t.x.p, Kin, t.x.amax, p.g_wcat, n, 4 * H, Kin, sd);
-    col_sum(c, GP, 4 * H, n, 4 * H, p.g_bcat, sd);
+    gemm_tn_bias(c, GP, 4 * H, gp_amax, t.x.p, Kin, t.x.amax, p.g_wcat, p.g_bcat, n, 4 * H, Kin, sd);
 }
 
 void run_backward(Ctx& c, const Tape& tp, const float* g_out) {
diff --git a/alignn_amd/ops.py b/alignn_amd/ops.py
--- a/alignn_amd/ops.py
+++ b/alignn_amd/ops.py
@@ -810,6 +810,24 @@
     return out
 
 
+def gemm_tn_bias(g, a, g_amax=None, a_amax=None):
+    if not F16X3 or g_amax is None or a_amax is None:
+        g_amax = a_amax = None
+    lib = _lib.load()
+    require_f32(g, a)
+    M, N = g.shape
+    K = a.shape[1]
+    out, sums = _empty(N, K, like=g), _empty(N, like=g)
+    nbytes = lib.alignn_gemm_tn_workspace(M, N, K)
+    ws = torch.empty(max(nbytes // 4, 1), dtype=torch.float32, device=g.device)
+    check(
+        lib.alignn_gemm_tn_bias(ptr(g), g.stride(0), ptr(g_amax), ptr(a), a.stride(0), ptr(a_amax), ptr(out), out.stride(0),
+                                ptr(sums), M, N, K, ptr(ws), nbytes, stream()),
+        "gemm_tn_bias",
+    )
+    return out, sums
+
+
 def col_sum(x):
     lib = _lib.load()
     rows, F = x.shape
@@ -1132,7 +1150,12 @@
             check(_lib.load().alignn_slab_sum(ptr(gb_part[0]), gb_part[1], gpre.shape[1], ptr(out), stream()), "slab_sum")
             return out
 
-        gw, gb = on_side_stream(lambda: (gemm_tn(gpre, x, g_amax, x_amax), bias_grad()),
+        def grads():
+            if gb_part is None and ctx.norm != "layer" and gpre.shape[1] > 1024:
+                return gemm_tn_bias(gpre, x, g_amax, x_amax)
+            return gemm_tn(gpre, x, g_amax, x_amax), bias_grad()
+
+        gw, gb = on_side_stream(grads,
                                 [gpre, x, g_amax, x_amax, gb_part[0] if gb_part is not None else None], ctx.wb, wait=(ev,))
         return gx, gw, gb, dgamma, dbeta, None, None, None, None
 
@@ -1852,7 +1875,7 @@
             g_beg_ = _empty(H, like=x)
             check(lib.alignn_slab_sum(ptr(gb_part), gslabs, H, ptr(g_beg_), stream()), "slab_sum")
             g_weg_ = fused_dw["g_weg"] if "g_weg" in fused_dw else gemm_tn(GM, y, gm_amax, y_amax)
-            return g_weg_, g_beg_, gemm_tn(GP, x, gp_amax, x_amax), col_sum(GP)
+            return (g_weg_, g_beg_) + gemm_tn_bias(GP, x, gp_amax, x_amax)
 
         x_amax, y_amax = ctx.x_amax, ctx.y_amax
 
diff --git a/include/alignn_gemm_bias.h b/include/alignn_gemm_bias.h
--- /dev/null
+++ b/include/alignn_gemm_bias.h
@@ -0,0 +1,18 @@
+#ifndef ALIGNN_GEMM_BIAS_H
+#define ALIGNN_GEMM_BIAS_H
+
+#include <stddef.h>
+#include <stdint.h>
+
+#ifdef __cplusplus
+extern "C" {
+#endif
+
+int alignn_gemm_tn_bias(const float* G, int64_t ldg, const float* g_amax, const float* A, int64_t lda,
+                        const float* a_amax, float* dW, int64_t lddw, float* col_sums, int64_t M, int N, int K,
+                        void* workspace, size_t workspace_bytes, void* stream);
+
+#ifdef __cplusplus
+}
+#endif
+#endif
```

New measurement: 4541 (median of 6 runs). Within noise of the previous version (+0.9%).
